# yml-bit/CTA-GAN

Measured on AMD Instinct MI355X. Metric: paired 512x512 slices/sec (G+D step); generator rel-L2 vs CPU reference, higher is better.
Workload: dtype bf16; 1 GPU; HdGan stage-2 full G+D train step (G, Reg, STN, D_m, losses, Adam x3), 16 paired 512x512 slices/GPU; per_gpu_batch=16, global_batch=16, size=512, parallelism=single, rccl_ranks=1, dp_backend=none

## Files before the change

cta_gan_amd/_lib.py:

```python
from __future__ import annotations

import ctypes
import os

import torch

_HERE = os.path.dirname(os.path.abspath(__file__))
LIB_PATH = os.environ.get("CTG_LIB") or os.path.join(_HERE, "_build", "libctagan_hip.so")

_I, _L, _P, _F = ctypes.c_int, ctypes.c_long, ctypes.c_void_p, ctypes.c_float

SIGNATURES = {
    "ctg_conv_igemm": "iipppp" + "i" * 20 + "ppppp",
    "ctg_conv_igemm_classes": "i" + "pppp" + "i" * 14 + "ppppppp",
    "ctg_conv_wgrad": "ipppiiiiiiiiiiiiipp",
    "ctg_wgrad_reduce": "piiiipiilllip",
    "ctg_wgrad_reduce_multi": "ippppppppppppp",
    "ctg_in_stats": "ipiiiiiipppp",
    "ctg_in_finalize": "piiiiippp",
    "ctg_in_apply": "ipippipipiiiiip",
    "ctg_in_apply_part": "ipipippipipiiiiip",
    "ctg_in_bwd_partial": "ipipiippiiiiiipp",
    "ctg_in_bwd_apply": "ipipiippppipiiiiip",
    "ctg_in_bwd_stats": "ipipiippipiiiiiipp",
    "ctg_in_bwd": "ipipiippipiiiiiipppp",
    "ctg_grad_combine": "ipipiipiipiiiiip",
    "ctg_fold_f32": "ppiiiiip",
    "ctg_act_bwd_f32": "ppiplp",
    "ctg_bias_grad": "ipiiiiiiiippip",
    "ctg_bias_grad_act": "ipiipiipiiiiiiippip",
    "ctg_maxpool2_fwd": "ipipiiiiip",
    "ctg_maxpool2_bwd": "ipipipiiiiiip",
    "ctg_bilinear_fwd": "ipipiiiiiiip",
    "ctg_bilinear_bwd": "ipipiiiiiiip",
    "ctg_copy_channels": "ipipiilp",
    "ctg_split_weights": "plpilp",
    "ctg_split_weights_multi": "ippppp",
    "ctg_pair_convert": "iplplilp",
    "ctg_abi_version": "",
    "ctg_chan_pad": "ipipilp",
    "ctg_im2col_pack": "ippiiiiiiiiipiiip",
    "ctg_conv_smallcin": "ippiiiiiiiiipiiipipiiiippp",
    "ctg_conv_tail7": "ipipppiiiip",
    "ctg_corr_smallcin": "piiiiiippiiiiiiiiiipip",
    "ctg_weight_pack": "ipllliipiiip",
    "ctg_weight_pack_multi": "iippppppppppp",
    "ctg_warp_fwd": "ppllllpiiip",
    "ctg_warp_bwd": "ppllllpppiiipp",
    "ctg_smooth_fwd": "plllliiiifppp",
    "ctg_smooth_bwd": "plllliiiifppip",
    "ctg_l1_fwd": "ppplfppp",
    "ctg_l1_bwd": "ppplfppip",
    "ctg_lsgan_fwd": "piiiffffippp",
    "ctg_lsgan_bwd": "piiiffffippp",
    "ctg_sum_scalars": "ippp",
    "ctg_act_bwd_sum_f32": "ppiplppip",
    "ctg_avgpool_fwd": "piipp",
    "ctg_avgpool_bwd": "piipp",
    "ctg_to_windowdata": "ppppilp",
    "ctg_window_metrics": "ppppiliippp",
    "ctg_ssim": "ppppiiiiidppp",
    "ctg_conv_cout1_fwd": "ipipppiiiiiiiiip",
    "ctg_conv_cout1_bwd": "ipppiiiiiiiiip",
    "ctg_conv_cout1_wgrad": "ippipiiiiiiiiip",
    "ctg_hu_to_inputs": "pffpplp",
    "ctg_resize_nearest": "piiipiip",
    "ctg_adam_step": "ipppppffffipp",
    "ctg_adam_tick": "pffp",
}
DIAG_SIGNATURES = {
    "ctg_lds_canary": "iipip",
}
_CT = {"i": _I, "l": _L, "p": _P, "f": _F, "d": ctypes.c_double}
ABI_VERSION = 11

_lib = None


def ensure_built():
    if os.environ.get("CTG_LIB") or os.environ.get("CTG_NO_AUTOBUILD") is not None:
        return
    from . import build as _build
    if _build.is_current():
        return
    try:
        _build._hipcc()
    except RuntimeError:
        return
    import sys
    print("cta_gan_amd: kernel sources changed -- building %s (hipcc, a few minutes)" % LIB_PATH, file=sys.stderr, flush=True)
    _build.build()


def load():
    global _lib
    if _lib is not None:
        return _lib
    ensure_built()
    if not os.path.exists(LIB_PATH):
        raise RuntimeError(
            "libctagan_hip.so not found at %s and hipcc is not available to build it (`python -m cta_gan_amd.build`): "
            "the HIP path is the only implementation; there is no fallback" % LIB_PATH)
    lib = ctypes.CDLL(LIB_PATH)
    try:
        ver = lib.ctg_abi_version
    except AttributeError:
        raise RuntimeError("%s predates ctg_abi_version(): rebuild it (`python -m cta_gan_amd.build --force`)" % LIB_PATH)
    ver.argtypes, ver.restype = [], _I
    if ver() != ABI_VERSION:
        raise RuntimeError("%s has C-ABI version %d, this binding was written against %d: rebuild it "
                           "(`python -m cta_gan_amd.build --force`)" % (LIB_PATH, ver(), ABI_VERSION))
    for name, sig in SIGNATURES.items():
        fn = getattr(lib, name)
        fn.argtypes = [_CT[c] for c in sig]
        fn.restype = _I
    for name, sig in DIAG_SIGNATURES.items():
        fn = getattr(lib, name, None)
        if fn is not None:
            fn.argtypes = [_CT[c] for c in sig]
            fn.restype = _I
    _lib = lib
    return lib


def check(status: int, what: str):
    if status != 0:
        if status == 1:
            raise RuntimeError("%s: invalid argument (CTG_EINVAL)" % what)
        raise RuntimeError("%s: HIP error %d" % (what, status - 1000))
```

cta_gan_amd/csrc/common.h:

```cpp
#pragma once
#include <hip/hip_runtime.h>
#include <stdint.h>
#include <utility>
#include "../../include/ctagan_hip.h"

#define CTG_OK 0
#define CTG_EINVAL 1

enum { DT_F32 = 0, DT_BF16 = 1, DT_PAIR = 2, DT_MIX = 3 };
enum { ACT_NONE = 0, ACT_RELU = 1, ACT_LRELU = 2, ACT_TANH = 3, ACT_SIGMOID = 4 };
enum { PAD_ZERO = 0, PAD_REFLECT = 1 };

typedef __bf16 bf16_t;
struct bfpair_t { bf16_t v; };
typedef float f32x4 __attribute__((ext_vector_type(4)));
typedef unsigned u32x4 __attribute__((ext_vector_type(4)));
typedef __bf16 bf16x8 __attribute__((ext_vector_type(8)));
typedef __bf16 bf16x4 __attribute__((ext_vector_type(4)));

#define LRELU_SLOPE 0.2f

#define CTG_ENTER() (void)hipGetLastError()

static inline int ctg_launch_status() {
    hipError_t e = hipGetLastError();
    return e == hipSuccess ? CTG_OK : 1000 + (int)e;
}

static inline int ctg_cu_count() {
    static int n_cu[64];
    int dev = 0;
    if (hipGetDevice(&dev) != hipSuccess) dev = 0;
    dev &= 63;
    if (n_cu[dev] == 0) {
        int n = 0;
        n_cu[dev] = (hipDeviceGetAttribute(&n, hipDeviceAttributeMultiprocessorCount, dev) == hipSuccess && n > 0) ? n : 256;
    }
    return n_cu[dev];
}
static inline int ctg_lds_attr_once(const void* fn, int bytes, unsigned long long* mask) {
    int dev = 0;
    if (hipGetDevice(&dev) != hipSuccess) dev = 0;
    const unsigned long long bit = 1ull << (dev & 63);
    if (*mask & bit) return CTG_OK;
    const hipError_t e = hipFuncSetAttribute(fn, hipFuncAttributeMaxDynamicSharedMemorySize, bytes);
    if (e != hipSuccess) return 1000 + (int)e;
    *mask |= bit;
    return CTG_OK;
}

template <typename T> struct VecOf;
template <> struct VecOf<float> { static constexpr int N = 4; };
template <> struct VecOf<bf16_t> { static constexpr int N = 8; };
template <> struct VecOf<bfpair_t> { static constexpr int N = 8; };

template <typename T> struct Chunk;
template <> struct Chunk<float> {
    static constexpr int N = 4;
    float v[4];
    __device__ __forceinline__ void load(const float* p) {
        const f32x4 t = *reinterpret_cast<const f32x4*>(p);
        v[0] = t[0]; v[1] = t[1]; v[2] = t[2]; v[3] = t[3];
    }
    __device__ __forceinline__ void store(float* p) const {
        *reinterpret_cast<f32x4*>(p) = f32x4{v[0], v[1], v[2], v[3]};
    }
    __device__ __forceinline__ void load(const float* p, int) { load(p); }
    __device__ __forceinline__ void store(float* p, int) const { store(p); }
    __device__ __forceinline__ void zero() { v[0] = v[1] = v[2] = v[3] = 0.f; }
};
template <> struct Chunk<bf16_t> {
    static constexpr int N = 8;
    float v[8];
    __device__ __forceinline__ void load(const bf16_t* p) {
        const u32x4 t = *reinterpret_cast<const u32x4*>(p);
#pragma unroll
        for (int i = 0; i < 4; ++i) {
            v[2 * i] = __uint_as_float(t[i] << 16);
            v[2 * i + 1] = __uint_as_float(t[i] & 0xffff0000u);
        }
    }
    __device__ __forceinline__ void store(bf16_t* p) const {
        bf16x8 o;
#pragma unroll
        for (int i = 0; i < 8; ++i) o[i] = (bf16_t)v[i];
        *reinterpret_cast<bf16x8*>(p) = o;
    }
    __device__ __forceinline__ void load(const bf16_t* p, int) { load(p); }
    __device__ __forceinline__ void store(bf16_t* p, int) const { store(p); }
    __device__ __forceinline__ void zero() {
#pragma unroll
        for (int i = 0; i < 8; ++i) v[i] = 0.f;
    }
};
template <> struct Chunk<bfpair_t> {
    static constexpr int N = 8;
    float v[8];
    __device__ __forceinline__ void load(const bfpair_t* p, int ld) {
        const u32x4 h = *reinterpret_cast<const u32x4*>(p);
        const u32x4 l = *reinterpret_cast<const u32x4*>(p + (ld >> 1));
#pragma unroll
        for (int i = 0; i < 4; ++i) {
            v[2 * i] = __uint_as_float(h[i] << 16) + __uint_as_float(l[i] << 16);
            v[2 * i + 1] = __uint_as_float(h[i] & 0xffff0000u) + __uint_as_float(l[i] & 0xffff0000u);
        }
    }
    __device__ __forceinline__ void store(bfpair_t* p, int ld) const {
        bf16x8 h, l;
#pragma unroll
        for (int i = 0; i < 8; ++i) {
            h[i] = (bf16_t)v[i];
            l[i] = (bf16_t)(v[i] - (float)h[i]);
        }
        *reinterpret_cast<bf16x8*>(p) = h;
        *reinterpret_cast<bf16x8*>(p + (ld >> 1)) = l;
    }
    __device__ __forceinline__ void zero() {
#pragma unroll
        for (int i = 0; i < 8; ++i) v[i] = 0.f;
    }
};
template <typename T> struct PlanesOf { static constexpr int N = 1; };
template <> struct PlanesOf<bfpair_t> { static constexpr int N = 2; };

__device__ __forceinline__ float ld1(const float* p) { return *p; }
__device__ __forceinline__ float ld1(const bf16_t* p) { return (float)*p; }
__device__ __forceinline__ void st1(float* p, float v) { *p = v; }
__device__ __forceinline__ void st1(bf16_t* p, float v) { *p = (bf16_t)v; }

__device__ __forceinline__ float act_apply(float x, int act) {
    switch (act) {
        case ACT_RELU: return x > 0.f ? x : 0.f;
        case ACT_LRELU: return x > 0.f ? x : LRELU_SLOPE * x;
        case ACT_TANH: return tanhf(x);
        case ACT_SIGMOID: return 1.f / (1.f + __expf(-x));
        default: return x;
    }
}
__device__ __forceinline__ float act_grad_from_out(float y, int act) {
    switch (act) {
        case ACT_RELU: return y > 0.f ? 1.f : 0.f;
        case ACT_LRELU: return y > 0.f ? 1.f : LRELU_SLOPE;
        case ACT_TANH: return 1.f - y * y;
        case ACT_SIGMOID: return y * (1.f - y);
        default: return 1.f;
    }
}

template <typename F, int... I>
__device__ __forceinline__ void static_for_impl(F&& f, std::integer_sequence<int, I...>) {
    (f(std::integral_constant<int, I>{}), ...);
}
template <int N, typename F> __device__ __forceinline__ void static_for(F&& f) {
    static_for_impl(static_cast<F&&>(f), std::make_integer_sequence<int, N>{});
}

#define IN_EPS 1e-5f

__device__ __forceinline__ int xcd_contiguous(int id, int G) {
    const int x = id & 7, q = G >> 3, r = G & 7;
    return x * q + (x < r ? x : r) + (id >> 3);
}

__device__ __forceinline__ void lds_barrier() {
    asm volatile("s_waitcnt lgkmcnt(0)" ::: "memory");
    __builtin_amdgcn_s_barrier();
    asm volatile("" ::: "memory");
}

template <int KCH> __device__ __forceinline__ int swz(int row, int c) {
    if constexpr (KCH == 4) return c ^ ((row >> 1) & 3);
    else return c ^ (row & 7);
}

__device__ __forceinline__ int reflect_idx(int i, int n) {
    i = i < 0 ? -i : i;
    return i >= n ? 2 * (n - 1) - i : i;
}

__device__ __forceinline__ float row16_sum_to_lane15(float v) {
    v += __builtin_bit_cast(float, __builtin_amdgcn_update_dpp(0, __builtin_bit_cast(int, v), 0x111, 0xf, 0xf, true));
    v += __builtin_bit_cast(float, __builtin_amdgcn_update_dpp(0, __builtin_bit_cast(int, v), 0x112, 0xf, 0xf, true));
    v += __builtin_bit_cast(float, __builtin_amdgcn_update_dpp(0, __builtin_bit_cast(int, v), 0x114, 0xf, 0xf, true));
    v += __builtin_bit_cast(float, __builtin_amdgcn_update_dpp(0, __builtin_bit_cast(int, v), 0x118, 0xf, 0xf, true));
    return v;
}

__device__ __forceinline__ float wave_sum(float v) {
#pragma unroll
    for (int o = 32; o > 0; o >>= 1) v += __shfl_xor(v, o, 64);
    return v;
}
```

cta_gan_amd/csrc/norm_act.hip:

```cpp
#include "common.h"
#include "ctg_knobs.h"

#define MAX_SLABS 128

__device__ __forceinline__ int fold_srcs(int y, int H, int p, int* s) {
    int k = 0;
    s[k++] = y;
    if (y >= 1 && y <= p) s[k++] = -y;
    if (y >= H - 1 - p && y <= H - 2) s[k++] = 2 * (H - 1) - y;
    return k;
}

template <typename T>
__device__ __forceinline__ void fold_load(Chunk<T>& out, const T* __restrict__ d, int n, int y, int x, int ch, int H,
                                          int W, int p, int ld) {
    if (p == 0) {
        out.load(d + (((size_t)n * H + y) * W + x) * ld + ch, ld);
        return;
    }
    const int Hp = H + 2 * p, Wp = W + 2 * p;
    int ys[3], xs[3];
    const int ny = fold_srcs(y, H, p, ys), nx = fold_srcs(x, W, p, xs);
    out.zero();
    for (int a = 0; a < ny; ++a)
// ... 23 lines not shown
    const int pbeg = slab * per, pend = min(pbeg + per, HW);
    const int ch = cc * EPC;
    float s1[EPC], s2[EPC], mu[EPC], rs[EPC];
#pragma unroll
    for (int e = 0; e < EPC; ++e) {
        s1[e] = 0.f; s2[e] = 0.f;
        if (MODE == 1) { mu[e] = mean[n * C + ch + e]; rs[e] = rstd[n * C + ch + e]; }
    }
    constexpr int UNR = 4;
    for (int pb = pbeg + pl; pb < pend; pb += PL * UNR) {
        Chunk<TX> v[UNR];
        Chunk<T> g[UNR];
        bool ok[UNR];
#pragma unroll
        for (int u = 0; u < UNR; ++u) {
            const int p = pb + u * PL;
            ok[u] = p < pend;
            const int pc = ok[u] ? p : pbeg;
            if (MODE == 0 || MODE == 1 || MODE == 3) v[u].load(x + ((size_t)n * HW + pc) * x_ld + ch, x_ld);
            if (MODE == 1 || MODE == 2 || MODE == 3) {
                if (pad == 0) {
                    g[u].load(dout + ((size_t)n * HW + pc) * d_ld + ch, d_ld);
                } else {
                    const int y = pc / W;
                    fold_load<T>(g[u], dout, n, y, pc - y * W, ch, H, W, pad, d_ld);
                }
            }
        }
#pragma unroll
        for (int u = 0; u < UNR; ++u) {
            if (!ok[u]) continue;
            if (MODE == 0) {
#pragma unroll
                for (int e = 0; e < EPC; ++e) { s1[e] += v[u].v[e]; s2[e] += v[u].v[e] * v[u].v[e]; }
            } else if (MODE == 1) {
#pragma unroll
                for (int e = 0; e < EPC; ++e) {
                    const float xh = (v[u].v[e] - mu[e]) * rs[e];
                    float gg = g[u].v[e];
                    if (act == ACT_RELU) gg = xh > 0.f ? gg : 0.f;
                    else if (act == ACT_LRELU) gg = xh > 0.f ? gg : LRELU_SLOPE * gg;
                    s1[e] += gg; s2[e] += gg * xh;
                }
            } else if (MODE == 3) {
                Chunk<T> o;
#pragma unroll
                for (int e = 0; e < EPC; ++e) {
                    o.v[e] = g[u].v[e] * act_grad_from_out(v[u].v[e], act);
                    s1[e] += o.v[e];
                }
                o.store(gout + ((size_t)n * HW + pb + u * PL) * go_ld + ch, go_ld);
            } else {
#pragma unroll
                for (int e = 0; e < EPC; ++e) s1[e] += g[u].v[e];
            }
        }
    }
    float* out = part + (((size_t)n * nslabs + slab) * C) * 2;
    __shared__ float stage[256 * 8];
#pragma unroll
    for (int which = 0; which < 2; ++which) {
        __syncthreads();
#pragma unroll
        for (int e = 0; e < EPC; ++e) stage[pl * C + ch + e] = which ? s2[e] : s1[e];
        __syncthreads();
        for (int c = tid; c < C; c += 256) {
            float s = 0.f;
            for (int q = 0; q < PL; ++q) s += stage[q * C + c];
            out[c * 2 + which] = s;
        }
    }
}


__global__ __launch_bounds__(64) void moments_finalize_wave_kernel(const float* __restrict__ part, int nslabs, int C,
                                                                   float invHW, int mode, float* __restrict__ mean,
                                                                   float* __restrict__ rstd) {
    const int i = blockIdx.x;
    const int n = i / C, c = i - n * C;
    double a = 0.0, b = 0.0;
    for (int s = threadIdx.x; s < nslabs; s += 64) {
        const float* p = part + (((size_t)n * nslabs + s) * C + c) * 2;
        a += (double)p[0];
        b += (double)p[1];
    }
#pragma unroll
    for (int o = 32; o > 0; o >>= 1) {
        a += __shfl_xor(a, o, 64);
        b += __shfl_xor(b, o, 64);
    }
    if (threadIdx.x == 0) {
        if (mode == 0) {
            const double m = a * invHW;
            double var = b * invHW - m * m;
            var = var < 0.0 ? 0.0 : var;
            mean[i] = (float)m;
            rstd[i] = (float)(1.0 / sqrt(var + (double)IN_EPS));
        } else {
            mean[i] = (float)(a * invHW);
            rstd[i] = (float)(b * invHW);
        }
    }
}

__global__ __launch_bounds__(64) void bias_finalize_kernel(const float* __restrict__ part, int B, int nslabs, int C,
                                                           int Creal, float* __restrict__ db, int accumulate) {
    const int c = blockIdx.x;
    if (c >= Creal) return;
    const int total = B * nslabs;
    float a = 0.f;
    for (int i = threadIdx.x; i < total; i += 64) a += part[((size_t)i * C + c) * 2];
    a = wave_sum(a);
    if (threadIdx.x == 0) db[c] = accumulate ? db[c] + a : a;
}

template <typename T> struct ChanParams {
    static constexpr int EPC = Chunk<T>::N;
    float v[EPC];
    __device__ __forceinline__ void load(const float* __restrict__ p) {
#pragma unroll
        for (int q = 0; q < EPC / 4; ++q) {
            const f32x4 t = *reinterpret_cast<const f32x4*>(p + 4 * q);
            v[4 * q] = t[0]; v[4 * q + 1] = t[1]; v[4 * q + 2] = t[2]; v[4 * q + 3] = t[3];
        }
    }
};

template <typename T>
__global__ __launch_bounds__(256) void in_apply_kernel(const T* x, int x_ld,
                                                       const float* __restrict__ mean,
                                                       const float* __restrict__ rstd, int act,
                                                       const T* res, int r_ld, T* out,
                                                       int o_ld, int HW, int C) {
    constexpr int EPC = Chunk<T>::N;
    const int CPP = C / EPC, PL = 256 / CPP;
    const int cc = threadIdx.x % CPP, pl = threadIdx.x / CPP;
    const int n = blockIdx.y, ch = cc * EPC;
    ChanParams<T> mu, rs;
    mu.load(mean + n * C + ch);
    rs.load(rstd + n * C + ch);
    const size_t base = (size_t)n * HW;
    for (int p = blockIdx.x * PL + pl; p < HW; p += gridDim.x * PL) {
        Chunk<T> v, o;
        v.load(x + (base + p) * x_ld + ch, x_ld);
#pragma unroll
        for (int e = 0; e < EPC; ++e) o.v[e] = act_apply((v.v[e] - mu.v[e]) * rs.v[e], act);
        if (res != nullptr) {
            Chunk<T> r;
            r.load(res + (base + p) * r_ld + ch, r_ld);
#pragma unroll
            for (int e = 0; e < EPC; ++e) o.v[e] += r.v[e];
        }
        o.store(out + (base + p) * o_ld + ch, o_ld);
    }
}

template <typename T, typename TX = T>
__global__ __launch_bounds__(256) void in_bwd_apply_kernel(const TX* __restrict__ x, int x_ld,
                                                           const T* __restrict__ dout, int d_ld, int pad,
                                                           const float* __restrict__ mean,
                                                           const float* __restrict__ rstd,
                                                           const float* __restrict__ s1,
                                                           const float* __restrict__ s2, int act,
                                                           T* __restrict__ dx, int dx_ld, int H, int W, int C) {
    constexpr int EPC = Chunk<T>::N;
    const int CPP = C / EPC, PL = 256 / CPP;
    const int cc = threadIdx.x % CPP, pl = threadIdx.x / CPP;
    const int n = blockIdx.y, ch = cc * EPC;
    const int HW = H * W;
    ChanParams<T> mu, rs, a1, a2;
    mu.load(mean + n * C + ch);
    rs.load(rstd + n * C + ch);
    a1.load(s1 + n * C + ch);
    a2.load(s2 + n * C + ch);
    const size_t base = (size_t)n * HW;
    for (int p = blockIdx.x * PL + pl; p < HW; p += gridDim.x * PL) {
        Chunk<TX> v;
        Chunk<T> g, o;
        v.load(x + (base + p) * x_ld + ch, x_ld);
        if (pad == 0) {
            g.load(dout + (base + p) * d_ld + ch, d_ld);
        } else {
            const int y = p / W;
            fold_load<T>(g, dout, n, y, p - y * W, ch, H, W, pad, d_ld);
        }
#pragma unroll
        for (int e = 0; e < EPC; ++e) {
            const float xh = (v.v[e] - mu.v[e]) * rs.v[e];
            float gg = g.v[e];
            if (act == ACT_RELU) gg = xh > 0.f ? gg : 0.f;
            else if (act == ACT_LRELU) gg = xh > 0.f ? gg : LRELU_SLOPE * gg;
            o.v[e] = rs.v[e] * (gg - a1.v[e] - xh * a2.v[e]);
        }
        o.store(dx + (base + p) * dx_ld + ch, dx_ld);
    }
}

#define FUSED_MAX_SLABS 128

template <int MODE>
__device__ __forceinline__ void wg_finalize(const float* __restrict__ part, int n, int nslabs, int C, int c0, int nch,
                                            float invHW, float* fa, float* fb, double* scratch) {
    const int tid = threadIdx.x;
    const int npairs = 2 * nch;
    const int stripes = 256 / npairs;
    const int pair = tid % npairs, stripe = tid / npairs;
    double acc = 0.0;
    const float* src = part + ((size_t)n * nslabs * C + c0) * 2 + pair;
    for (int s = stripe; s < nslabs; s += stripes) acc += (double)src[(size_t)s * C * 2];
    scratch[stripe * npairs + pair] = acc;
    __syncthreads();
    if (tid < nch) {
        double a = 0.0, b = 0.0;
        for (int q = 0; q < stripes; ++q) { a += scratch[q * npairs + 2 * tid]; b += scratch[q * npairs + 2 * tid + 1]; }
        if (MODE == 0) {
            const double m = a * invHW;
            double var = b * invHW - m * m;
            var = var < 0.0 ? 0.0 : var;
            fa[tid] = (float)m;
            fb[tid] = (float)(1.0 / sqrt(var + (double)IN_EPS));
        } else {
            fa[tid] = (float)(a * invHW);
            fb[tid] = (float)(b * invHW);
        }
    }
    __syncthreads();
}

template <typename T>
__global__ __launch_bounds__(256) void in_apply_part_kernel(const T* x, int x_ld,
                                                            const float* __restrict__ part, int nslabs, float invHW,
                                                            float* __restrict__ mean, float* __restrict__ rstd, int act,
                                                            const T* res, int r_ld, T* out,
                                                            int o_ld, int HW, int C, int CGC) {
    constexpr int EPC = Chunk<T>::N;
    __shared__ double scratch[256];
    __shared__ float fa[64], fb[64];
    const int PL = 256 / CGC;
    const int cc = threadIdx.x % CGC, pl = threadIdx.x / CGC;
    const int n = blockIdx.z, c0 = blockIdx.y * CGC * EPC, ch = c0 + cc * EPC;
    const size_t base = (size_t)n * HW;
    constexpr int UNR = 4;
    const int p0 = blockIdx.x * PL + pl, pstep = gridDim.x * PL;
    Chunk<T> v[UNR], r[UNR];
#pragma unroll
    for (int u = 0; u < UNR; ++u) {
        const int p = p0 + u * pstep;
        const int pc = p < HW ? p : 0;
        v[u].load(x + (base + pc) * x_ld + ch, x_ld);
        if (res != nullptr) r[u].load(res + (base + pc) * r_ld + ch, r_ld);
    }
    wg_finalize<0>(part, n, nslabs, C, c0, CGC * EPC, invHW, fa, fb, scratch);
    if (blockIdx.x == 0 && threadIdx.x < CGC * EPC) {
        mean[(size_t)n * C + c0 + threadIdx.x] = fa[threadIdx.x];
        rstd[(size_t)n * C + c0 + threadIdx.x] = fb[threadIdx.x];
    }
    float mu[EPC], rs[EPC];
#pragma unroll
    for (int e = 0; e < EPC; ++e) { mu[e] = fa[cc * EPC + e]; rs[e] = fb[cc * EPC + e]; }
    for (int pb = p0; pb < HW; pb += UNR * pstep) {
#pragma unroll
        for (int u = 0; u < UNR; ++u) {
            const int p = pb + u * pstep;
            if (p < HW) {
                Chunk<T> o;
#pragma unroll
                for (int e = 0; e < EPC; ++e) o.v[e] = act_apply((v[u].v[e] - mu[e]) * rs[e], act);
                if (res != nullptr) {
#pragma unroll
                    for (int e = 0; e < EPC; ++e) o.v[e] += r[u].v[e];
                }
                o.store(out + (base + p) * o_ld + ch, o_ld);
            }
        }
        const int pn = pb + UNR * pstep;
        if (pn < HW) {
#pragma unroll
            for (int u = 0; u < UNR; ++u) {
                const int p = pn + u * pstep;
                const int pc = p < HW ? p : 0;
                v[u].load(x + (base + pc) * x_ld + ch, x_ld);
                if (res != nullptr) r[u].load(res + (base + pc) * r_ld + ch, r_ld);
            }
        }
    }
}

template <typename T, typename TX = T>
__global__ __launch_bounds__(256) void in_bwd_apply_part_kernel(const TX* __restrict__ x, int x_ld,
                                                                const T* __restrict__ dout, int d_ld, int pad,
                                                                const float* __restrict__ mean,
                                                                const float* __restrict__ rstd,
                                                                const float* __restrict__ part, int nslabs, float invHW,
                                                                int act, T* __restrict__ dx, int dx_ld, int H, int W,
                                                                int C, int CGC) {
    constexpr int EPC = Chunk<T>::N;
    __shared__ double scratch[256];
    __shared__ float fa[64], fb[64];
    const int PL = 256 / CGC;
    const int cc = threadIdx.x % CGC, pl = threadIdx.x / CGC;
    const int n = blockIdx.z, c0 = blockIdx.y * CGC * EPC, ch = c0 + cc * EPC;
    const int HW = H * W;
    const size_t base = (size_t)n * HW;
    constexpr int UNR = 2;
    const int p0 = blockIdx.x * PL + pl, pstep = gridDim.x * PL;
    Chunk<TX> v[UNR];
// ... 21 lines not shown
#pragma unroll
    for (int e = 0; e < EPC; ++e) { a1[e] = fa[cc * EPC + e]; a2[e] = fb[cc * EPC + e]; }
    for (int pb = p0; pb < HW; pb += UNR * pstep) {
#pragma unroll
        for (int u = 0; u < UNR; ++u) {
            const int p = pb + u * pstep;
            if (p < HW) {
                Chunk<T> o;
#pragma unroll
                for (int e = 0; e < EPC; ++e) {
                    const float xh = (v[u].v[e] - mu.v[e]) * rs.v[e];
                    float gg = g[u].v[e];
                    if (act == ACT_RELU) gg = xh > 0.f ? gg : 0.f;
                    else if (act == ACT_LRELU) gg = xh > 0.f ? gg : LRELU_SLOPE * gg;
                    o.v[e] = rs.v[e] * (gg - a1[e] - xh * a2[e]);
                }
                o.store(dx + (base + p) * dx_ld + ch, dx_ld);
            }
        }
        const int pn = pb + UNR * pstep;
        if (pn < HW) fetch(pn);
    }
}

template <typename T>
__global__ void grad_combine_kernel(const T* __restrict__ a, int a_ld, const T* __restrict__ b, int b_ld, int pad,
                                    const T* __restrict__ yact, int y_ld, int act, T* __restrict__ out, int o_ld,
                                    int H, int W, int C, long items) {
    constexpr int EPC = Chunk<T>::N;
    const int CPP = C / EPC;
    const int HW = H * W;
    for (long it = (long)blockIdx.x * blockDim.x + threadIdx.x; it < items; it += (long)gridDim.x * blockDim.x) {
        const unsigned pixu = (unsigned)it / (unsigned)CPP;
        const long pix = pixu;
        const int ch = (int)(it - pix * CPP) * EPC;
        Chunk<T> o;
        o.zero();
        if (a != nullptr) o.load(a + pix * a_ld + ch, a_ld);
        if (b != nullptr) {
            const int n = (int)(pixu / (unsigned)HW);
            const int p = (int)(pix - (long)n * HW);
            const int y = p / W, xx = p - y * W;
            Chunk<T> t;
            fold_load<T>(t, b, n, y, xx, ch, H, W, pad, b_ld);
#pragma unroll
            for (int e = 0; e < EPC; ++e) o.v[e] += t.v[e];
        }
        if (yact != nullptr) {
            Chunk<T> yv;
            yv.load(yact + pix * y_ld + ch, y_ld);
#pragma unroll
            for (int e = 0; e < EPC; ++e) o.v[e] *= act_grad_from_out(yv.v[e], act);
        }
        o.store(out + pix * o_ld + ch, o_ld);
    }
}

__global__ void fold_f32_kernel(const float* __restrict__ dp, float* __restrict__ out, int B, int H, int W, int C,
                                int p) {
    const long total = (long)B * H * W * C;
    const int Hp = H + 2 * p, Wp = W + 2 * p;
    for (long i = (long)blockIdx.x * blockDim.x + threadIdx.x; i < total; i += (long)gridDim.x * blockDim.x) {
        const int c = (int)(i % C);
        const int x = (int)((i / C) % W);
        const int y = (int)((i / ((long)C * W)) % H);
        const int n = (int)(i / ((long)C * W * H));
        int ys[3], xs[3];
        const int ny = fold_srcs(y, H, p, ys), nx = fold_srcs(x, W, p, xs);
        float s = 0.f;
        for (int a = 0; a < ny; ++a)
            for (int b = 0; b < nx; ++b) s += dp[(((size_t)n * Hp + ys[a] + p) * Wp + xs[b] + p) * C + c];
        out[i] = s;
    }
}

__global__ void act_bwd_f32_kernel(const float* __restrict__ g, const float* __restrict__ y, int act,
                                   float* __restrict__ out, long n) {
    for (long i = (long)blockIdx.x * blockDim.x + threadIdx.x; i < n; i += (long)gridDim.x * blockDim.x)
        out[i] = g[i] * act_grad_from_out(y[i], act);
}

static inline int ew_blocks(long items) {
    long b = (items + 255) / 256;
    return (int)(b < 1 ? 1 : (b > 8192 ? 8192 : b));
}

static inline dim3 pix_grid(int dtype, int B, int HW, int C) {
    const int cpp = C / (dtype == DT_F32 ? 4 : 8);
    const int pl = 256 / cpp;
    const bool no_smallb = ctg_knobs().no_smallb;
    int per = 16;
    if (!no_smallb) while (per > 2 && (((long)HW + pl * per - 1) / (pl * per)) * B < 2048) per >>= 1;
    long bx = ((long)HW + pl * per - 1) / (pl * per);
    if (bx < 1) bx = 1;
    if (bx > 4096) bx = 4096;
    return dim3((unsigned)bx, (unsigned)B);
}

static inline bool pow2(int v) { return v > 0 && (v & (v - 1)) == 0; }

#define DISPATCH_T(dtype, CALL)                   \
    if ((dtype) == DT_BF16) { typedef bf16_t T; CALL; } \
    else if ((dtype) == DT_F32) { typedef float T; CALL; } \
    else if ((dtype) == DT_PAIR) { typedef bfpair_t T; CALL; } \
    else return CTG_EINVAL;

#define DISPATCH_TX(dtype, CALL)                  \
    if ((dtype) == DT_BF16) { typedef bf16_t T; typedef bf16_t TX; CALL; } \
    else if ((dtype) == DT_F32) { typedef float T; typedef float TX; CALL; } \
    else if ((dtype) == DT_PAIR) { typedef bfpair_t T; typedef bfpair_t TX; CALL; } \
    else if ((dtype) == DT_MIX) { typedef bf16_t T; typedef bfpair_t TX; CALL; } \
    else return CTG_EINVAL;

static int check_c(int dtype, int C) {
    const int epc = dtype == DT_F32 ? 4 : 8;
    if (C % epc) return CTG_EINVAL;
    const int cpp = C / epc;
    return (pow2(cpp) && cpp <= 256) ? CTG_OK : CTG_EINVAL;
}

extern "C" int ctg_in_stats(int dtype, const void* x, int x_ld, int B, int H, int W, int C, int nslabs, float* part,
                            float* mean, float* rstd, void* stream) {
    CTG_ENTER();
    if (check_c(dtype, C) || nslabs < 1 || nslabs > MAX_SLABS) return CTG_EINVAL;
    hipStream_t st = (hipStream_t)stream;
    DISPATCH_T(dtype, hipLaunchKernelGGL((moments_partial_kernel<T, 0>), dim3(nslabs, B), dim3(256), 0, st,
                                         (const T*)x, x_ld, (const T*)nullptr, 0, 0, (const float*)nullptr,
                                         (const float*)nullptr, 0, H, W, C, part));
    if (mean != nullptr)
        hipLaunchKernelGGL(moments_finalize_wave_kernel, dim3(B * C), dim3(64), 0, st, part, nslabs, C,
                           1.0f / (float)(H * W), 0, mean, rstd);
    return ctg_launch_status();
}

extern "C" int ctg_in_finalize(const float* part, int B, int C, int nslabs, int HW, int mode, float* mean, float* rstd,
                               void* stream) {
    CTG_ENTER();
    if (B < 1 || C < 1 || nslabs < 1 || HW < 1 || (mode != 0 && mode != 1)) return CTG_EINVAL;
    hipLaunchKernelGGL(moments_finalize_wave_kernel, dim3(B * C), dim3(64), 0, (hipStream_t)stream, part, nslabs, C,
                       1.0f / (float)HW, mode, mean, rstd);
    return ctg_launch_status();
}

extern "C" int ctg_in_apply(int dtype, const void* x, int x_ld, const float* mean, const float* rstd, int act,
                            const void* res, int r_ld, void* out, int o_ld, int B, int H, int W, int C, void* stream) {
    CTG_ENTER();
    if (check_c(dtype, C) || out == nullptr) return CTG_EINVAL;
    DISPATCH_T(dtype, hipLaunchKernelGGL((in_apply_kernel<T>), pix_grid(dtype, B, H * W, C), dim3(256), 0,
                                         (hipStream_t)stream, (const T*)x, x_ld, mean, rstd, act, (const T*)res, r_ld,
                                         (T*)out, o_ld, H * W, C));
    return ctg_launch_status();
}

static inline dim3 fused_grid(int dtype, int B, int HW, int C, int nslabs, int* cgc_out) {
    const int cpp = C / (dtype == DT_F32 ? 4 : 8);
    const int cgc = cpp < 8 ? cpp : 8;
    const int ncg = cpp / cgc, pl = 256 / cgc;
    long gx = (long)HW / (16L * nslabs);
    if (gx * ncg * B < 1024) gx = (1024 + (long)ncg * B - 1) / ((long)ncg * B);
    const long gmax = ((long)HW + pl * 4 - 1) / (pl * 4);
    if (gx > gmax) gx = gmax;
    if (gx < 1) gx = 1;
    *cgc_out = cgc;
    return dim3((unsigned)gx, (unsigned)ncg, (unsigned)B);
}

extern "C" int ctg_in_apply_part(int dtype, const void* x, int x_ld, const float* part, int nslabs, float* mean,
                                 float* rstd, int act, const void* res, int r_ld, void* out, int o_ld, int B, int H,
                                 int W, int C, void* stream) {
    CTG_ENTER();
    if (check_c(dtype, C) || nslabs < 1 || nslabs > FUSED_MAX_SLABS || part == nullptr || mean == nullptr || rstd == nullptr)
        return CTG_EINVAL;
    int cgc;
    const dim3 grid = fused_grid(dtype, B, H * W, C, nslabs, &cgc);
    DISPATCH_T(dtype, hipLaunchKernelGGL((in_apply_part_kernel<T>), grid, dim3(256), 0, (hipStream_t)stream, (const T*)x,
                                         x_ld, part, nslabs, 1.0f / (float)(H * W), mean, rstd, act, (const T*)res, r_ld,
                                         (T*)out, o_ld, H * W, C, cgc));
    return ctg_launch_status();
}

extern "C" int ctg_in_bwd_partial(int dtype, const void* x, int x_ld, const void* dout, int d_ld, int pad,
                                  const float* mean, const float* rstd, int act, int B, int H, int W, int C, int nslabs,
                                  float* part, void* stream) {
    CTG_ENTER();
    if (check_c(dtype, C) || nslabs < 1 || nslabs > MAX_SLABS || pad < 0 || pad >= H || pad >= W) return CTG_EINVAL;
    DISPATCH_TX(dtype, hipLaunchKernelGGL((moments_partial_kernel<T, 1, TX>), dim3(nslabs, B), dim3(256), 0,
                                          (hipStream_t)stream, (const TX*)x, x_ld, (const T*)dout, d_ld, pad, mean, rstd, act,
                                          H, W, C, part, (T*)nullptr, 0));
    return ctg_launch_status();
}

extern "C" int ctg_in_bwd(int dtype, const void* x, int x_ld, const void* dout, int d_ld, int pad, const float* mean,
                          const float* rstd, int act, void* dx, int dx_ld, int B, int H, int W, int C, int nslabs,
                          float* part, float* s1, float* s2, void* stream) {
    int st = ctg_in_bwd_partial(dtype, x, x_ld, dout, d_ld, pad, mean, rstd, act, B, H, W, C, nslabs, part, stream);
    if (st != CTG_OK) return st;
    st = ctg_in_finalize(part, B, C, nslabs, H * W, 1, s1, s2, stream);
    if (st != CTG_OK) return st;
    return ctg_in_bwd_apply(dtype, x, x_ld, dout, d_ld, pad, mean, rstd, s1, s2, act, dx, dx_ld, B, H, W, C, stream);
}

extern "C" int ctg_in_bwd_apply(int dtype, const void* x, int x_ld, const void* dout, int d_ld, int pad, const float* mean,
                                const float* rstd, const float* s1, const float* s2, int act, void* dx, int dx_ld, int B,
                                int H, int W, int C, void* stream) {
    CTG_ENTER();
    if (check_c(dtype, C) || pad < 0 || pad >= H || pad >= W || s1 == nullptr || s2 == nullptr) return CTG_EINVAL;
    DISPATCH_TX(dtype, hipLaunchKernelGGL((in_bwd_apply_kernel<T, TX>), pix_grid(dtype, B, H * W, C), dim3(256), 0,
                                          (hipStream_t)stream, (const TX*)x, x_ld, (const T*)dout, d_ld, pad, mean, rstd, s1, s2,
                                          act, (T*)dx, dx_ld, H, W, C));
    return ctg_launch_status();
}

extern "C" int ctg_in_bwd_stats(int dtype, const void* x, int x_ld, const void* dout, int d_ld, int pad, const float* mean,
                                const float* rstd, int act, void* dx, int dx_ld, int B, int H, int W, int C, int nslabs,
                                const float* part, void* stream) {
    CTG_ENTER();
    if (check_c(dtype, C) || nslabs < 1 || nslabs > FUSED_MAX_SLABS || part == nullptr || pad < 0 || pad >= H || pad >= W)
        return CTG_EINVAL;
    int cgc;
    const dim3 grid = fused_grid(dtype, B, H * W, C, nslabs, &cgc);
    DISPATCH_TX(dtype, hipLaunchKernelGGL((in_bwd_apply_part_kernel<T, TX>), grid, dim3(256), 0, (hipStream_t)stream, (const TX*)x,
                                          x_ld, (const T*)dout, d_ld, pad, mean, rstd, part, nslabs, 1.0f / (float)(H * W), act,
                                          (T*)dx, dx_ld, H, W, C, cgc));
    return ctg_launch_status();
}

extern "C" int ctg_grad_combine(int dtype, const void* a, int a_ld, const void* b, int b_ld, int pad, const void* yact,
                                int y_ld, int act, void* out, int o_ld, int B, int H, int W, int C, void* stream) {
    CTG_ENTER();
    const int epc = dtype == DT_F32 ? 4 : 8;
    if (C % epc || (a == nullptr && b == nullptr) || pad < 0 || pad >= H || pad >= W) return CTG_EINVAL;
    const long items = (long)B * H * W * (C / epc);
    if (items >= (1L << 31)) return CTG_EINVAL;
    DISPATCH_T(dtype, hipLaunchKernelGGL((grad_combine_kernel<T>), dim3(ew_blocks(items)), dim3(256), 0,
                                         (hipStream_t)stream, (const T*)a, a_ld, (const T*)b, b_ld, pad,
                                         (const T*)yact, y_ld, act, (T*)out, o_ld, H, W, C, items));
    return ctg_launch_status();
}

extern "C" int ctg_act_bwd_f32(const float* g, const float* y, int act, float* out, long n, void* stream) {
    CTG_ENTER();
    if (n < 1 || g == nullptr || y == nullptr || out == nullptr) return CTG_EINVAL;
    hipLaunchKernelGGL(act_bwd_f32_kernel, dim3(ew_blocks(n)), dim3(256), 0, (hipStream_t)stream, g, y, act, out, n);
    return ctg_launch_status();
}

extern "C" int ctg_bias_grad(int dtype, const void* g, int g_ld, int pad, int B, int H, int W, int C, int Creal,
                             int nslabs, float* part, float* db, int accumulate, void* stream) {
    CTG_ENTER();
    if (check_c(dtype, C) || nslabs < 1 || nslabs > MAX_SLABS || Creal > C) return CTG_EINVAL;
    hipStream_t st = (hipStream_t)stream;
    DISPATCH_T(dtype, hipLaunchKernelGGL((moments_partial_kernel<T, 2>), dim3(nslabs, B), dim3(256), 0, st,
                                         (const T*)nullptr, 0, (const T*)g, g_ld, pad, (const float*)nullptr,
                                         (const float*)nullptr, 0, H, W, C, part));
    hipLaunchKernelGGL(bias_finalize_kernel, dim3(Creal), dim3(64), 0, st, part, B, nslabs, C, Creal, db,
                       accumulate);
    return ctg_launch_status();
}

extern "C" int ctg_bias_grad_act(int dtype, const void* g, int g_ld, int pad, const void* yact, int y_ld, int act, void* gout,
                                 int go_ld, int B, int H, int W, int C, int Creal, int nslabs, float* part, float* db,
                                 int accumulate, void* stream) {
    CTG_ENTER();
    if (check_c(dtype, C) || nslabs < 1 || nslabs > MAX_SLABS || Creal > C || yact == nullptr || gout == nullptr) return CTG_EINVAL;
    if (act != ACT_RELU && act != ACT_LRELU) return CTG_EINVAL;
    hipStream_t st = (hipStream_t)stream;
    DISPATCH_T(dtype, hipLaunchKernelGGL((moments_partial_kernel<T, 3>), dim3(nslabs, B), dim3(256), 0, st,
                                         (const T*)yact, y_ld, (const T*)g, g_ld, pad, (const float*)nullptr,
                                         (const float*)nullptr, act, H, W, C, part, (T*)gout, go_ld));
    hipLaunchKernelGGL(bias_finalize_kernel, dim3(Creal), dim3(64), 0, st, part, B, nslabs, C, Creal, db, accumulate);
    return ctg_launch_status();
}

extern "C" int ctg_fold_f32(const float* dp, float* out, int B, int H, int W, int C, int pad, void* stream) {
    CTG_ENTER();
    if (pad < 1 || pad >= H || pad >= W || C < 1) return CTG_EINVAL;
    hipLaunchKernelGGL(fold_f32_kernel, dim3(ew_blocks((long)B * H * W * C)), dim3(256), 0, (hipStream_t)stream, dp,
                       out, B, H, W, C, pad);
    return ctg_launch_status();
}
```

cta_gan_amd/csrc/spatial.hip:

```cpp
#include "common.h"

static inline int ew_blocks(long items) {
    long b = (items + 255) / 256;
    return (int)(b < 1 ? 1 : (b > 8192 ? 8192 : b));
}

#define DISPATCH_T(dtype, CALL)                   \
    if ((dtype) == DT_BF16) { typedef bf16_t T; CALL; } \
    else if ((dtype) == DT_F32) { typedef float T; CALL; } \
    else if ((dtype) == DT_PAIR) { typedef bfpair_t T; CALL; } \
    else return CTG_EINVAL;

template <typename T>
__global__ void maxpool2_fwd_kernel(const T* __restrict__ x, int x_ld, T* __restrict__ out, int o_ld, int H, int W,
                                    int C, long items) {
    constexpr int EPC = Chunk<T>::N;
    const int CPP = C / EPC, Ho = H / 2, Wo = W / 2;
    for (long it = (long)blockIdx.x * blockDim.x + threadIdx.x; it < items; it += (long)gridDim.x * blockDim.x) {
        const unsigned pixu = (unsigned)it / (unsigned)CPP;
        const long pix = pixu;
        const int ch = (int)(it - pix * CPP) * EPC;
        const int ox = (int)(pixu % (unsigned)Wo);
        const int oy = (int)((pixu / (unsigned)Wo) % (unsigned)Ho);
        const int n = (int)(pixu / ((unsigned)Wo * (unsigned)Ho));
        const T* base = x + (((size_t)n * H + 2 * oy) * W + 2 * ox) * x_ld + ch;
        Chunk<T> a, b, c, d, o;
        a.load(base, x_ld); b.load(base + x_ld, x_ld); c.load(base + (size_t)W * x_ld, x_ld); d.load(base + (size_t)(W + 1) * x_ld, x_ld);
#pragma unroll
        for (int e = 0; e < EPC; ++e) o.v[e] = fmaxf(fmaxf(a.v[e], b.v[e]), fmaxf(c.v[e], d.v[e]));
        o.store(out + pix * o_ld + ch, o_ld);
    }
}

template <typename T, typename TX = T>
__global__ void maxpool2_bwd_kernel(const TX* __restrict__ x, int x_ld, const T* __restrict__ dout, int d_ld,
                                    T* __restrict__ dx, int dx_ld, int accumulate, int H, int W, int C, long items) {
    constexpr int EPC = Chunk<T>::N;
    const int CPP = C / EPC, Ho = H / 2, Wo = W / 2;
    for (long it = (long)blockIdx.x * blockDim.x + threadIdx.x; it < items; it += (long)gridDim.x * blockDim.x) {
        const unsigned pixu = (unsigned)it / (unsigned)CPP;
        const long pix = pixu;
        const int ch = (int)(it - pix * CPP) * EPC;
        const int xx = (int)(pixu % (unsigned)W);
        const int y = (int)((pixu / (unsigned)W) % (unsigned)H);
        const int n = (int)(pixu / ((unsigned)W * (unsigned)H));
        const int oy = y >> 1, ox = xx >> 1;
        Chunk<T> o;
        o.zero();
        if (oy < Ho && ox < Wo) {
            const TX* base = x + (((size_t)n * H + 2 * oy) * W + 2 * ox) * x_ld + ch;
            Chunk<TX> w[4];
            Chunk<T> g;
            w[0].load(base, x_ld); w[1].load(base + x_ld, x_ld); w[2].load(base + (size_t)W * x_ld, x_ld);
            w[3].load(base + (size_t)(W + 1) * x_ld, x_ld);
            g.load(dout + (((size_t)n * Ho + oy) * Wo + ox) * d_ld + ch, d_ld);
            const int me = (y & 1) * 2 + (xx & 1);
#pragma unroll
            for (int e = 0; e < EPC; ++e) {
                int arg = 0;
                float m = w[0].v[e];
#pragma unroll
                for (int k = 1; k < 4; ++k)
                    if (w[k].v[e] > m) { m = w[k].v[e]; arg = k; }
                o.v[e] = arg == me ? g.v[e] : 0.f;
            }
        }
        T* dst = dx + pix * dx_ld + ch;
        if (accumulate) {
            Chunk<T> prev;
            prev.load(dst, dx_ld);
#pragma unroll
            for (int e = 0; e < EPC; ++e) o.v[e] += prev.v[e];
        }
        o.store(dst, dx_ld);
    }
}

__device__ __forceinline__ void bil_src(int o, float scale, int Hi, int& i0, int& i1, float& l) {
    float s = scale * ((float)o + 0.5f) - 0.5f;
    s = s < 0.f ? 0.f : s;
    i0 = (int)s;
    i1 = i0 + (i0 < Hi - 1 ? 1 : 0);
    l = s - (float)i0;
}

template <typename T>
__global__ void bilinear_fwd_kernel(const T* __restrict__ x, int x_ld, T* __restrict__ out, int o_ld, int Hi, int Wi,
                                    int Ho, int Wo, int C, long items) {
    constexpr int EPC = Chunk<T>::N;
    const int CPP = C / EPC;
    const float sh = (float)Hi / (float)Ho, sw = (float)Wi / (float)Wo;
    for (long it = (long)blockIdx.x * blockDim.x + threadIdx.x; it < items; it += (long)gridDim.x * blockDim.x) {
        const unsigned pixu = (unsigned)it / (unsigned)CPP;
        const long pix = pixu;
        const int ch = (int)(it - pix * CPP) * EPC;
        const int ox = (int)(pixu % (unsigned)Wo);
        const int oy = (int)((pixu / (unsigned)Wo) % (unsigned)Ho);
        const int n = (int)(pixu / ((unsigned)Wo * (unsigned)Ho));
        int y0, y1, x0, x1;
        float ly, lx;
        bil_src(oy, sh, Hi, y0, y1, ly);
        bil_src(ox, sw, Wi, x0, x1, lx);
        const T* b = x + (size_t)n * Hi * Wi * x_ld + ch;
        Chunk<T> v00, v01, v10, v11, o;
        v00.load(b + ((size_t)y0 * Wi + x0) * x_ld, x_ld); v01.load(b + ((size_t)y0 * Wi + x1) * x_ld, x_ld);
        v10.load(b + ((size_t)y1 * Wi + x0) * x_ld, x_ld); v11.load(b + ((size_t)y1 * Wi + x1) * x_ld, x_ld);
        const float hy = 1.f - ly, hx = 1.f - lx;
#pragma unroll
        for (int e = 0; e < EPC; ++e)
            o.v[e] = hy * (hx * v00.v[e] + lx * v01.v[e]) + ly * (hx * v10.v[e] + lx * v11.v[e]);
        o.store(out + pix * o_ld + ch, o_ld);
    }
}

template <typename T>
__global__ void bilinear_bwd_kernel(const T* __restrict__ dout, int d_ld, T* __restrict__ dx, int dx_ld, int Hi,
                                    int Wi, int Ho, int Wo, int C, long items) {
    constexpr int EPC = Chunk<T>::N;
    const int CPP = C / EPC;
    const float sh = (float)Hi / (float)Ho, sw = (float)Wi / (float)Wo;
    for (long it = (long)blockIdx.x * blockDim.x + threadIdx.x; it < items; it += (long)gridDim.x * blockDim.x) {
        const unsigned pixu = (unsigned)it / (unsigned)CPP;
        const long pix = pixu;
        const int ch = (int)(it - pix * CPP) * EPC;
        const int ix = (int)(pixu % (unsigned)Wi);
        const int iy = (int)((pixu / (unsigned)Wi) % (unsigned)Hi);
        const int n = (int)(pixu / ((unsigned)Wi * (unsigned)Hi));
        float wy[5], wx[5];
#pragma unroll
        for (int k = 0; k < 5; ++k) {
            const int oy = 2 * iy - 2 + k, ox = 2 * ix - 2 + k;
            wy[k] = 0.f; wx[k] = 0.f;
            if (oy >= 0 && oy < Ho) {
                int a0, a1; float l;
                bil_src(oy, sh, Hi, a0, a1, l);
                wy[k] = (a0 == iy ? 1.f - l : 0.f) + (a1 == iy ? l : 0.f);
            }
            if (ox >= 0 && ox < Wo) {
                int a0, a1; float l;
                bil_src(ox, sw, Wi, a0, a1, l);
                wx[k] = (a0 == ix ? 1.f - l : 0.f) + (a1 == ix ? l : 0.f);
            }
        }
        Chunk<T> o;
        o.zero();
        const T* b = dout + (size_t)n * Ho * Wo * d_ld + ch;
        for (int a = 0; a < 5; ++a) {
            if (wy[a] == 0.f) continue;
            const int oy = 2 * iy - 2 + a;
            for (int c = 0; c < 5; ++c) {
                if (wx[c] == 0.f) continue;
                const int ox = 2 * ix - 2 + c;
                Chunk<T> g;
                g.load(b + ((size_t)oy * Wo + ox) * d_ld, d_ld);
                const float w = wy[a] * wx[c];
#pragma unroll
                for (int e = 0; e < EPC; ++e) o.v[e] += w * g.v[e];
            }
        }
        o.store(dx + pix * dx_ld + ch, dx_ld);
    }
}

template <typename T>
__global__ void chan_pad_kernel(const float* __restrict__ src, int Cs, T* __restrict__ dst, int Cpad, long P) {
    constexpr int EPC = Chunk<T>::N;
    const int CPP = Cpad / EPC;
    for (long pix = (long)blockIdx.x * blockDim.x + threadIdx.x; pix < P; pix += (long)gridDim.x * blockDim.x) {
        Chunk<T> o;
        o.zero();
        if (Cs == 2 && ((uintptr_t)src & 7) == 0) {
            const float2 v = *reinterpret_cast<const float2*>(src + pix * 2);
            o.v[0] = v.x; o.v[1] = v.y;
        } else {
            for (int c = 0; c < Cs; ++c) o.v[c] = src[pix * Cs + c];
        }
        constexpr int PL = PlanesOf<T>::N;
        T* d = dst + pix * Cpad * PL;
        o.store(d, Cpad * PL);
        o.zero();
        for (int cc = 1; cc < CPP; ++cc) o.store(d + cc * EPC, Cpad * PL);
    }
}

template <typename T>
__global__ void im2col_pack_kernel(const float* __restrict__ s0, const float* __restrict__ s1, int Cin, int Hi, int Wi,
                                   int kh, int kw, int stride, int pad, int pad_mode, T* __restrict__ dst, int Ho,
                                   int Wo, int Kpad, long items) {
    constexpr int EPC = Chunk<T>::N;
    const int CPP = Kpad / EPC;
    const int K = Cin * kh * kw;
    for (long it = (long)blockIdx.x * blockDim.x + threadIdx.x; it < items; it += (long)gridDim.x * blockDim.x) {
        const unsigned pixu = (unsigned)it / (unsigned)CPP;
        const long pix = pixu;
        const int cc = (int)(it - pix * CPP);
        const int ox = (int)(pixu % (unsigned)Wo);
        const int oy = (int)((pixu / (unsigned)Wo) % (unsigned)Ho);
        const int n = (int)(pixu / ((unsigned)Wo * (unsigned)Ho));
        Chunk<T> o;
#pragma unroll
        for (int e = 0; e < EPC; ++e) {
            const int k = cc * EPC + e;
            float v = 0.f;
            if (k < K) {
                const int c = k / (kh * kw);
                const int r = k - c * kh * kw;
                const int ky = r / kw, kx = r - ky * kw;
                int iy = oy * stride - pad + ky, ix = ox * stride - pad + kx;
                bool ok = true;
                if (pad_mode == PAD_REFLECT) { iy = reflect_idx(iy, Hi); ix = reflect_idx(ix, Wi); }
                else ok = (unsigned)iy < (unsigned)Hi && (unsigned)ix < (unsigned)Wi;
                if (ok) v = (c == 0 ? s0 : s1)[((size_t)n * Hi + iy) * Wi + ix];
            }
            o.v[e] = v;
        }
        o.store(dst + pix * Kpad * PlanesOf<T>::N + cc * EPC, Kpad * PlanesOf<T>::N);
    }
}

template <typename T>
__global__ void copy_channels_kernel(const T* __restrict__ src, int s_ld, T* __restrict__ dst, int d_ld, int C,
                                     long items) {
    constexpr int EPC = Chunk<T>::N;
    const int CPP = C / EPC;
    for (long it = (long)blockIdx.x * blockDim.x + threadIdx.x; it < items; it += (long)gridDim.x * blockDim.x) {
        const unsigned pixu = (unsigned)it / (unsigned)CPP;
        const long pix = pixu;
        const int ch = (int)(it - pix * CPP) * EPC;
        *reinterpret_cast<u32x4*>(dst + pix * d_ld + ch) = *reinterpret_cast<const u32x4*>(src + pix * s_ld + ch);
        if constexpr (PlanesOf<T>::N == 2)
            *reinterpret_cast<u32x4*>(dst + pix * d_ld + (d_ld >> 1) + ch) = *reinterpret_cast<const u32x4*>(src + pix * s_ld + (s_ld >> 1) + ch);
    }
}

extern "C" int ctg_maxpool2_fwd(int dtype, const void* x, int x_ld, void* out, int o_ld, int B, int H, int W, int C,
                                void* stream) {
    CTG_ENTER();
    const int epc = dtype == DT_F32 ? 4 : 8;
    if (C % epc || H < 2 || W < 2) return CTG_EINVAL;
    const long items = (long)B * (H / 2) * (W / 2) * (C / epc);
    if (items >= (1L << 31)) return CTG_EINVAL;
    DISPATCH_T(dtype, hipLaunchKernelGGL((maxpool2_fwd_kernel<T>), dim3(ew_blocks(items)), dim3(256), 0,
                                         (hipStream_t)stream, (const T*)x, x_ld, (T*)out, o_ld, H, W, C, items));
    return ctg_launch_status();
}

extern "C" int ctg_maxpool2_bwd(int dtype, const void* x, int x_ld, const void* dout, int d_ld, void* dx, int dx_ld,
                                int accumulate, int B, int H, int W, int C, void* stream) {
    CTG_ENTER();
    const int epc = dtype == DT_F32 ? 4 : 8;
    if (C % epc || H < 2 || W < 2) return CTG_EINVAL;
    const long items = (long)B * H * W * (C / epc);
    if (items >= (1L << 31)) return CTG_EINVAL;
    if (dtype == DT_MIX) {
        hipLaunchKernelGGL((maxpool2_bwd_kernel<bf16_t, bfpair_t>), dim3(ew_blocks(items)), dim3(256), 0, (hipStream_t)stream,
                           (const bfpair_t*)x, x_ld, (const bf16_t*)dout, d_ld, (bf16_t*)dx, dx_ld, accumulate, H, W, C, items);
        return ctg_launch_status();
    }
    DISPATCH_T(dtype, hipLaunchKernelGGL((maxpool2_bwd_kernel<T>), dim3(ew_blocks(items)), dim3(256), 0,
                                         (hipStream_t)stream, (const T*)x, x_ld, (const T*)dout, d_ld, (T*)dx, dx_ld,
                                         accumulate, H, W, C, items));
    return ctg_launch_status();
}

extern "C" int ctg_bilinear_fwd(int dtype, const void* x, int x_ld, void* out, int o_ld, int B, int Hi, int Wi, int Ho,
                                int Wo, int C, void* stream) {
    CTG_ENTER();
    const int epc = dtype == DT_F32 ? 4 : 8;
    if (C % epc) return CTG_EINVAL;
    const long items = (long)B * Ho * Wo * (C / epc);
    if (items >= (1L << 31)) return CTG_EINVAL;
    DISPATCH_T(dtype, hipLaunchKernelGGL((bilinear_fwd_kernel<T>), dim3(ew_blocks(items)), dim3(256), 0,
                                         (hipStream_t)stream, (const T*)x, x_ld, (T*)out, o_ld, Hi, Wi, Ho, Wo, C,
                                         items));
    return ctg_launch_status();
}

extern "C" int ctg_bilinear_bwd(int dtype, const void* dout, int d_ld, void* dx, int dx_ld, int B, int Hi, int Wi,
                                int Ho, int Wo, int C, void* stream) {
    CTG_ENTER();
    const int epc = dtype == DT_F32 ? 4 : 8;
    if (C % epc || Ho != 2 * Hi || Wo != 2 * Wi) return CTG_EINVAL;
    const long items = (long)B * Hi * Wi * (C / epc);
    if (items >= (1L << 31)) return CTG_EINVAL;
    DISPATCH_T(dtype, hipLaunchKernelGGL((bilinear_bwd_kernel<T>), dim3(ew_blocks(items)), dim3(256), 0,
                                         (hipStream_t)stream, (const T*)dout, d_ld, (T*)dx, dx_ld, Hi, Wi, Ho, Wo, C,
                                         items));
    return ctg_launch_status();
}

__global__ void split_weights_kernel(const float* __restrict__ x, long x_ld, bf16_t* __restrict__ out, int C, long P) {
    const int cpp = C / 8;
    const long items = P * cpp;
    for (long it = (long)blockIdx.x * blockDim.x + threadIdx.x; it < items; it += (long)gridDim.x * blockDim.x) {
        const long p = it / cpp;
        const int c = (int)(it - p * cpp) * 8;
        const float* src = x + p * x_ld + c;
        const f32x4 a = *reinterpret_cast<const f32x4*>(src), b = *reinterpret_cast<const f32x4*>(src + 4);
        bf16x8 hi, lo;
#pragma unroll
        for (int e = 0; e < 4; ++e) {
            hi[e] = (bf16_t)a[e];
            lo[e] = (bf16_t)(a[e] - (float)hi[e]);
            hi[4 + e] = (bf16_t)b[e];
            lo[4 + e] = (bf16_t)(b[e] - (float)hi[4 + e]);
        }
        bf16_t* row = out + p * (2L * C);
        const int j = c >> 5, i = c & 31;
        *reinterpret_cast<bf16x8*>(row + 64 * j + i) = hi;
        *reinterpret_cast<bf16x8*>(row + 64 * j + 32 + i) = lo;
    }
}

extern "C" int ctg_split_weights(const float* x, long x_ld, void* out, int C, long P, void* stream) {
    CTG_ENTER();
    if (C < 32 || C % 32 || x_ld < C || x_ld % 4 || P < 1 || ((uintptr_t)x & 15) || ((uintptr_t)out & 15)) return CTG_EINVAL;
    hipLaunchKernelGGL(split_weights_kernel, dim3(ew_blocks(P * (C / 8))), dim3(256), 0, (hipStream_t)stream, x, x_ld,
                       (bf16_t*)out, C, P);
    return ctg_launch_status();
}

#define SPLIT_MAX_T 32
struct SplitList {
    const float* src[SPLIT_MAX_T];
    bf16_t* dst[SPLIT_MAX_T];
    int C[SPLIT_MAX_T];
    long P[SPLIT_MAX_T];
    int first[SPLIT_MAX_T + 1];
    int count;
};
__global__ __launch_bounds__(256) void split_weights_multi_kernel(const SplitList L) {
    int j = 0;
    while (j + 1 < L.count && (int)blockIdx.x >= L.first[j + 1]) ++j;
    const int C = L.C[j], cpp = C / 8;
    const long items = L.P[j] * cpp;
    const long it = ((long)blockIdx.x - L.first[j]) * 256 + threadIdx.x;
    if (it >= items) return;
    const long p = it / cpp;
    const int c = (int)(it - p * cpp) * 8;
    const float* src = L.src[j] + p * C + c;
    const f32x4 a = *reinterpret_cast<const f32x4*>(src), b = *reinterpret_cast<const f32x4*>(src + 4);
    bf16x8 hi, lo;
#pragma unroll
    for (int e = 0; e < 4; ++e) {
        hi[e] = (bf16_t)a[e];
        lo[e] = (bf16_t)(a[e] - (float)hi[e]);
        hi[4 + e] = (bf16_t)b[e];
        lo[4 + e] = (bf16_t)(b[e] - (float)hi[4 + e]);
    }
    bf16_t* row = L.dst[j] + p * (2L * C);
    const int jj = c >> 5, i = c & 31;
    *reinterpret_cast<bf16x8*>(row + 64 * jj + i) = hi;
    *reinterpret_cast<bf16x8*>(row + 64 * jj + 32 + i) = lo;
}

extern "C" int ctg_split_weights_multi(int count, const void* const* x, void* const* out, const int* C, const long* P, void* stream) {
    CTG_ENTER();
    if (count < 0) return CTG_EINVAL;
    for (int base = 0; base < count; base += SPLIT_MAX_T) {
        SplitList L;
        L.count = count - base < SPLIT_MAX_T ? count - base : SPLIT_MAX_T;
        long blocks = 0;
        for (int i = 0; i < L.count; ++i) {
            const int q = base + i;
            if (C[q] < 32 || C[q] % 32 || P[q] < 1 || x[q] == nullptr || out[q] == nullptr || ((uintptr_t)x[q] & 15) || ((uintptr_t)out[q] & 15))
                return CTG_EINVAL;
            L.src[i] = (const float*)x[q]; L.dst[i] = (bf16_t*)out[q]; L.C[i] = C[q]; L.P[i] = P[q];
            L.first[i] = (int)blocks;
            blocks += (P[q] * (C[q] / 8) + 255) / 256;
            if (blocks >= (1L << 31)) return CTG_EINVAL;
        }
        L.first[L.count] = (int)blocks;
        if (blocks == 0) continue;
        hipLaunchKernelGGL(split_weights_multi_kernel, dim3((unsigned)blocks), dim3(256), 0, (hipStream_t)stream, L);
    }
    return ctg_launch_status();
}

__global__ void pair_from_f32_kernel(const float* __restrict__ src, long s_ld, bfpair_t* __restrict__ dst, int d_ld, int C,
                                     long items) {
    const int cpp = C / 8;
    for (long it = (long)blockIdx.x * blockDim.x + threadIdx.x; it < items; it += (long)gridDim.x * blockDim.x) {
        const long p = it / cpp;
        const int c = (int)(it - p * cpp) * 8;
        Chunk<float> a, b;
        a.load(src + p * s_ld + c);
        b.load(src + p * s_ld + c + 4);
        Chunk<bfpair_t> o;
#pragma unroll
        for (int e = 0; e < 4; ++e) { o.v[e] = a.v[e]; o.v[4 + e] = b.v[e]; }
        o.store(dst + p * d_ld + c, d_ld);
    }
}
__global__ void pair_to_f32_kernel(const bfpair_t* __restrict__ src, int s_ld, float* __restrict__ dst, long d_ld, int C,
                                   long items) {
    const int cpp = C / 8;
    for (long it = (long)blockIdx.x * blockDim.x + threadIdx.x; it < items; it += (long)gridDim.x * blockDim.x) {
        const long p = it / cpp;
        const int c = (int)(it - p * cpp) * 8;
        Chunk<bfpair_t> v;
        v.load(src + p * s_ld + c, s_ld);
        Chunk<float> a, b;
#pragma unroll
        for (int e = 0; e < 4; ++e) { a.v[e] = v.v[e]; b.v[e] = v.v[4 + e]; }
        a.store(dst + p * d_ld + c);
        b.store(dst + p * d_ld + c + 4);
    }
}

extern "C" int ctg_pair_convert(int dir, const void* src, long s_ld, void* dst, long d_ld, int C, long P, void* stream) {
    CTG_ENTER();
    if (C < 8 || C % 8 || P < 1 || (dir != 0 && dir != 1) || ((uintptr_t)src & 15) || ((uintptr_t)dst & 15)) return CTG_EINVAL;
    const long pl = dir == 0 ? d_ld : s_ld, fl = dir == 0 ? s_ld : d_ld;
    if (pl < 2 * C || pl % 16 || pl >= (1L << 31) || fl < C || fl % 4) return CTG_EINVAL;
    const long items = P * (C / 8);
    if (dir == 0)
        hipLaunchKernelGGL(pair_from_f32_kernel, dim3(ew_blocks(items)), dim3(256), 0, (hipStream_t)stream, (const float*)src,
                           s_ld, (bfpair_t*)dst, (int)d_ld, C, items);
    else
        hipLaunchKernelGGL(pair_to_f32_kernel, dim3(ew_blocks(items)), dim3(256), 0, (hipStream_t)stream,
                           (const bfpair_t*)src, (int)s_ld, (float*)dst, d_ld, C, items);
    return ctg_launch_status();
}

extern "C" int ctg_chan_pad(int dtype, const float* src, int Cs, void* dst, int Cpad, long P, void* stream) {
    CTG_ENTER();
    const int epc = dtype == DT_F32 ? 4 : 8;
    if (Cs < 1 || Cs > 4 || Cpad % epc || P * (Cpad / epc) >= (1L << 31)) return CTG_EINVAL;
    DISPATCH_T(dtype, hipLaunchKernelGGL((chan_pad_kernel<T>), dim3(ew_blocks(P)), dim3(256), 0,
                                         (hipStream_t)stream, src, Cs, (T*)dst, Cpad, P));
    return ctg_launch_status();
}

extern "C" int ctg_im2col_pack(int dtype, const float* s0, const float* s1, int Cin, int B, int Hi, int Wi, int kh,
                               int kw, int stride, int pad, int pad_mode, void* dst, int Ho, int Wo, int Kpad,
                               void* stream) {
    CTG_ENTER();
    const int epc = dtype == DT_F32 ? 4 : 8;
    if (Cin < 1 || Cin > 2 || (Cin == 2 && s1 == nullptr) || Kpad % epc || Kpad < Cin * kh * kw) return CTG_EINVAL;
    if (pad_mode == PAD_REFLECT && (pad >= Hi || pad >= Wi)) return CTG_EINVAL;
    if (Ho != (Hi + 2 * pad - kh) / stride + 1 || Wo != (Wi + 2 * pad - kw) / stride + 1) return CTG_EINVAL;
// ... 22 lines not shown
```

cta_gan_amd/engine.py:

```python
from __future__ import annotations

import os

from dataclasses import dataclass
from typing import Callable, List, Optional

import torch

from . import dp, ops
from .ops import ACT_LRELU, ACT_NONE, ACT_RELU, ACT_SIGMOID, ACT_TANH, PAD_REFLECT, PAD_ZERO, pack_tap


class Act:
    __slots__ = ("t", "grad", "req", "moments", "in_src", "in_plain", "grad_stats")

    def __init__(self, t: torch.Tensor, req: bool = False):
        self.t = t
        self.grad = None
        self.req = req
        self.moments = None
        self.in_src = None
        self.in_plain = False
        self.grad_stats = None

    @property
    def shape(self):
        return tuple(self.t.shape)


class Tape:
    def __init__(self, enabled: bool):
        self.enabled = enabled
        self.nodes: List[Callable[[], None]] = []

    def record(self, fn: Callable[[], None]):
        if self.enabled:
            self.nodes.append(fn)

    def backward(self):
        for fn in reversed(self.nodes):
            fn()
        self.nodes = []


_EMU_BF16_BWD = int(os.environ.get("CTG_EMU_BF16_BWD", "0") or 0)


def add_grad(a: Act, g: torch.Tensor, pad: int = 0):
    if not a.req:
        return
    if a.grad is None:
        a.grad = (g, pad)
        return
    g0, p0 = a.grad
    if p0 and pad:
        g0, p0 = _fold(g0, p0, a.t.shape), 0
    out = ops.empty_act(a.t.shape, g.dtype, g.device)
    if p0:
        ops.grad_combine(g, g0, p0, None, ACT_NONE, out)
    else:
        ops.grad_combine(g0, g, pad, None, ACT_NONE, out)
    a.grad = (out, 0)


def _fold(g, pad, shape):
    out = ops.empty_act(shape, g.dtype, g.device)
    ops.grad_combine(None, g, pad, None, ACT_NONE, out)
    return out


def take_grad(a: Act, allow_pad: bool = False):
    if a.grad is None:
        return None, 0
    g, pad = a.grad
    a.grad = None
    if _EMU_BF16_BWD and ops.is_pair(g):
        ops.pair_lo(g).zero_()
    if pad and not allow_pad:
        return _fold(g, pad, a.t.shape), 0
    return g, pad


class PackCache:

    def __init__(self):
        self.store = {}

    @staticmethod
    def _ver(param):
        return (param._version, getattr(param, "_ctg_version", 0))

    def get(self, param: torch.Tensor, kind: str, dtype, maker):
        key = (id(param), kind, dtype)
        ver = self._ver(param)
        hit = self.store.get(key)
        if hit is not None and hit[0] == ver and hit[2] == param.data_ptr():
            return hit[1]
        val = maker()
        self.store[key] = (ver, val, param.data_ptr(), None, None)
        return val

    def get_pack(self, param: torch.Tensor, kind: str, dtype, recipe):
        key = (id(param), kind, dtype)
        ver = self._ver(param)
        hit = self.store.get(key)
        if hit is not None and hit[0] == ver and hit[2] == param.data_ptr():
            return hit[1]
        ntaps, nreal, kreal, npad, kpad, sn, sk, stp = recipe
        val = ops.weight_pack(param, dtype, ntaps, nreal, kreal, npad, kpad, sn, sk, stp)
        self.store[key] = (ver, val, param.data_ptr(), recipe, param)
        return val

    def refresh(self):
        stale = {}
        for key, (ver, val, ptr, recipe, param) in self.store.items():
            if recipe is None or param is None:
                continue
            nv = self._ver(param)
            if nv != ver and ptr == param.data_ptr() and param.is_contiguous():
                stale.setdefault(key[2], []).append((key, nv, val, recipe, param))
        for dtype, items in stale.items():
            ops.weight_pack_multi([(param.detach(), val, r[0], r[1], r[2], r[3], r[4], r[5], r[6], r[7])
                                   for (_, _, val, r, param) in items])
            for key, nv, val, recipe, param in items:
                self.store[key] = (nv, val, param.data_ptr(), recipe, param)
            if ops.PAIR and dtype == torch.float32:
                ops.split_w_pair_refresh([val for (_, _, val, _, _) in items])


_NO_IN_FUSE = bool(os.environ.get("CTG_NO_IN_FUSE"))
_NO_BIAS_ACT = bool(os.environ.get("CTG_NO_BIAS_ACT"))
_NO_FRAME = bool(os.environ.get("CTG_NO_FRAME"))


def _round_up(v, m):
    return (v + m - 1) // m * m


def _bn_for(cout):
    return 128 if cout > 64 else 64 if cout > 32 else 32 if cout > 16 else 16


@dataclass
class ConvSpec:
    cin: int
    cout: int
    k: int
    stride: int = 1
    pad: int = 0
    reflect: bool = False
    transposed: bool = False
    use_bias: bool = True
    act: int = ACT_NONE
    out_f32: bool = False

    @property
    def kk(self):
        return self.k * self.k


def _taps_fwd(spec: ConvSpec):
    return [pack_tap(ky - spec.pad, kx - spec.pad, ky * spec.k + kx) for ky in range(spec.k) for kx in range(spec.k)]


def _taps_1d_transposed(k, pad, parity):
    return [(ky, (parity + pad - ky) // 2) for ky in range(k) if (parity + pad - ky) % 2 == 0]


def _convT_classes(k, pad):
    classes = []
    for py in (0, 1):
        for px in (0, 1):
            taps = [pack_tap(dy, dx, ky * k + kx)
                    for ky, dy in _taps_1d_transposed(k, pad, py) for kx, dx in _taps_1d_transposed(k, pad, px)]
            classes.append((py, px, taps))
    return classes


def _pack_dtype(dtype):
    return torch.float32 if (ops.PAIR and dtype == torch.bfloat16) else dtype


def _pack_fwd(cache: PackCache, spec: ConvSpec, w: torch.Tensor, dtype, kpad=None):
    dtype = _pack_dtype(dtype)
    npad = _round_up(spec.cout, _bn_for(spec.cout))
    kk = spec.kk
    if kpad is not None:
        return cache.get_pack(w, "fwd_packed", dtype, (1, spec.cout, spec.cin * kk, npad, kpad, spec.cin * kk, 1, 0)), npad
    if spec.transposed:
        return cache.get_pack(w, "fwd", dtype, (kk, spec.cout, spec.cin, npad, spec.cin, kk, spec.cout * kk, 1)), npad
    return cache.get_pack(w, "fwd", dtype, (kk, spec.cout, spec.cin, npad, spec.cin, spec.cin * kk, kk, 1)), npad


def _pack_bwd(cache: PackCache, spec: ConvSpec, w: torch.Tensor, dtype, kpad=None):
    dtype = _pack_dtype(dtype)
    npad = _round_up(spec.cin, _bn_for(spec.cin))
    kk = spec.kk
    kdim = spec.cout if kpad is None else kpad
    if spec.transposed:
        return cache.get_pack(w, "bwd", dtype, (kk, spec.cin, spec.cout, npad, kdim, spec.cout * kk, kk, 1)), npad
    return cache.get_pack(w, "bwd", dtype, (kk, spec.cin, spec.cout, npad, kdim, kk, spec.cin * kk, 1)), npad


def conv_out_hw(spec: ConvSpec, h, w):
    if spec.transposed:
        return 2 * h, 2 * w
    return (h + 2 * spec.pad - spec.k) // spec.stride + 1, (w + 2 * spec.pad - spec.k) // spec.stride + 1


def _cout1(spec, dtype):
    return ops.cout1_ok(spec.cin, spec.cout, spec.k, spec.stride, spec.reflect, spec.pad, spec.transposed, dtype)



def conv_forward(tape: Tape, cache: PackCache, spec: ConvSpec, x: Act, weight, bias, dtype,
                 img_sources=None) -> Act:
    dev = weight.device
    pad_mode = PAD_REFLECT if spec.reflect else PAD_ZERO
    b_eff = bias if spec.use_bias else None
    odt = torch.float32 if spec.out_f32 else dtype
    packed_x = None
    moments = None
    preq = (bool(weight.requires_grad), bool(bias is not None and bias.requires_grad))
    if img_sources is not None:
        s0, s1 = img_sources
        bsz, hi, wi = s0.shape
        ho, wo = conv_out_hw(spec, hi, wi)
        kpad = _round_up(spec.cin * spec.kk, 32)
        wp, npad = _pack_fwd(cache, spec, weight, dtype, kpad=kpad)
        y = ops.empty_act((bsz, ho, wo, spec.cout), odt, dev)

        def packed_x():
            return ops.im2col_pack(s0, s1, spec.k, spec.stride, spec.pad, pad_mode, dtype, kpad)
        packed_x.sources = (s0, s1)
        if ops.smallcin_ok(spec.cin, spec.cout, spec.k, dtype, odt, spec.stride):
            kxw = ops.kxw_ok(spec.cin, spec.cout, spec.k, spec.stride, dtype) and odt == dtype
            if kxw:
                pdt = _pack_dtype(dtype)
                wp = cache.get(weight, "fwd_kxw", pdt, lambda: ops.kxw_pack(weight.reshape(spec.cout, spec.kk), spec.k, npad, pdt))
            moments = ops.conv_smallcin(s0, s1, spec.k, spec.stride, spec.pad, pad_mode, wp, npad, b_eff, spec.act, y,
                                        spec.cout, want_stats=not spec.use_bias, kxw=kxw)
        else:
            px = packed_x()
            packed_x = lambda: px
            packed_x.sources = (s0, s1)
            ops.conv_igemm(px, wp, npad, y, b_eff, spec.cout, ho, wo, 0, 0, 1, 1, PAD_ZERO, spec.act,
                           [pack_tap(0, 0, 0)])
    else:
        bsz, hi, wi, cin = x.t.shape
        assert cin == spec.cin, (cin, spec.cin)
        ho, wo = conv_out_hw(spec, hi, wi)
        y = ops.empty_act((bsz, ho, wo, spec.cout), odt, dev)
        if spec.out_f32 and ops.conv_tail7_ok(spec.cin, spec.cout, spec.k, spec.stride, spec.reflect, spec.pad, dtype, hi, wi):
            tdt = "pair" if (ops.PAIR and dtype == torch.bfloat16) else dtype
            wp7 = cache.get(weight, "tail7", tdt, lambda: ops.tail7_pack(weight, tdt))
            ops.conv_tail7(x.t, wp7, b_eff, y, spec.act)
            out = Act(y, req=tape.enabled)
            if tape.enabled:
                tape.record(lambda: _conv_backward(cache, spec, x, out, weight, bias, dtype, None, preq))
            return out
        if spec.out_f32 and _cout1(spec, dtype):
            w16 = cache.get(weight, "cout1", torch.float32, lambda: ops.cout1_pack(weight))
            ops.conv_cout1_fwd(x.t, w16, b_eff, y, spec.act, spec.pad)
            out = Act(y, req=tape.enabled)
            if tape.enabled:
                tape.record(lambda: _conv_backward(cache, spec, x, out, weight, bias, dtype, None, preq))
            return out
        wp, npad = _pack_fwd(cache, spec, weight, dtype)
        if spec.transposed:
            classes = _convT_classes(spec.k, spec.pad)
            merged = ops.conv_igemm_classes(x.t, wp, npad, y, b_eff, spec.cout, hi, wi, classes, PAD_ZERO, spec.act,
                                            want_stats=not spec.use_bias)
            if merged is not None:
                if merged[0] is not None and merged[1] > 0:
                    moments = merged
            else:
                parts = []
                for py, px, taps in classes:
                    parts.append(ops.conv_igemm(x.t, wp, npad, y, b_eff, spec.cout, hi, wi, py, px, 2, 1, PAD_ZERO,
                                                spec.act, taps, want_stats=not spec.use_bias))
                if all(p is not None and p[1] > 0 for p in parts):
                    moments = (torch.cat([p[0] for p in parts], dim=1), sum(p[1] for p in parts))
        else:
            moments = ops.conv_igemm(x.t, wp, npad, y, b_eff, spec.cout, ho, wo, 0, 0, 1, spec.stride, pad_mode,
                                     spec.act, _taps_fwd(spec), want_stats=not spec.use_bias)
    out = Act(y, req=tape.enabled)
    if moments is not None and moments[1] > 0:
        out.moments = moments
    if tape.enabled:
        tape.record(lambda: _conv_backward(cache, spec, x, out, weight, bias, dtype, packed_x, preq))
    return out


def _conv_backward(cache, spec: ConvSpec, x: Act, out: Act, weight, bias, dtype, packed_x, preq=(True, True)):
    wreq, breq = preq
    g, _ = take_grad(out)
    if g is None:
        return
    dev = weight.device
    bsz, ho, wo, cout = out.t.shape
    pad_mode = PAD_REFLECT if spec.reflect else PAD_ZERO
    kk = spec.kk
    tail_db = fused_db = None
    if (spec.act != ACT_NONE and spec.out_f32 and cout == 1 and spec.use_bias and bias is not None and breq):
        tail_db = _grad_like(bias)
        g = ops.act_bwd_sum_f32(g.contiguous(), out.t.contiguous(), spec.act, tail_db)
    elif spec.act != ACT_NONE:
        if spec.out_f32 and g.numel() % 4:
            gg = ops.act_bwd_f32(g.contiguous(), out.t.contiguous(), spec.act)
        elif spec.out_f32:
            gg = torch.empty_like(g)
            n4 = g.numel() // 4
            ops.grad_combine(g.view(1, 1, n4, 4), None, 0, out.t.view(1, 1, n4, 4), spec.act, gg.view(1, 1, n4, 4))
        elif (spec.act in (ACT_RELU, ACT_LRELU) and spec.use_bias and bias is not None and breq and not _NO_BIAS_ACT
              and g.shape[-1] % 8 == 0):
            gg = ops.empty_like_act(g)
            fused_db = _grad_like(bias)
            ops.bias_grad_act(g, 0, out.t, spec.act, gg, cout, fused_db)
        else:
            gg = ops.empty_like_act(g)
            ops.grad_combine(g, None, 0, out.t, spec.act, gg)
        g = gg
    tail_dx_small = (spec.out_f32 and cout == 1 and spec.reflect and packed_x is None and spec.k * spec.k <= 64
                     and spec.stride == 1 and ops.smallcin_ok(1, spec.cin, spec.k, dtype, dtype))
    tail_small = tail_dx_small and ops.corr_smallcin_ok(1, spec.cin, spec.k, spec.stride, dtype)
    tail_dx_small = tail_small or (tail_dx_small and ops.PAIR)
    cout1 = spec.out_f32 and packed_x is None and _cout1(spec, dtype)
    if cout1:
        g1 = g.contiguous()
        if spec.use_bias and bias is not None and breq:
            db = tail_db
            if db is None:
                db = _grad_like(bias)
                torch.sum(g1.reshape(1, -1), dim=1, out=db)
            _store_param_grad(bias, db)
        if wreq:
            dw = _grad_like(weight)
            ops.conv_cout1_wgrad(g1, x.t, dw, spec.pad, defer=_REDUCE_JOBS)
            _store_param_grad(weight, dw)
        if x.req:
            bsz, hi, wi, cin = x.t.shape
            dx = ops.empty_act((bsz, hi, wi, cin), dtype, dev)
            ops.conv_cout1_bwd(g1, cache.get(weight, "cout1", torch.float32, lambda: ops.cout1_pack(weight)), dx, spec.pad)
            add_grad(x, dx, 0)
        return
    if tail_small:
        gm, m_c = None, cout
    elif spec.out_f32:
        gm = ops.chan_pad(g.contiguous(), cout, dtype, 32)
        m_c = 32
    else:
        gm = g
        m_c = cout
    if spec.use_bias and bias is not None and breq:
        if tail_db is not None or fused_db is not None:
            db = tail_db if tail_db is not None else fused_db
        elif tail_small:
            db = _grad_like(bias)
            torch.sum(g.reshape(1, -1), dim=1, out=db)
        else:
            db = _grad_like(bias)
            ops.bias_grad(gm, 0, cout, db)
        _store_param_grad(bias, db)
    if wreq:
        dw = _grad_like(weight)
        if tail_small:
            p = spec.pad
            ops.corr_smallcin(x.t, p, PAD_REFLECT, g.reshape(bsz, ho, wo), None, spec.k, 2 * p, PAD_ZERO,
                              ho + 2 * p, wo + 2 * p, dw, kk - 1, spec.cin, kk, kk, -1, defer=_REDUCE_JOBS)
        elif packed_x is not None and ops.corr_smallcin_ok(spec.cin, cout, spec.k, spec.stride, dtype) and not spec.out_f32:
            s0, s1 = packed_x.sources
            ops.corr_smallcin(gm, 0, PAD_ZERO, s0, s1, spec.k, spec.pad, pad_mode, ho, wo, dw, 0, cout,
                              spec.cin * kk, spec.cin * kk, 1, defer=_REDUCE_JOBS)
        elif packed_x is not None:
            ops.conv_wgrad(gm, packed_x(), [pack_tap(0, 0, 0)], 1, PAD_ZERO, dw, cout, spec.cin * kk,
                           spec.cin * kk, 1, 0, defer=_REDUCE_JOBS)
        elif spec.transposed:
            taps = [pack_tap(ky - spec.pad, kx - spec.pad, ky * spec.k + kx)
                    for ky in range(spec.k) for kx in range(spec.k)]
            ops.conv_wgrad(x.t, gm, taps, 2, PAD_ZERO, dw, spec.cin, cout, cout * kk, kk, 1, defer=_REDUCE_JOBS)
        else:
            g_w = gm[..., :16] if (spec.out_f32 and dtype == torch.bfloat16 and spec.stride == 1 and spec.k == 7
                                   and spec.cin % 64 == 0 and ho >= 8 and wo >= 16) else gm
            ops.conv_wgrad(g_w, x.t, _taps_fwd(spec), spec.stride, pad_mode, dw, cout, spec.cin, spec.cin * kk, kk, 1,
                           defer=_REDUCE_JOBS)
        _store_param_grad(weight, dw)
    if not x.req:
        return
    if packed_x is not None:
        bsz, hi, wi, cin = x.t.shape
        wb, npad = _pack_bwd(cache, spec, weight, dtype, kpad=m_c if spec.out_f32 else None)
        if spec.reflect:
            p = spec.pad
            assert spec.stride == 1
            dxp = torch.empty((bsz, hi + 2 * p, wi + 2 * p, cin), dtype=torch.float32, device=dev)
            taps = [pack_tap(-ky, -kx, ky * spec.k + kx) for ky in range(spec.k) for kx in range(spec.k)]
            ops.conv_igemm(gm, wb, npad, dxp, None, cin, hi + 2 * p, wi + 2 * p, 0, 0, 1, 1, PAD_ZERO, ACT_NONE, taps)
            add_grad(x, ops.fold_f32(dxp, p), 0)
            return
        dx = torch.empty((bsz, hi, wi, cin), dtype=torch.float32, device=dev)
        _bwd_data_launch(spec, gm, wb, npad, dx, hi, wi, cin)
        add_grad(x, dx, 0)
        return
    bsz, hi, wi, cin = x.t.shape
    if tail_dx_small:
        p = spec.pad
        kxw = ops.kxw_ok(1, cin, spec.k, 1, dtype)
        if kxw:
            wflip = cache.get(weight, "tail_bwd_kxw", _pack_dtype(dtype), lambda: ops.kxw_pack(
                weight.detach()[0].flip(-1, -2).reshape(cin, kk), spec.k, _round_up(cin, 32), _pack_dtype(dtype)))
        else:
            wflip = cache.get(weight, "tail_bwd_small", _pack_dtype(dtype), lambda: ops.weight_pack(
                weight.detach()[0].flip(-1, -2).reshape(cin, kk).contiguous(), _pack_dtype(dtype), 1, cin, kk, _round_up(cin, 32), 64,
                kk, 1, 0))
        dxp = ops.empty_act((bsz, hi + 2 * p, wi + 2 * p, cin), dtype, dev)
        ops.conv_smallcin(g.reshape(bsz, ho, wo), None, spec.k, 1, 2 * p, PAD_ZERO, wflip, _round_up(cin, 32), None,
                          ACT_NONE, dxp, cin, kxw=kxw)
        add_grad(x, dxp, p)
        return
    wb, npad = _pack_bwd(cache, spec, weight, dtype, kpad=m_c if spec.out_f32 else None)
    if spec.transposed:
        dx = ops.empty_act((bsz, hi, wi, cin), dtype, dev)
        taps = [pack_tap(ky - spec.pad, kx - spec.pad, ky * spec.k + kx) for ky in range(spec.k) for kx in range(spec.k)]
        ops.conv_igemm(gm, wb, npad, dx, None, cin, hi, wi, 0, 0, 1, 2, PAD_ZERO, ACT_NONE, taps)
        add_grad(x, dx, 0)
    elif spec.reflect:
        p = spec.pad
        dxp = ops.empty_act((bsz, hi + 2 * p, wi + 2 * p, cin), dtype, dev)
        assert spec.stride == 1
        taps = [pack_tap(-ky, -kx, ky * spec.k + kx) for ky in range(spec.k) for kx in range(spec.k)]
        if p == 1 and hi % 16 == 0 and wi % 16 == 0 and hi >= 32 and wi >= 32 and not _NO_FRAME:
            taps_in = [pack_tap(p - ky, p - kx, ky * spec.k + kx) for ky in range(spec.k) for kx in range(spec.k)]
            if ops.conv_fusable(cin, hi, wi):
                ops.conv_igemm(gm, wb, npad, dxp, None, cin, hi + 2 * p, wi + 2 * p, 0, 0, 1, 1, PAD_ZERO, ACT_NONE, taps,
                               frame=True)
                res = None
                if x.grad is not None and x.grad[1] == 0 and x.grad[0].dtype == dtype \
                        and tuple(x.grad[0].shape) == (bsz, hi, wi, cin):
                    res, x.grad = x.grad[0], None
                dx = ops.empty_act((bsz, hi, wi, cin), dtype, dev)
                want_in = (x.in_src is not None and x.grad is None and dtype == torch.bfloat16 and not _NO_IN_FUSE)
                in_arg = x.in_src if want_in else None
                if want_in and ops.PAIR_BWD_ACTIVE:
                    zact = x.in_src[3]
                    if zact == ACT_RELU and x.in_plain:
                        in_arg = (x.t, _unit_stats(x.t, 0.0), _unit_stats(x.t, 1.0), ACT_RELU)
                    elif zact != ACT_NONE:
                        want_in, in_arg = False, None
                part, slabs = ops.conv_igemm(gm, wb, npad, dx, None, cin, hi, wi, 0, 0, 1, 1, PAD_ZERO, ACT_NONE, taps_in,
                                             res=res, fold=dxp, in_bwd=in_arg)
                add_grad(x, dx, 0)
                if want_in and slabs > 0:
                    x.grad_stats = (dx, part)
                return
            ops.conv_igemm(gm, wb, npad, dxp, None, cin, hi, wi, p, p, 1, 1, PAD_ZERO, ACT_NONE, taps_in)
            ops.conv_igemm(gm, wb, npad, dxp, None, cin, hi + 2 * p, wi + 2 * p, 0, 0, 1, 1, PAD_ZERO, ACT_NONE, taps,
                           frame=True)
        else:
            ops.conv_igemm(gm, wb, npad, dxp, None, cin, hi + 2 * p, wi + 2 * p, 0, 0, 1, 1, PAD_ZERO, ACT_NONE, taps)
        add_grad(x, dxp, p)
    else:
        dx = ops.empty_act((bsz, hi, wi, cin), dtype, dev)
        _bwd_data_launch(spec, gm, wb, npad, dx, hi, wi, cin)
        add_grad(x, dx, 0)


_UNIT_STATS = {}


def _unit_stats(t, value):
    key = (t.device, t.shape[0], t.shape[3], value)
    hit = _UNIT_STATS.get(key)
    if hit is None:
        hit = _UNIT_STATS[key] = torch.full((t.shape[0], t.shape[3]), value, dtype=torch.float32, device=t.device)
    return hit


def _bwd_data_launch(spec: ConvSpec, gm, wb, npad, dx, hi, wi, cin):
    if spec.stride == 1:
        taps = [pack_tap(spec.pad - ky, spec.pad - kx, ky * spec.k + kx) for ky in range(spec.k) for kx in range(spec.k)]
        ops.conv_igemm(gm, wb, npad, dx, None, cin, hi, wi, 0, 0, 1, 1, PAD_ZERO, ACT_NONE, taps)
    else:
        assert spec.stride == 2
        classes = _convT_classes(spec.k, spec.pad)
        if hi % 2 == 0 and wi % 2 == 0 and dx.dtype == gm.dtype and \
                ops.conv_igemm_classes(gm, wb, npad, dx, None, cin, hi // 2, wi // 2, classes, PAD_ZERO, ACT_NONE) is not None:
            return
        for py, px, taps in classes:
            hs, ws = (hi - py + 1) // 2, (wi - px + 1) // 2
            if hs > 0 and ws > 0 and taps:
                ops.conv_igemm(gm, wb, npad, dx, None, cin, hs, ws, py, px, 2, 1, PAD_ZERO, ACT_NONE, taps)
            elif hs > 0 and ws > 0:
                ops.zero_act(dx[:, py::2, px::2, :])


def _grad_like(param):
    if dp._ACTIVE:
        buf = dp.grad_buffer(param)
        if buf is not None:
            return buf
    return torch.empty_like(param)


def fire_mark(net, tag):
    if dp._ACTIVE and (tag == "done" or dp.wants_mark(net, tag)):
        flush_reduces()
        dp.fire_mark(net, tag)


_PARAM_GRADS = None
_REDUCE_JOBS = None


def flush_reduces():
    if _REDUCE_JOBS:
        ops.wgrad_reduce_multi(_REDUCE_JOBS)
        del _REDUCE_JOBS[:]


def _store_param_grad(param, grad):
    if _PARAM_GRADS is None:
        raise RuntimeError("parameter gradient produced outside a network backward")
    prev = _PARAM_GRADS.get(id(param))
    if prev is not None:
        flush_reduces()
    _PARAM_GRADS[id(param)] = grad if prev is None else prev + grad


_INPLACE_NOGRAD = not __import__("os").environ.get("CTG_NO_INPLACE_IN")


def conv_inorm_forward(tape: Tape, cache: PackCache, spec: ConvSpec, x: Act, weight, bias, dtype, act: int,
                       res: Optional[Act] = None, out_t: Optional[torch.Tensor] = None) -> Act:
    if (not tape.enabled) and (not spec.use_bias) and spec.act == ACT_NONE and (not spec.transposed) and (not spec.out_f32) \
            and x.t.shape[-1] == spec.cin:
        bsz, hi, wi, _ = x.t.shape
        ho, wo = conv_out_hw(spec, hi, wi)
        if ops.conv_in_fusable(x.t, spec.cin, spec.cout, spec.k, spec.stride, ho, wo) and (ho, wo) == (hi, wi):
            wp, npad = _pack_fwd(cache, spec, weight, dtype)
            o = out_t if out_t is not None else ops.empty_act((bsz, ho, wo, spec.cout), dtype, weight.device)
            r = ops.conv_igemm(x.t, wp, npad, o, None, spec.cout, ho, wo, 0, 0, 1, 1, PAD_REFLECT if spec.reflect else PAD_ZERO,
                               ACT_NONE, _taps_fwd(spec), want_stats=True, res=res.t if res is not None else None, in_fuse=act)
            if r is not None:
                return Act(o, req=False)
    y = conv_forward(tape, cache, spec, x, weight, bias, dtype)
    return inorm_forward(tape, y, act, res=res, out_t=out_t)


def inorm_forward(tape: Tape, y: Act, act: int, res: Optional[Act] = None, out_t: Optional[torch.Tensor] = None) -> Act:
    if y.moments is not None:
        part, nsl = y.moments
        y.moments = None
    else:
        part, nsl = ops.in_partial(y.t)
    if out_t is not None:
        o = out_t
    elif not tape.enabled and _INPLACE_NOGRAD:
        o = y.t
    else:
        o = ops.empty_like_act(y.t)
    if ops.fin_fusable(nsl):
        mean, rstd = ops.in_apply_part(y.t, part, act, res.t if res is not None else None, o)
    else:
        mean, rstd = ops.in_finalize(part, nsl, y.t.shape[1] * y.t.shape[2])
        ops.in_apply(y.t, mean, rstd, act, res.t if res is not None else None, o)
    out = Act(o, req=tape.enabled)
    if tape.enabled:
        out.in_src = (y.t, mean, rstd, act)
        out.in_plain = res is None

        def bwd():
            g, pad = take_grad(out, allow_pad=True)
            st, out.grad_stats = out.grad_stats, None
            if g is None:
                return
            if res is not None and res.req:
                if pad:
                    g = _fold(g, pad, out.t.shape)
                    pad = 0
                add_grad(res, g, 0)
            if y.req:
                dy = ops.empty_like_act(y.t)
                if st is not None and st[0] is g and pad == 0:
                    ops.in_bwd_stats(y.t, g, mean, rstd, act, dy, st[1])
                else:
                    ops.in_bwd(y.t, g, pad, mean, rstd, act, dy)
                add_grad(y, dy, 0)
        tape.record(bwd)
    return out


def bnorm_forward(tape: Tape, y: Act, act: int, bn) -> Act:
    b, h, w, c = y.t.shape
    n = b * h * w
    training = bool(bn.training)
    gamma, beta = bn.weight.detach(), bn.bias.detach()
    with torch.no_grad():
        if training:
            part, nsl = y.moments if y.moments is not None else ops.in_partial(y.t)
            y.moments = None
            mean, rstd = ops.in_finalize(part.reshape(1, b * nsl, c, 2), b * nsl, n)
            mean, rstd = mean[0], rstd[0]
            var = 1.0 / (rstd * rstd) - bn.eps
            bn.running_mean.mul_(1.0 - bn.momentum).add_(bn.momentum * mean)
            bn.running_var.mul_(1.0 - bn.momentum).add_(bn.momentum * var * (n / max(n - 1, 1)))
            bn.num_batches_tracked += 1
        else:
            mean, rstd = bn.running_mean.float(), torch.rsqrt(bn.running_var.float() + bn.eps)
        gs = torch.where(gamma.abs() < 1e-30, torch.full_like(gamma, 1e-30), gamma)
        rstd_f = (rstd * gs).contiguous()
        mean_f = (mean - beta / rstd_f).contiguous()
        mean_bc, rstd_bc = mean_f.expand(b, c).contiguous(), rstd_f.expand(b, c).contiguous()
    o = ops.empty_like_act(y.t)
    ops.in_apply(y.t, mean_bc, rstd_bc, act, None, o)
    out = Act(o, req=tape.enabled)
    if tape.enabled:
        greq = (bool(bn.weight.requires_grad), bool(bn.bias.requires_grad))

        def bwd():
            g, pad = take_grad(out, allow_pad=True)
            if g is None:
                return
            part = ops.in_bwd_partial(y.t, g, pad, mean_bc, rstd_bc, act)
            sums = part.sum(dim=(0, 1))
            s1 = sums[:, 0]
            s2x = (sums[:, 1] - beta * s1) / gs
            if greq[0]:
                dg = _grad_like(bn.weight)
                dg.copy_(s2x)
                _store_param_grad(bn.weight, dg)
            if greq[1]:
                db = _grad_like(bn.bias)
                db.copy_(s1)
                _store_param_grad(bn.bias, db)
            if y.req:
                if training:
                    a2 = s2x / (gs * n)
                    a1 = s1 / n - beta * a2
                else:
                    a1 = a2 = torch.zeros_like(s1)
                dy = ops.empty_like_act(y.t)
                ops.in_bwd_apply(y.t, g, pad, mean_bc, rstd_bc, a1.expand(b, c).contiguous(), a2.expand(b, c).contiguous(), act, dy)
                add_grad(y, dy, 0)
        tape.record(bwd)
    return out


def maxpool_forward(tape: Tape, x: Act) -> Act:
    b, h, w, c = x.t.shape
    o = ops.empty_act((b, h // 2, w // 2, c), x.t.dtype, x.t.device)
    ops.maxpool2_fwd(x.t, o)
    out = Act(o, req=tape.enabled)
    if tape.enabled:
        def bwd():
            g, _ = take_grad(out)
            if g is None or not x.req:
                return
            if x.grad is not None and x.grad[1] == 0 and x.grad[0].shape == x.t.shape:
                ops.maxpool2_bwd(x.t, g, x.grad[0], True)
            else:
                dx = ops.empty_act(x.t.shape, g.dtype, g.device)
                ops.maxpool2_bwd(x.t, g, dx, False)
                add_grad(x, dx, 0)
        tape.record(bwd)
    return out


def upsample_concat_forward(tape: Tape, x: Act, skip: Act, buf: Optional[torch.Tensor] = None) -> Act:
    b, h, w, c1 = x.t.shape
    _, hs, ws, c2 = skip.t.shape
    in_place = buf is not None
    if in_place:
        assert buf.shape == (b, hs, ws, c1 + c2) and skip.t.data_ptr() == buf[..., c1:].data_ptr()
    else:
        buf = ops.empty_act((b, hs, ws, c1 + c2), x.t.dtype, x.t.device)
        ops.copy_channels(skip.t, buf[..., c1:])
    ops.bilinear_fwd(x.t, buf[..., :c1])
    out = Act(buf, req=tape.enabled)
    if tape.enabled:
        def bwd():
            g, _ = take_grad(out)
            if g is None:
                return
            if x.req:
                dx = ops.empty_act(x.t.shape, g.dtype, g.device)
                ops.bilinear_bwd(g[..., :c1], dx)
                add_grad(x, dx, 0)
            if skip.req:
                if in_place:
                    add_grad(skip, g[..., c1:], 0)
                else:
                    ds = ops.empty_act(skip.t.shape, g.dtype, g.device)
                    ops.copy_channels(g[..., c1:], ds)
                    add_grad(skip, ds, 0)
        tape.record(bwd)
    return out
```

cta_gan_amd/nets.py:

```python
from __future__ import annotations

import math
import os
from typing import Dict, List, Sequence

import torch
import torch.nn as nn

from . import engine as E
from . import ops
from .engine import ACT_LRELU, ACT_NONE, ACT_RELU, ACT_SIGMOID, ACT_TANH, Act, ConvSpec, Tape

_DEFAULT_DTYPE = torch.float32


def set_default_compute_dtype(dtype):
    global _DEFAULT_DTYPE
    pair = isinstance(dtype, str) and dtype in ("bf16x3", "bf16x3f")
    bwd_plain = pair and (dtype == "bf16x3f" or bool(os.environ.get("CTG_X3F")))
    if pair:
        dtype = torch.bfloat16
    if dtype not in (torch.float32, torch.bfloat16):
        raise ValueError('compute dtype must be torch.float32, torch.bfloat16, "bf16x3" or "bf16x3f"')
    _DEFAULT_DTYPE = dtype
    ops.set_pair_mode(pair, bwd_plain)


def default_compute_dtype():
    return _DEFAULT_DTYPE


def compute_mode():
    if ops.PAIR:
        return "bf16x3f" if ops.PAIR_BWD_PLAIN else "bf16x3"
    return "bf16" if _DEFAULT_DTYPE == torch.bfloat16 else "fp32"


class _Slot(nn.Module):

    def __init__(self, wshape, bshape):
        super().__init__()
        self.weight = nn.Parameter(torch.empty(wshape))
        self.bias = nn.Parameter(torch.empty(bshape))


class _BNSlot(nn.Module):

    def __init__(self, c, eps=1e-5, momentum=0.1):
        super().__init__()
        self.weight = nn.Parameter(torch.ones(c))
        self.bias = nn.Parameter(torch.zeros(c))
        self.register_buffer("running_mean", torch.zeros(c))
        self.register_buffer("running_var", torch.ones(c))
        self.register_buffer("num_batches_tracked", torch.tensor(0, dtype=torch.long))
        self.eps, self.momentum = eps, momentum


class _Tree(nn.Module):
    """Anonymous container: children are attached by (possibly numeric) name."""


def _attach(root: nn.Module, dotted: str, mod: nn.Module):
    parts = dotted.split(".")
    cur = root
    for p in parts[:-1]:
        if p not in cur._modules:
            cur.add_module(p, _Tree())
        cur = cur._modules[p]
    cur.add_module(parts[-1], mod)


def _default_conv_init(slot: _Slot):
    nn.init.kaiming_uniform_(slot.weight, a=math.sqrt(5))
    fan_in, _ = nn.init._calculate_fan_in_and_fan_out(slot.weight)
    bound = 1 / math.sqrt(fan_in) if fan_in > 0 else 0
    nn.init.uniform_(slot.bias, -bound, bound)


def _to_nhwc(x: torch.Tensor, dtype) -> torch.Tensor:
    t = x.permute(0, 2, 3, 1)
    if ops.PAIR and dtype == torch.bfloat16:
        return ops.to_pair(t.float().contiguous())
    if t.dtype != dtype:
        t = t.to(dtype)
    return t.contiguous()


def _to_nchw_view(t: torch.Tensor) -> torch.Tensor:
    if ops.is_pair(t):
        t = ops.from_pair(t)
    return t.permute(0, 3, 1, 2)


_NO_MULTI_REDUCE = bool(os.environ.get("CTG_NO_MULTI_REDUCE"))


def _require_cuda(x):
    if not x.is_cuda:
        raise RuntimeError("cta_gan_amd runs on an MI355X only: got a %s tensor and there is no CPU fallback "
                           "(use oracle/ for CPU reference results in tests)" % x.device)


class _NetFn(torch.autograd.Function):
    @staticmethod
    def forward(ctx, net, n_in, *tensors):
        n_in, grad_on = n_in
        inputs = tensors[:n_in]
        ctx.set_materialize_grads(False)
        need_in = [bool(f) and grad_on for f in ctx.needs_input_grad[2:2 + n_in]]
        need_any = grad_on and any(ctx.needs_input_grad[2:])
        tape = Tape(need_any)
        net._cache.refresh()
        out_acts, in_acts, finish = net._run(tape, inputs, need_in)
        ctx.tape, ctx.out_acts, ctx.in_acts, ctx.finish = tape, out_acts, in_acts, finish
        ctx.params = tensors[n_in:]
        ctx.net = net
        ctx.n_in = n_in
        ctx.in_shapes = [tuple(t.shape) for t in inputs]
        outs = tuple(_to_nchw_view(a.t) for a in out_acts)
        return outs

    @staticmethod
    def backward(ctx, *gouts):
        tape = ctx.tape
        if tape is None:
            raise RuntimeError("this network call was already back-propagated (the tape keeps no second copy)")
        grads: Dict[int, torch.Tensor] = {}
        E._PARAM_GRADS = grads
        E._REDUCE_JOBS = [] if not _NO_MULTI_REDUCE else None
        try:
            with ops.plain_backward():
                for a, g in zip(ctx.out_acts, gouts):
                    if g is None:
                        continue
                    E.add_grad(a, _to_nhwc(g, a.t.dtype), 0)
                tape.backward()
                E.flush_reduces()
                E.fire_mark(ctx.net, "done")
                in_grads = ctx.finish(ctx.in_acts) if ctx.finish is not None else [None] * ctx.n_in
        finally:
            E._PARAM_GRADS = None
            E._REDUCE_JOBS = None
        res = [None, None]
        for i in range(ctx.n_in):
            res.append(in_grads[i] if ctx.needs_input_grad[2 + i] else None)
        for p in ctx.params:
            res.append(grads.get(id(p)))
        ctx.tape = None
        ctx.net = None
        ctx.out_acts = ctx.in_acts = None
        return tuple(res)


class HipNet(nn.Module):

    def __init__(self):
        super().__init__()
        self.compute_dtype = None
        self._cache = E.PackCache()

    @property
    def dtype_(self):
        return self.compute_dtype or _DEFAULT_DTYPE

    def _call(self, *inputs):
        for x in inputs:
            _require_cuda(x)
        params = [p for p in self.parameters()]
        return _NetFn.apply(self, (len(inputs), torch.is_grad_enabled()), *inputs, *params)

    def _p(self, key: str):
        mod = self
        for part in key.split("."):
            mod = mod._modules[part] if part in mod._modules else getattr(mod, part)
        return mod


def _img_plane(x: torch.Tensor, c: int) -> torch.Tensor:
    t = x[:, c]
    if t.dtype != torch.float32:
        t = t.float()
    return t.contiguous()


def _image_grad_finish(n_ch):
    def finish(in_acts):
        a = in_acts[0]
        g, _ = E.take_grad(a)
        if g is None:
            return [None]
        return [_to_nchw_view(g)]
    return finish


class GeneratorNet(HipNet):

    def grad_buckets(self):
        late, early = [], []
        split = self.n_blocks // 2
        for key, p in self.named_parameters():
            parts = key.split(".")
            is_late = parts[0] == "model_tail" or (parts[0] == "model_body" and int(parts[1]) > split)
            (late if is_late else early).append(p)
        return [(late, "mid"), (early, "done")]

    def __init__(self, input_nc: int, output_nc: int, n_residual_blocks: int = 9):
        super().__init__()
        if input_nc not in (1, 2) or not 1 <= output_nc <= 4:
            raise NotImplementedError("HIP generator supports input_nc in {1,2}, output_nc <= 4 (reference uses 1/1)")
        self.input_nc, self.output_nc, self.n_blocks = input_nc, output_nc, n_residual_blocks
        shapes = [("model_head.1", (64, input_nc, 7, 7), 64), ("model_head.4", (128, 64, 3, 3), 128),
                  ("model_head.7", (256, 128, 3, 3), 256)]
        for i in range(n_residual_blocks):
            shapes += [("model_body.%d.conv_block.1" % i, (256, 256, 3, 3), 256),
                       ("model_body.%d.conv_block.5" % i, (256, 256, 3, 3), 256)]
        shapes += [("model_tail.0", (256, 128, 3, 3), 128), ("model_tail.3", (128, 64, 3, 3), 64),
                   ("model_tail.7", (output_nc, 64, 7, 7), output_nc)]
        for key, ws, bs in shapes:
            slot = _Slot(ws, (bs,))
            _attach(self, key, slot)
            _default_conv_init(slot)
        self.s_head = ConvSpec(input_nc, 64, 7, 1, 3, reflect=True, use_bias=False)
        self.s_d1 = ConvSpec(64, 128, 3, 2, 1, use_bias=False)
        self.s_d2 = ConvSpec(128, 256, 3, 2, 1, use_bias=False)
        self.s_res = ConvSpec(256, 256, 3, 1, 1, reflect=True, use_bias=False)
        self.s_u1 = ConvSpec(256, 128, 3, 2, 1, transposed=True, use_bias=False)
        self.s_u2 = ConvSpec(128, 64, 3, 2, 1, transposed=True, use_bias=False)
        self.s_tail = ConvSpec(64, output_nc, 7, 1, 3, reflect=True, use_bias=True, act=ACT_TANH, out_f32=True)

    def forward(self, x):
        return self._call(x)[0]

    def _run(self, tape: Tape, inputs, need_in):
        (x,) = inputs
        dt, cache = self.dtype_, self._cache
        b, c, h, w = x.shape
        assert c == self.input_nc
        if h % 4 or w % 4:
            raise RuntimeError("generator input height/width must be multiples of 4")
        x_act = Act(torch.zeros(1, device=x.device).expand(b, h, w, c), req=need_in[0])
        srcs = (_img_plane(x, 0), _img_plane(x, 1) if c == 2 else None)

        def wb(key):
            s = self._p(key)
            return s.weight, s.bias

        a = E.conv_forward(tape, cache, self.s_head, x_act, *wb("model_head.1"), dt, img_sources=srcs)
        a = E.inorm_forward(tape, a, ACT_RELU)
        a = E.conv_forward(tape, cache, self.s_d1, a, *wb("model_head.4"), dt)
        a = E.inorm_forward(tape, a, ACT_RELU)
        a = E.conv_forward(tape, cache, self.s_d2, a, *wb("model_head.7"), dt)
        a = E.inorm_forward(tape, a, ACT_RELU)
        for i in range(self.n_blocks):
            a = _res_block(tape, cache, self.s_res, a, wb("model_body.%d.conv_block.1" % i),
                           wb("model_body.%d.conv_block.5" % i), dt)
            if i == self.n_blocks // 2:
                tape.record(lambda: E.fire_mark(self, "mid"))
        a = E.conv_forward(tape, cache, self.s_u1, a, *wb("model_tail.0"), dt)
        a = E.inorm_forward(tape, a, ACT_RELU)
        a = E.conv_forward(tape, cache, self.s_u2, a, *wb("model_tail.3"), dt)
        a = E.inorm_forward(tape, a, ACT_RELU)
        a = E.conv_forward(tape, cache, self.s_tail, a, *wb("model_tail.7"), dt)
        return [a], [x_act], _image_grad_finish(c)


def _res_block(tape, cache, spec, x: Act, wb1, wb2, dt, out_t=None) -> Act:
    h = E.conv_inorm_forward(tape, cache, spec, x, wb1[0], wb1[1], dt, ACT_RELU)
    return E.conv_inorm_forward(tape, cache, spec, h, wb2[0], wb2[1], dt, ACT_NONE, res=x, out_t=out_t)


class ResidualBlockNet(HipNet):

    def __init__(self, in_features: int):
        super().__init__()
        c = in_features
        for idx in (1, 5):
            slot = _Slot((c, c, 3, 3), (c,))
            _attach(self, "conv_block.%d" % idx, slot)
            _default_conv_init(slot)
        self.spec = ConvSpec(c, c, 3, 1, 1, reflect=True, use_bias=False)

    def forward(self, x):
        return self._call(x)[0].to(x.dtype)

    def _run(self, tape, inputs, need_in):
        (x,) = inputs
        dt = self.dtype_
        xa = Act(_to_nhwc(x, dt), req=need_in[0])
        s1, s5 = self._p("conv_block.1"), self._p("conv_block.5")
        out = _res_block(tape, self._cache, self.spec, xa, (s1.weight, s1.bias), (s5.weight, s5.bias), dt)

        def finish(in_acts):
            g, _ = E.take_grad(in_acts[0])
            return [None if g is None else _to_nchw_view(g).to(x.dtype)]
        return [out], [xa], finish


class PatchStack:

    def __init__(self, owner: nn.Module, input_nc: int, keys: Sequence[str], ndf: int = 64, n_layers: int = 3,
                 sigmoid: bool = False, norm: str = "instance", norm_keys: Sequence[str] = ()):
        if input_nc not in (1, 2):
            raise NotImplementedError("HIP discriminator supports input_nc in {1, 2}")
        self.norm = norm
        self.input_nc = input_nc
        chans = [input_nc, ndf]
        nf = ndf
        for _ in range(1, n_layers):
            nf = min(nf * 2, 512)
            chans.append(nf)
        chans.append(min(nf * 2, 512))
        chans.append(1)
        self.chans = chans
        nconv = len(chans) - 1
        assert len(keys) == nconv
        self.keys = list(keys)
        root = owner
        self._root = [root]
        for i, key in enumerate(keys):
            slot = _Slot((chans[i + 1], chans[i], 4, 4), (chans[i + 1],))
            _attach(root, key, slot)
            _default_conv_init(slot)
        bn = norm == "batch"
        self.norm_keys = list(norm_keys)
        if bn:
            assert len(self.norm_keys) == nconv - 2
            for i, key in enumerate(self.norm_keys):
                _attach(root, key, _BNSlot(chans[i + 2]))
        self.specs = [ConvSpec(chans[0], chans[1], 4, 2, 1, use_bias=True, act=ACT_LRELU)]
        for i in range(1, nconv - 2):
            self.specs.append(ConvSpec(chans[i], chans[i + 1], 4, 2, 1, use_bias=bn))
        self.specs.append(ConvSpec(chans[nconv - 2], chans[nconv - 1], 4, 1, 1, use_bias=bn))
        self.specs.append(ConvSpec(chans[nconv - 1], 1, 4, 1, 1, use_bias=True, out_f32=True,
                                   act=ACT_SIGMOID if sigmoid else ACT_NONE))

    def _slots(self):
        root = self._root[0]
        out = []
        for key in self.keys:
            mod = root
            for part in key.split("."):
                mod = mod._modules[part]
            out.append(mod)
        return out

    def _norm_slot(self, j):
        mod = self._root[0]
        for part in self.norm_keys[j].split("."):
            mod = mod._modules[part]
        return mod

    def run_stack(self, tape: Tape, cache, x: torch.Tensor, need_in: bool, dt):
        b, c, h, w = x.shape
        assert c == self.input_nc
        slots = self._slots()
        x_act = Act(torch.zeros(1, device=x.device).expand(b, h, w, c), req=need_in)
        srcs = (_img_plane(x, 0), _img_plane(x, 1) if c == 2 else None)
        feats = []
        a = E.conv_forward(tape, cache, self.specs[0], x_act, slots[0].weight, slots[0].bias, dt, img_sources=srcs)
        feats.append(a)
        for i in range(1, len(self.specs) - 1):
            a = E.conv_forward(tape, cache, self.specs[i], a, slots[i].weight, slots[i].bias, dt)
            if self.norm == "batch":
                a = E.bnorm_forward(tape, a, ACT_LRELU, self._norm_slot(i - 1))
            else:
                a = E.inorm_forward(tape, a, ACT_LRELU)
            feats.append(a)
        a = E.conv_forward(tape, cache, self.specs[-1], a, slots[-1].weight, slots[-1].bias, dt)
        feats.append(a)
        return feats, x_act


class RegNet(HipNet):

    NDF = [32, 64, 64, 64, 64, 64, 64]
    NUF = [64, 64, 64, 64, 64, 64, 32]

    def __init__(self, nc_a: int, nc_b: int):
        super().__init__()
        if nc_a != 1 or nc_b != 1:
            raise NotImplementedError("HIP Reg supports single-channel image pairs (the reference's configuration)")
        self.add_module("offset_map", _Tree())

        def conv(key, cin, cout, k, act_lrelu=True, zeros=False):
            slot = _Slot((cout, cin, k, k), (cout,))
            _attach(self._modules["offset_map"], key + ".conv2d", slot)
            if zeros:
                nn.init.normal_(slot.weight, mean=0.0, std=1e-5)
            elif act_lrelu:
                nn.init.kaiming_normal_(slot.weight, a=0.2, nonlinearity="leaky_relu", mode="fan_in")
            else:
                nn.init.kaiming_normal_(slot.weight, a=0.0, nonlinearity="relu", mode="fan_in")
            slot.bias.data.zero_()

        def resblocks(key, dim, n):
            for i in range(n):
                for idx in (1, 5):
                    slot = _Slot((dim, dim, 3, 3), (dim,))
                    _attach(self._modules["offset_map"], "%s.model.%d.conv_block.%d" % (key, i, idx), slot)
                    nn.init.kaiming_normal_(slot.weight, a=0.0, nonlinearity="relu", mode="fan_in")
                    slot.bias.data.zero_()

        cin = nc_a + nc_b
        for i, c in enumerate(self.NDF, start=1):
            conv("down_%d.conv_0" % i, cin, c, 3)
            resblocks("down_%d.conv_0.resnet_block" % i, c, 1)
            cin = c
        conv("c1", cin, 2 * cin, 1)
        resblocks("t", 2 * cin, 3)
        conv("c2", 2 * cin, cin, 1)
        n = len(self.NDF)
        for i, c in zip(range(n, 0, -1), self.NUF):
            conv("up_%d" % i, cin + self.NDF[i - 1], c, 3)
            cin = c
        resblocks("refine.0", cin, 1)
        conv("refine.1", cin, cin, 1)
        conv("output", cin, 2, 3, act_lrelu=False, zeros=True)

    def _wb(self, key):
        mod = self._modules["offset_map"]
        for part in key.split("."):
            mod = mod._modules[part]
        return mod.weight, mod.bias

    def forward(self, img_a, img_b):
        return self._call(img_a, img_b)[0]

    def _resblocks(self, tape, x, key, dim, n, dt, out_t=None):
        spec = ConvSpec(dim, dim, 3, 1, 1, reflect=True, use_bias=False)
        for i in range(n):
            x = _res_block(tape, self._cache, spec, x, self._wb("%s.model.%d.conv_block.1" % (key, i)),
                           self._wb("%s.model.%d.conv_block.5" % (key, i)), dt, out_t=out_t if i == n - 1 else None)
        return x

    def _run(self, tape: Tape, inputs, need_in):
        img_a, img_b = inputs
        dt, cache = self.dtype_, self._cache
        b, _, h, w = img_a.shape
        if h % 128 or w % 128 or h < 256 or w < 256:
            raise RuntimeError("Reg input must be a multiple of 128 and >= 256 pixels: 7 pooling levels and a reflection-"
                               "padded bottleneck need >= 2x2 there (the reference fails the same way below 256)")
        need = need_in[0] or need_in[1]
        x_act = Act(torch.zeros(1, device=img_a.device).expand(b, h, w, 2), req=need)
        srcs = (_img_plane(img_a, 0), _img_plane(img_b, 0))
        skips = []
        x = None
        cin = 2
        n_lv = len(self.NDF)
        c_up, cprev = {}, self.NDF[-1]
        for i, c in zip(range(n_lv, 0, -1), self.NUF):
            c_up[i], cprev = cprev, c
        hh, ww = h, w
        for i, c in enumerate(self.NDF, start=1):
            spec = ConvSpec(cin, c, 3, 1, 1, use_bias=True, act=ACT_LRELU)
            wgt, bias = self._wb("down_%d.conv_0.conv2d" % i)
            if i == 1:
                x = E.conv_forward(tape, cache, spec, x_act, wgt, bias, dt, img_sources=srcs)
            else:
                x = E.conv_forward(tape, cache, spec, x, wgt, bias, dt)
            buf = ops.empty_act((b, hh, ww, c_up[i] + c), dt, img_a.device)
            x = self._resblocks(tape, x, "down_%d.conv_0.resnet_block" % i, c, 1, dt, out_t=buf[..., c_up[i]:])
            skips.append((x, buf))
            x = E.maxpool_forward(tape, x)
            cin = c
            hh, ww = hh // 2, ww // 2
        x = E.conv_forward(tape, cache, ConvSpec(cin, 2 * cin, 1, 1, 0, act=ACT_LRELU), x, *self._wb("c1.conv2d"), dt)
        x = self._resblocks(tape, x, "t", 2 * cin, 3, dt)
        x = E.conv_forward(tape, cache, ConvSpec(2 * cin, cin, 1, 1, 0, act=ACT_LRELU), x, *self._wb("c2.conv2d"), dt)
        n = len(self.NDF)
        for i, c in zip(range(n, 0, -1), self.NUF):
            s, buf = skips[i - 1]
            x = E.upsample_concat_forward(tape, x, s, buf=buf)
            x = E.conv_forward(tape, cache, ConvSpec(cin + self.NDF[i - 1], c, 3, 1, 1, act=ACT_LRELU), x,
                               *self._wb("up_%d.conv2d" % i), dt)
            cin = c
        x = self._resblocks(tape, x, "refine.0", cin, 1, dt)
        x = E.conv_forward(tape, cache, ConvSpec(cin, cin, 1, 1, 0, act=ACT_LRELU), x, *self._wb("refine.1.conv2d"), dt)
        x = E.conv_forward(tape, cache, ConvSpec(cin, 2, 3, 1, 1, use_bias=True, out_f32=True), x,
                           *self._wb("output.conv2d"), dt)

        def finish(in_acts):
            g, _ = E.take_grad(in_acts[0])
            if g is None:
                return [None, None]
            gv = _to_nchw_view(g)
            return [gv[:, 0:1] if need_in[0] else None, gv[:, 1:2] if need_in[1] else None]
        return [x], [x_act], finish


class _AvgPoolFn(torch.autograd.Function):

    @staticmethod
    def forward(ctx, x):
        ctx.shape = tuple(x.shape)
        return ops.avgpool_fwd(x.contiguous())

    @staticmethod
    def backward(ctx, g):
        return ops.avgpool_bwd(g, ctx.shape)


def global_avgpool(x: torch.Tensor) -> torch.Tensor:
    _require_cuda(x)
    if x.shape[1] != 1:
        raise NotImplementedError("global_avgpool: single-channel PatchGAN map expected")
    if x.dtype != torch.float32:
        x = x.float()
    return _AvgPoolFn.apply(x)


class _WarpFn(torch.autograd.Function):
    @staticmethod
    def forward(ctx, src, flow):
        ctx.save_for_backward(src, flow)
        return ops.warp_fwd(src, flow)

    @staticmethod
    def backward(ctx, g):
        src, flow = ctx.saved_tensors
        dsrc, dflow = ops.warp_bwd(src, flow, g, ctx.needs_input_grad[0], ctx.needs_input_grad[1])
        return dsrc, dflow


def warp(src, flow):
    _require_cuda(src)
    if src.shape[1] != 1 or flow.shape[1] != 2:
        raise NotImplementedError("Transformer_2D: 1-channel source and 2-channel flow expected")
    return _WarpFn.apply(src.float(), flow.float())


class _SmoothFn(torch.autograd.Function):
    @staticmethod
    def forward(ctx, f, weight):
        ctx.save_for_backward(f)
        ctx.weight = weight
        return ops.smooth_fwd(f, weight)

    @staticmethod
    def backward(ctx, g):
        (f,) = ctx.saved_tensors
        return ops.smooth_bwd(f, g.contiguous(), ctx.weight), None


def smoothing_loss(flow, weight=1.0):
    _require_cuda(flow)
    return _SmoothFn.apply(flow.float(), float(weight))


class _L1Fn(torch.autograd.Function):
    @staticmethod
    def forward(ctx, a, b, mask, weight):
        a, b = a.contiguous(), b.contiguous()
        mask = mask.contiguous() if mask is not None else None
        ctx.save_for_backward(a, b, mask)
        ctx.weight = weight
        return ops.l1_fwd(a, b, mask, weight)

    @staticmethod
    def backward(ctx, g):
        a, b, mask = ctx.saved_tensors
        return ops.l1_bwd(a, b, mask, g.contiguous(), ctx.weight), None, None, None


def l1_loss(a, b, weight=1.0):
    _require_cuda(a)
    return _L1Fn.apply(a.float(), b.detach().float(), None, float(weight))


def masked_l1_loss(a, b, mask_src, weight=1.0):
    _require_cuda(a)
    return _L1Fn.apply(a.float(), b.detach().float(), mask_src.detach().float(), float(weight))


class _LsganFn(torch.autograd.Function):
    @staticmethod
    def forward(ctx, x, nb, t0, s0, t1, s1, mode):
        loss, pooled = ops.lsgan_fwd(x, nb, t0, s0, t1, s1, mode)
        ctx.save_for_backward(pooled)
        ctx.args = (tuple(x.shape), nb, t0, s0, t1, s1, mode)
        return loss

    @staticmethod
    def backward(ctx, g):
        (pooled,) = ctx.saved_tensors
        shape, nb, t0, s0, t1, s1, mode = ctx.args
        return ops.lsgan_bwd(pooled, shape, nb, t0, s0, t1, s1, g.contiguous(), mode), None, None, None, None, None, None


def lsgan_loss(patch, target, weight=1.0, bce=False):
    _require_cuda(patch)
    if patch.shape[1] != 1:
        raise NotImplementedError("lsgan_loss: single-channel PatchGAN map expected")
    b = patch.shape[0]
    return _LsganFn.apply(patch.float().contiguous(), b, float(target), float(weight) / b, 0.0, 0.0, int(bool(bce)))


def lsgan_loss_pair(patch, nb, target_first, target_rest, weight=1.0, bce=False):
    _require_cuda(patch)
    b = patch.shape[0]
    if patch.shape[1] != 1 or not 0 < nb < b:
        raise NotImplementedError("lsgan_loss_pair: (B, 1, h, w) map with 0 < nb < B expected")
    return _LsganFn.apply(patch.float().contiguous(), nb, float(target_first), float(weight) / nb, float(target_rest),
                          float(weight) / (b - nb), int(bool(bce)))


class _SumFn(torch.autograd.Function):
    @staticmethod
    def forward(ctx, *terms):
        return ops.sum_scalars([t.reshape(()) for t in terms])

    @staticmethod
    def backward(ctx, g):
        return tuple(g for _ in ctx.needs_input_grad)

# ... 7 lines not shown
```

cta_gan_amd/ops.py:

```python
from __future__ import annotations

import ctypes
import os
import threading
from typing import Optional, Sequence

import torch

from . import _lib

ACT_NONE, ACT_RELU, ACT_LRELU, ACT_TANH, ACT_SIGMOID = 0, 1, 2, 3, 4
PAD_ZERO, PAD_REFLECT = 0, 1
_DT = {torch.float32: 0, torch.bfloat16: 1}
_EPC = {torch.float32: 4, torch.bfloat16: 8}


def dt(dtype) -> int:
    return _DT[dtype]


def epc(dtype) -> int:
    return _EPC[dtype]


DT_PAIR = 2
DT_MIX = 3

_env = os.environ.get
_NO_NIE = bool(_env("CTG_NO_NIE"))
NIE_POISON = bool(_env("CTG_NIE_POISON"))
NIE_MAX_WGS = int(_env("CTG_NIE_MAX_WGS", "1024"))
NIE_MAX_WGS_PAIR = int(_env("CTG_NIE_MAX_WGS_PAIR", "2048"))
NIE_BUDGET = int(_env("CTG_NIE_BUDGET", "0"))
NIE_SHARE = max(1, int(_env("CTG_NIE_SHARE", "2") or 2))
_TH8_WGS = 0 if _env("CTG_NO_TH8") is not None else int(_env("CTG_TH8_WGS", "384"))
_NO_HALO = bool(_env("CTG_NO_HALO"))
_NO_EPI_FUSE = bool(_env("CTG_NO_EPI_FUSE"))
_NO_WG_GROUPS_FIX = bool(_env("CTG_NO_WG_GROUPS_FIX"))
_WG_S2_FIX = not _env("CTG_NO_WG_S2_FIX")
_WG_FIX_BELOW = int(_env("CTG_WG_FIX_BELOW", "512"))
_NO_SMALLB = bool(_env("CTG_NO_SMALLB"))
_FIN_FUSE = bool(_env("CTG_FIN_FUSE"))
_NO_KXW = bool(_env("CTG_NO_KXW"))
DETERMINISTIC = bool(_env("CTG_DETERMINISTIC"))


def dtc(t) -> int:
    if _pair_now() and t.dtype == torch.bfloat16:
        return DT_PAIR
    return _DT[t.dtype]


def dtc_saved(t) -> int:
    if _PAIR_MODE and getattr(_TLS, "bwd_plain", False) and t.dtype == torch.bfloat16:
        return DT_MIX
    return dtc(t)


KERNEL_EVENTS = None


KERNEL_EVENT_STRIDE = 3
_event_count = {}
KERNEL_BYTES = {}


def _timed_begin(key, nbytes=None):
    if KERNEL_EVENTS is None or key is None:
        return None
    n = _event_count.get(key, 0)
    _event_count[key] = n + 1
    if n % KERNEL_EVENT_STRIDE:
        return None
    if nbytes is not None:
        KERNEL_BYTES[key] = nbytes
    e0 = torch.cuda.Event(enable_timing=True)
    e0.record()
    return e0


def _timed_end(key, e0):
    if e0 is not None:
        e1 = torch.cuda.Event(enable_timing=True)
        e1.record()
        KERNEL_EVENTS.setdefault(key, []).append((e0, e1))


OP_LOG = None


def _log_begin(label, flop, nbytes):
    if OP_LOG is None:
        return None
    e0 = torch.cuda.Event(enable_timing=True)
    e0.record()
    return (label, float(flop), float(nbytes), e0)


def _log_end(tok):
    if tok is not None:
        e1 = torch.cuda.Event(enable_timing=True)
        e1.record()
        OP_LOG.append(tok + (e1,))


def _esz(t):
    return 4 if is_pair(t) else t.element_size()


def _hbm_key(name, x, c_want=256):
    if KERNEL_EVENTS is None or x.shape[-1] != c_want:
        return None
    return "%s|%dx%dx%dx%d" % ((name,) + tuple(x.shape))


_PAIR_MODE = False
PAIR_BWD_PLAIN = False
_TLS = threading.local()


def set_pair_mode(pair: bool, bwd_plain: bool = False):
    global _PAIR_MODE, PAIR_BWD_PLAIN
    _PAIR_MODE, PAIR_BWD_PLAIN = bool(pair), bool(pair and bwd_plain)


def _pair_now() -> bool:
    return _PAIR_MODE and not getattr(_TLS, "bwd_plain", False)


class plain_backward:

    def __enter__(self):
        self.prev = getattr(_TLS, "bwd_plain", False)
        if PAIR_BWD_PLAIN:
            _TLS.bwd_plain = True
        return self

    def __exit__(self, *exc):
        _TLS.bwd_plain = self.prev
        return False


def __getattr__(name):
    if name == "PAIR":
        return _pair_now()
    if name == "PAIR_BWD_ACTIVE":
        return _PAIR_MODE and getattr(_TLS, "bwd_plain", False)
    raise AttributeError("module %r has no attribute %r" % (__name__, name))


def is_pair(t) -> bool:
    return _pair_now() and t.dtype == torch.bfloat16


def empty_act(shape, dtype, device):
    if _pair_now() and dtype == torch.bfloat16:
        b, h, w, c = shape
        if c % 8:
            raise RuntimeError("split-pair activations need a multiple of 8 channels, got %d" % c)
        return torch.empty((b, h, w, 2 * c), dtype=dtype, device=device)[..., :c]
    return torch.empty(tuple(shape), dtype=dtype, device=device)


def empty_like_act(t):
    return empty_act(t.shape, t.dtype, t.device)


def pair_lo(t):
    ld = _nhwc(t)[4]
    return t.as_strided(t.shape, t.stride(), t.storage_offset() + ld // 2)


def to_pair(x32, out=None):
    lib = _lib.load()
    b, h, w, c, ld = _nhwc(x32)
    assert x32.dtype == torch.float32 and _pair_now()
    if out is None:
        out = empty_act((b, h, w, c), torch.bfloat16, x32.device)
    assert tuple(out.shape) == (b, h, w, c) and is_pair(out)
    _lib.check(lib.ctg_pair_convert(0, _p(x32), ld, _p(out), _nhwc(out)[4], c, b * h * w, _stream()), "ctg_pair_convert")
    return out


def from_pair(xp):
    lib = _lib.load()
    b, h, w, c, ld = _nhwc(xp)
    assert is_pair(xp)
    out = torch.empty((b, h, w, c), dtype=torch.float32, device=xp.device)
    _lib.check(lib.ctg_pair_convert(1, _p(xp), ld, _p(out), c, c, b * h * w, _stream()), "ctg_pair_convert")
    return out


def zero_act(t):
    t.zero_()
    if is_pair(t):
        pair_lo(t).zero_()
# ... 308 lines not shown
    dtype = jobs[0][1].dtype
    assert all(j[1].dtype == dtype and j[0].dtype == torch.float32 and j[0].is_contiguous() for j in jobs)
    for j in jobs:
        old = getattr(j[1], "_ctg_split3w", None)
        if old is not None:
            j[1]._ctg_split3w_old = old
        j[1]._ctg_split3w = None
    _lib.check(lib.ctg_weight_pack_multi(
        dt(dtype), n, vp(*[j[0].data_ptr() for j in jobs]), vp(*[j[1].data_ptr() for j in jobs]),
        lg(*[j[7] for j in jobs]), lg(*[j[8] for j in jobs]), lg(*[j[9] for j in jobs]),
        it(*[j[3] for j in jobs]), it(*[j[4] for j in jobs]), it(*[j[2] for j in jobs]),
        it(*[j[5] for j in jobs]), it(*[j[6] for j in jobs]), _stream()), "ctg_weight_pack_multi")


def conv_wgrad(g, x, taps, is_, pad_mode, dst, mreal, nreal, sm, sn, stp, accumulate=False, target_blocks=768,
               defer=None):
    lib = _lib.load()
    b, hs, ws, mc, g_ld = _nhwc(g)
    b2, hi, wi, nc, x_ld = _nhwc(x)
    assert b == b2 and g.dtype == x.dtype and dst.dtype == torch.float32
    pairs = [(g, x)]
    fused_pair = is_pair(g)
    if fused_pair:
        assert is_pair(x)
    cdt = pairs[0][0].dtype
    bm = 128 if mc % 128 == 0 else 64 if mc % 64 == 0 else 32 if mc % 32 == 0 else 16
    bn = 128 if nc % 128 == 0 else 64 if nc % 64 == 0 else 32
    tiles = (mc // bm) * (nc // bn)
    hw = hs * ws
    nt_blk = 9 if (len(taps) == 9 and (bm, bn) in ((32, 32), (64, 32), (32, 64))) else \
        49 if (len(taps) == 49 and bm == 16) else 7 if (len(taps) == 49 and (bm, bn) == (32, 64)) else 1
    groups = tiles * (len(taps) // nt_blk) * b
    if is_ == 1 and cdt == torch.bfloat16 and len(taps) in (1, 4, 9) and hs >= 8 and ws >= 16 and not _NO_WG_GROUPS_FIX:
        halo_groups = (mc // min(bm, 64)) * (nc // min(bn, 64)) * b
        old_sps = max(1, min((target_blocks + groups - 1) // groups, (hw + 63) // 64))
        if halo_groups * old_sps < _WG_FIX_BELOW and not (mc == 256 and nc == 256):
            groups = halo_groups
            if _WG_FIX_BELOW > 256:
                target_blocks = 512
    if is_ == 2 and cdt == torch.bfloat16 and pad_mode == PAD_ZERO and hs >= 8 and ws >= 16 and mc % 32 == 0:
        halo_groups = (mc // min(bm, 64)) * (nc // min(bn, 64)) * b
        old_sps = max(1, min((target_blocks + groups - 1) // groups, (hw + 63) // 64))
        if halo_groups * old_sps < 256 or _WG_S2_FIX:
            groups = halo_groups
        target_blocks = 512
    sps = max(1, min((target_blocks + groups - 1) // groups, (hw + 63) // 64))
    slab = (((hw + sps - 1) // sps) + 63) // 64 * 64
    sps = (hw + slab - 1) // slab
    z1 = b * sps
    arr = _tap_array(taps)
    tok = _log_begin("wgrad %dx%d %dtaps is%d @%dx%d" % (mc, nc, len(taps), is_, hs, ws), 2.0 * b * hs * ws * mc * nc * len(taps),
                     (g.shape.numel() * _esz(g) + x.shape.numel() * _esz(x)) + z1 * len(taps) * mc * nc * 4.0) \
        if OP_LOG is not None else None
    e0 = _timed_begin("wgrad" if (mc == 256 and nc == 256 and len(taps) == 9 and is_ == 1) else None)
    part = None
    z = z1
    if fused_pair:
        part = torch.empty((3 * z1, len(taps), mc, nc), dtype=torch.float32, device=g.device)
        st = lib.ctg_conv_wgrad(DT_PAIR, _p(g), _p(x), _p(part), b, hs, ws, mc, g_ld, hi, wi, nc, x_ld, is_, pad_mode, slab,
                                len(taps), arr, _stream())
        if st == 2:
            pairs = [(g, x), (g, pair_lo(x)), (pair_lo(g), x)]
            z = 3 * z1
        elif st == 3:
            pairs = []
            z = 3 * z1
        else:
            _lib.check(st, "ctg_conv_wgrad")
            pairs = []
    if part is None:
        part = torch.empty((z, len(taps), mc, nc), dtype=torch.float32, device=g.device)
    for i, (gg, xx) in enumerate(pairs):
        st = lib.ctg_conv_wgrad(dt(cdt), _p(gg), _p(xx), _p(part[i * z1]), b, hs, ws, mc, _nhwc(gg)[4], hi, wi, nc,
                                _nhwc(xx)[4], is_, pad_mode, slab, len(taps), arr, _stream())
        _lib.check(st, "ctg_conv_wgrad")
    _timed_end("wgrad", e0)
    _log_end(tok)
    if defer is not None:
        defer.append((part, dst.data_ptr(), z, len(taps), mc, nc, mreal, nreal, sm, sn, stp, int(accumulate), dst))
        return
    _lib.check(lib.ctg_wgrad_reduce(_p(part), z, len(taps), mc, nc, _p(dst), mreal, nreal, sm, sn, stp,
                                    int(accumulate), _stream()), "ctg_wgrad_reduce")


def wgrad_reduce_multi(jobs):
    if not jobs:
        return
    lib = _lib.load()
    n = len(jobs)
    vp, lg, it = ctypes.c_void_p * n, ctypes.c_long * n, ctypes.c_int * n
    _lib.check(lib.ctg_wgrad_reduce_multi(
        n, vp(*[j[0].data_ptr() for j in jobs]), vp(*[j[1] for j in jobs]), it(*[j[2] for j in jobs]),
        it(*[j[3] for j in jobs]), it(*[j[4] for j in jobs]), it(*[j[5] for j in jobs]), it(*[j[6] for j in jobs]),
        it(*[j[7] for j in jobs]), lg(*[j[8] for j in jobs]), lg(*[j[9] for j in jobs]), lg(*[j[10] for j in jobs]),
        it(*[j[11] for j in jobs]), _stream()), "ctg_wgrad_reduce_multi")


def _nslabs(b, hw):
    if b < 16 and not _NO_SMALLB:
        return int(max(1, min(128, (1024 + b - 1) // b, (hw + 63) // 64)))
    return int(max(1, min(64, (1024 + b - 1) // b, (hw + 255) // 256)))


def in_stats(x):
    lib = _lib.load()
    b, h, w, c, ld = _nhwc(x)
    ns = _nslabs(b, h * w)
    part = torch.empty((b, ns, c, 2), dtype=torch.float32, device=x.device)
    mean = torch.empty((b, c), dtype=torch.float32, device=x.device)
    rstd = torch.empty_like(mean)
    _lib.check(lib.ctg_in_stats(dtc(x), _p(x), ld, b, h, w, c, ns, _p(part), _p(mean), _p(rstd), _stream()),
               "ctg_in_stats")
    return mean, rstd


def in_partial(x):
    lib = _lib.load()
    b, h, w, c, ld = _nhwc(x)
    ns = _nslabs(b, h * w)
    part = torch.empty((b, ns, c, 2), dtype=torch.float32, device=x.device)
    _lib.check(lib.ctg_in_stats(dtc(x), _p(x), ld, b, h, w, c, ns, _p(part), None, None, _stream()), "ctg_in_stats")
    return part, ns


def in_finalize(part, nslabs, hw, mode=0):
    lib = _lib.load()
    b, ns, c, _ = part.shape
    assert ns == nslabs and part.is_contiguous()
    mean = torch.empty((b, c), dtype=torch.float32, device=part.device)
    rstd = torch.empty_like(mean)
    _lib.check(lib.ctg_in_finalize(_p(part), b, c, nslabs, hw, mode, _p(mean), _p(rstd), _stream()), "ctg_in_finalize")
    return mean, rstd


FUSED_MAX_SLABS = 128


def fin_fusable(nslabs):
    return nslabs <= FUSED_MAX_SLABS and _FIN_FUSE


def in_apply(x, mean, rstd, act, res, out):
    lib = _lib.load()
    b, h, w, c, ld = _nhwc(x)
    _, _, _, _, o_ld = _nhwc(out)
    r_ld = _nhwc(res)[4] if res is not None else 0
    key = _hbm_key("in_apply_res" if res is not None else "in_apply", x)
    e0 = _timed_begin(key, x.numel() * _esz(x) * (3 if res is not None else 2))
    _lib.check(lib.ctg_in_apply(dtc(x), _p(x), ld, _p(mean), _p(rstd), act, _p(res), r_ld, _p(out), o_ld, b, h, w, c, _stream()),
               "ctg_in_apply")
    _timed_end(key, e0)


def in_apply_part(x, part, act, res, out):
    lib = _lib.load()
    b, h, w, c, ld = _nhwc(x)
    _, _, _, _, o_ld = _nhwc(out)
    r_ld = _nhwc(res)[4] if res is not None else 0
    ns = part.shape[1]
    assert part.shape == (b, ns, c, 2) and part.is_contiguous() and ns <= FUSED_MAX_SLABS
    mean = torch.empty((b, c), dtype=torch.float32, device=x.device)
    rstd = torch.empty_like(mean)
    key = _hbm_key("in_apply_res" if res is not None else "in_apply", x)
    e0 = _timed_begin(key, x.numel() * _esz(x) * (3 if res is not None else 2))
    _lib.check(lib.ctg_in_apply_part(dtc(x), _p(x), ld, _p(part), ns, _p(mean), _p(rstd), act, _p(res), r_ld, _p(out),
                                     o_ld, b, h, w, c, _stream()), "ctg_in_apply_part")
    _timed_end(key, e0)
    return mean, rstd


def in_bwd(x, dout, pad, mean, rstd, act, dx):
    lib = _lib.load()
    b, h, w, c, ld = _nhwc(x)
    d_ld = _nhwc(dout)[4]
    assert dout.shape[1] == h + 2 * pad and dout.shape[2] == w + 2 * pad and dout.dtype == x.dtype
    ns = _nslabs(b, h * w)
    part = torch.empty((b, ns, c, 2), dtype=torch.float32, device=x.device)
    key = _hbm_key("in_bwd_partial", x) if pad == 0 else None
    e0 = _timed_begin(key, x.numel() * x.element_size() * 2)
    _lib.check(lib.ctg_in_bwd_partial(dtc_saved(x), _p(x), ld, _p(dout), d_ld, pad, _p(mean), _p(rstd), act, b, h, w, c, ns,
                                      _p(part), _stream()), "ctg_in_bwd_partial")
    _timed_end(key, e0)
    in_bwd_stats(x, dout, mean, rstd, act, dx, part, pad=pad)


def in_bwd_partial(x, dout, pad, mean, rstd, act):
    lib = _lib.load()
    b, h, w, c, ld = _nhwc(x)
    d_ld = _nhwc(dout)[4]
    ns = _nslabs(b, h * w)
    part = torch.empty((b, ns, c, 2), dtype=torch.float32, device=x.device)
    _lib.check(lib.ctg_in_bwd_partial(dtc_saved(x), _p(x), ld, _p(dout), d_ld, pad, _p(mean), _p(rstd), act, b, h, w, c, ns,
                                      _p(part), _stream()), "ctg_in_bwd_partial")
    return part


def in_bwd_apply(x, dout, pad, mean, rstd, s1, s2, act, dx):
    lib = _lib.load()
    b, h, w, c, ld = _nhwc(x)
    _lib.check(lib.ctg_in_bwd_apply(dtc_saved(x), _p(x), ld, _p(dout), _nhwc(dout)[4], pad, _p(mean), _p(rstd), _p(s1), _p(s2), act,
                                    _p(dx), _nhwc(dx)[4], b, h, w, c, _stream()), "ctg_in_bwd_apply")


def in_bwd_stats(x, dout, mean, rstd, act, dx, part, pad=0):
    lib = _lib.load()
    b, h, w, c, ld = _nhwc(x)
    d_ld = _nhwc(dout)[4]
    dx_ld = _nhwc(dx)[4]
    assert tuple(dout.shape) == (b, h + 2 * pad, w + 2 * pad, c) and dout.dtype == x.dtype
    assert part.shape[0] == b and part.shape[2] == c and part.is_contiguous()
    key = _hbm_key("in_bwd_apply", x) if pad == 0 else None
    nbytes = x.numel() * _esz(x) * 3
    if fin_fusable(part.shape[1]):
        e0 = _timed_begin(key, nbytes)
        _lib.check(lib.ctg_in_bwd_stats(dtc_saved(x), _p(x), ld, _p(dout), d_ld, pad, _p(mean), _p(rstd), act, _p(dx), dx_ld, b,
                                        h, w, c, part.shape[1], _p(part), _stream()), "ctg_in_bwd_stats")
        _timed_end(key, e0)
        return
    s1, s2 = in_finalize(part, part.shape[1], h * w, mode=1)
    e0 = _timed_begin(key, nbytes)
    _lib.check(lib.ctg_in_bwd_apply(dtc_saved(x), _p(x), ld, _p(dout), d_ld, pad, _p(mean), _p(rstd), _p(s1), _p(s2), act,
                                    _p(dx), dx_ld, b, h, w, c, _stream()), "ctg_in_bwd_apply")
    _timed_end(key, e0)


def grad_combine(a, b, pad, yact, act, out):
    lib = _lib.load()
    bsz, h, w, c, o_ld = _nhwc(out)
    a_ld = _nhwc(a)[4] if a is not None else 0
    b_ld = _nhwc(b)[4] if b is not None else 0
    y_ld = _nhwc(yact)[4] if yact is not None else 0
    if b is not None:
        assert b.shape[1] == h + 2 * pad and b.shape[2] == w + 2 * pad
    _lib.check(lib.ctg_grad_combine(dtc(out), _p(a), a_ld, _p(b), b_ld, pad, _p(yact), y_ld, act, _p(out), o_ld,
                                    bsz, h, w, c, _stream()), "ctg_grad_combine")


def fold_f32(dp, pad):
    lib = _lib.load()
    b, hp, wp, c = dp.shape
    assert dp.dtype == torch.float32 and dp.is_contiguous()
    out = torch.empty((b, hp - 2 * pad, wp - 2 * pad, c), dtype=torch.float32, device=dp.device)
    _lib.check(lib.ctg_fold_f32(_p(dp), _p(out), b, hp - 2 * pad, wp - 2 * pad, c, pad, _stream()), "ctg_fold_f32")
    return out


def act_bwd_f32(g, y, act):
    lib = _lib.load()
    assert g.dtype == torch.float32 and y.dtype == torch.float32 and g.is_contiguous() and y.is_contiguous()
    assert g.numel() == y.numel()
    out = torch.empty_like(g)
    _lib.check(lib.ctg_act_bwd_f32(_p(g), _p(y), act, _p(out), g.numel(), _stream()), "ctg_act_bwd_f32")
    return out


def bias_grad(g, pad, creal, db, accumulate=False):
    lib = _lib.load()
    b, hp, wp, c, ld = _nhwc(g)
    h, w = hp - 2 * pad, wp - 2 * pad
    ns = _nslabs(b, h * w)
    part = torch.empty((b, ns, c, 2), dtype=torch.float32, device=g.device)
    _lib.check(lib.ctg_bias_grad(dtc(g), _p(g), ld, pad, b, h, w, c, creal, ns, _p(part), _p(db), int(accumulate),
                                 _stream()), "ctg_bias_grad")


def bias_grad_act(g, pad, yact, act, gout, creal, db, accumulate=False):
    lib = _lib.load()
    b, hp, wp, c, ld = _nhwc(g)
    h, w = hp - 2 * pad, wp - 2 * pad
    assert tuple(yact.shape) == (b, h, w, c) == tuple(gout.shape) and yact.dtype == g.dtype == gout.dtype
    ns = _nslabs(b, h * w)
    part = torch.empty((b, ns, c, 2), dtype=torch.float32, device=g.device)
    _lib.check(lib.ctg_bias_grad_act(dtc(g), _p(g), ld, pad, _p(yact), _nhwc(yact)[4], act, _p(gout), _nhwc(gout)[4], b, h, w, c,
                                     creal, ns, _p(part), _p(db), int(accumulate), _stream()), "ctg_bias_grad_act")


def maxpool2_fwd(x, out):
    lib = _lib.load()
    b, h, w, c, ld = _nhwc(x)
    _lib.check(lib.ctg_maxpool2_fwd(dtc(x), _p(x), ld, _p(out), _nhwc(out)[4], b, h, w, c, _stream()),
               "ctg_maxpool2_fwd")


def maxpool2_bwd(x, dout, dx, accumulate):
    lib = _lib.load()
    b, h, w, c, ld = _nhwc(x)
    _lib.check(lib.ctg_maxpool2_bwd(dtc_saved(x), _p(x), ld, _p(dout), _nhwc(dout)[4], _p(dx), _nhwc(dx)[4],
                                    int(accumulate), b, h, w, c, _stream()), "ctg_maxpool2_bwd")


def bilinear_fwd(x, out):
    lib = _lib.load()
    b, hi, wi, c, ld = _nhwc(x)
    _, ho, wo, _, o_ld = _nhwc(out)
    _lib.check(lib.ctg_bilinear_fwd(dtc(x), _p(x), ld, _p(out), o_ld, b, hi, wi, ho, wo, c, _stream()),
               "ctg_bilinear_fwd")


def bilinear_bwd(dout, dx):
    lib = _lib.load()
    b, ho, wo, c, d_ld = _nhwc(dout)
    _, hi, wi, _, dx_ld = _nhwc(dx)
    _lib.check(lib.ctg_bilinear_bwd(dtc(dx), _p(dout), d_ld, _p(dx), dx_ld, b, hi, wi, ho, wo, c, _stream()),
               "ctg_bilinear_bwd")


def copy_channels(src, dst):
    lib = _lib.load()
    b, h, w, c, s_ld = _nhwc(src)
    _lib.check(lib.ctg_copy_channels(dtc(src), _p(src), s_ld, _p(dst), _nhwc(dst)[4], c, b * h * w, _stream()),
               "ctg_copy_channels")


def chan_pad(src_f32, cs, dtype, cpad):
    lib = _lib.load()
    b, h, w, c = src_f32.shape
    assert c == cs and src_f32.is_contiguous() and src_f32.dtype == torch.float32
    out = empty_act((b, h, w, cpad), dtype, src_f32.device)
    _lib.check(lib.ctg_chan_pad(dtc(out), _p(src_f32), cs, _p(out), cpad, b * h * w, _stream()), "ctg_chan_pad")
    return out


def im2col_pack(s0, s1, k, stride, pad, pad_mode, dtype, kpad):
    lib = _lib.load()
    b, hi, wi = s0.shape
    cin = 1 if s1 is None else 2
    ho = (hi + 2 * pad - k) // stride + 1
    wo = (wi + 2 * pad - k) // stride + 1
    assert s0.is_contiguous() and (s1 is None or s1.is_contiguous())
    out = empty_act((b, ho, wo, kpad), dtype, s0.device)
    _lib.check(lib.ctg_im2col_pack(dtc(out), _p(s0), _p(s1), cin, b, hi, wi, k, k, stride, pad, pad_mode, _p(out),
                                   ho, wo, kpad, _stream()), "ctg_im2col_pack")
    return out


def kxw_ok(cin, cout, k, stride, dtype):
    return (not _NO_KXW) and cin == 1 and stride == 1 and 5 <= k <= 8 and 32 < cout <= 64 and dtype == torch.bfloat16


def kxw_pack(w2d, k, npad, dtype):
    n = w2d.shape[0]
    out = torch.zeros((npad, 8, 8), dtype=torch.float32, device=w2d.device)
    out[:n, :k, :k] = w2d.detach().reshape(n, k, k)
    return out.reshape(1, npad, 64).to(dtype).contiguous()


def conv_smallcin(s0, s1, k, stride, pad, pad_mode, w_packed, w_npad, bias, act, y, cout, want_stats=False, kxw=False):
    lib = _lib.load()
    b, hi, wi = s0.shape
    cin = 1 if s1 is None else 2
    b2, ho, wo, cy, y_ld = _nhwc(y)
    kpad = w_packed.shape[-1]
    assert b == b2 and cy == cout and (y.dtype == w_packed.dtype or (is_pair(y) and w_packed.dtype == torch.float32))
    assert w_packed.shape[-2] == w_npad
    assert s0.is_contiguous() and s0.dtype == torch.float32 and (s1 is None or (s1.is_contiguous() and s1.shape == s0.shape))
    part, slabs = None, ctypes.c_int(0)
    if want_stats and bias is None and act == ACT_NONE:
        part = torch.empty(b * ((ho + 15) // 16) * ((wo + 15) // 16) * cout * 2, dtype=torch.float32, device=y.device)
    if is_pair(y):
        w_packed = split_w_pair(w_packed, kpad)
    tok = _log_begin("first-layer conv %d->%d %dx%d s%d @%dx%d" % (cin, cout, k, k, stride, ho, wo),
                     2.0 * b * ho * wo * cout * cin * k * k, b * hi * wi * cin * 4.0 + b * ho * wo * cout * _esz(y)) \
        if OP_LOG is not None else None
    _lib.check(lib.ctg_conv_smallcin(dtc(y), _p(s0), _p(s1), cin, b, hi, wi, k, k, stride, pad, pad_mode,
                                     _p(w_packed), w_npad, kpad, int(kxw), _p(bias), act, _p(y), y_ld, ho, wo, cout, _p(part),
                                     ctypes.addressof(slabs) if part is not None else None, _stream()),
               "ctg_conv_smallcin")
    _log_end(tok)
    if part is not None and slabs.value > 0:
        part = part.view(b, slabs.value, cout, 2)
    return part, slabs.value


_TAIL_IDX = {}


def tail7_pack(weight, dtype=torch.bfloat16):
    dev = weight.device
    sc = 32 if dtype in (torch.bfloat16, "pair") else 16
    ns = 64 // sc
    idx = _TAIL_IDX.get((dev, sc))
    if idx is None:
        import numpy as np
        ix = np.full((ns, 8, 16, sc), 64 * 49, dtype=np.int64)
        for s in range(ns):
            for j in range(8):
                for o in range(2):
                    kx = j - o
                    if 0 <= kx <= 6:
                        for ky in range(7):
                            ix[s, j, o * 8 + ky, :] = (np.arange(sc) + sc * s) * 49 + ky * 7 + kx
        idx = torch.from_numpy(ix).to(dev)
        _TAIL_IDX[(dev, sc)] = idx
    flat = torch.cat([weight.detach().reshape(-1), weight.new_zeros(1)])
    if dtype == "pair":
        g = flat[idx]
        hi = g.to(torch.bfloat16)
        return torch.stack([hi, (g - hi.float()).to(torch.bfloat16)]).contiguous()
    return flat[idx].to(dtype).contiguous()


def conv_tail7(x, wp, bias, y, act):
    lib = _lib.load()
    b, h, w, c, x_ld = _nhwc(x)
    assert c == 64 and wp.dtype == x.dtype and y.dtype == torch.float32 and y.is_contiguous() and y.numel() == b * h * w
    assert not is_pair(x) or wp.shape[0] == 2
    tok = _log_begin("tail conv 64->1 7x7 @%dx%d" % (h, w), 2.0 * b * h * w * 64 * 49, b * h * w * (64 * _esz(x) + 4.0)) \
        if OP_LOG is not None else None
    _lib.check(lib.ctg_conv_tail7(dtc(x), _p(x), x_ld, _p(wp), _p(bias), _p(y), act, b, h, w, _stream()),
               "ctg_conv_tail7")
    _log_end(tok)


def conv_tail7_ok(spec_cin, spec_cout, k, stride, reflect, pad, dtype, h, w):
    if os.environ.get("CTG_NO_TAIL7"):
        return False
    return (spec_cin == 64 and spec_cout == 1 and k == 7 and stride == 1 and reflect and pad == 3
            and dtype in (torch.bfloat16, torch.float32) and h >= 4 and w >= 4)


def lds_canary(blocks=1024, spins=2000, cap=64, stream=None):
    lib = _lib.load()
    rep = torch.zeros(4 + 4 * cap, dtype=torch.int32, device="cuda")
    st = _stream() if stream is None else stream.cuda_stream
    _lib.check(lib.ctg_lds_canary(blocks, spins, _p(rep), cap, st), "ctg_lds_canary")
    return rep


def cout1_ok(cin, cout, k, stride, reflect, pad, transposed, dtype):
    if os.environ.get("CTG_NO_COUT1"):
        return False
    return (cin == 512 and cout == 1 and k == 4 and stride == 1 and not reflect and not transposed and 0 <= pad < 4
            and dtype == torch.bfloat16)


def cout1_pack(weight):
    assert tuple(weight.shape[:1]) == (1,) and weight.shape[1] == 512 and weight.shape[2] == weight.shape[3] == 4
    return weight.detach()[0].permute(1, 2, 0).reshape(16, 512).float().contiguous()


def conv_cout1_fwd(x, w16, bias, y, act, pad):
    lib = _lib.load()
    b, hi, wi, c, x_ld = _nhwc(x)
    ho, wo = hi + 2 * pad - 3, wi + 2 * pad - 3
    assert c == 512 and x.dtype == torch.bfloat16 and w16.dtype == torch.float32 and tuple(w16.shape) == (16, 512)
    assert y.dtype == torch.float32 and y.is_contiguous() and y.numel() == b * ho * wo
    tok = _log_begin("conv 512->1 16taps is1 os1 @%dx%d" % (ho, wo), 2.0 * b * ho * wo * 512 * 16, b * hi * wi * 512 * _esz(x) + 4.0 * b * ho * wo) \
        if OP_LOG is not None else None
    _lib.check(lib.ctg_conv_cout1_fwd(dtc(x), _p(x), x_ld, _p(w16), _p(bias), _p(y), act, b, hi, wi, 512, 4, pad, ho, wo, _stream()),
               "ctg_conv_cout1_fwd")
    _log_end(tok)


def conv_cout1_bwd(g, w16, dx, pad):
    lib = _lib.load()
    b, hi, wi, c, dx_ld = _nhwc(dx)
    ho, wo = hi + 2 * pad - 3, wi + 2 * pad - 3
# ... 321 lines not shown
```

cta_gan_amd/trainer/layers.py:

```python
from __future__ import annotations

import torch.nn as nn

from .. import engine as E
from ..engine import ACT_LRELU, ACT_NONE, ACT_RELU, ConvSpec
from ..nets import HipNet, ResidualBlockNet, _Slot, _attach, _res_block, _to_nchw_view, _to_nhwc

_ACTS = {"leaky_relu": ACT_LRELU, "relu": ACT_RELU, None: ACT_NONE}


def _init_conv(slot, activation, init_func):
    if init_func == "zeros":
        nn.init.normal_(slot.weight, mean=0.0, std=1e-5)
    elif init_func == "kaiming":
        act = "relu" if activation is None else activation
        a = 0.2 if activation == "leaky_relu" else 0.0
        nn.init.kaiming_normal_(slot.weight, a=a, nonlinearity=act, mode="fan_in")
    else:
        raise NotImplementedError("init_func=%r" % (init_func,))
    slot.bias.data.zero_()


class ResnetBlock(ResidualBlockNet):

    def __init__(self, dim, padding_type="reflect", norm_layer=None, use_dropout=False, use_bias=True):
        if padding_type != "reflect" or use_dropout or not use_bias:
            raise NotImplementedError("ResnetBlock: only reflect / no dropout / bias (layers.py:220-222)")
        super().__init__(dim)
        for p in (self._p("conv_block.1"), self._p("conv_block.5")):
            nn.init.kaiming_normal_(p.weight, a=0.0, nonlinearity="relu", mode="fan_in")
            p.bias.data.zero_()


class _BlockNet(HipNet):

    def _setup(self, cin, cout, k, stride, pad, activation, init_func, n_res, res_prefix, conv_key, pool):
        if activation not in _ACTS:
            raise NotImplementedError("activation=%r" % (activation,))
        if cin % 32 or cout % 32:
            raise NotImplementedError("stand-alone Conv needs channel counts that are multiples of 32")
        self.spec = ConvSpec(cin, cout, k, stride, pad, use_bias=True, act=_ACTS[activation]) if cin else None
        self.n_res, self.res_prefix, self.conv_key, self.pool, self.dim = n_res, res_prefix, conv_key, pool, cout
        if cin:
            slot = _Slot((cout, cin, k, k), (cout,))
            _attach(self, conv_key, slot)
            _init_conv(slot, activation, init_func)
        for i in range(n_res):
            for idx in (1, 5):
                slot = _Slot((cout, cout, 3, 3), (cout,))
                _attach(self, "%s.%d.conv_block.%d" % (res_prefix, i, idx), slot)
                nn.init.kaiming_normal_(slot.weight, a=0.0, nonlinearity="relu", mode="fan_in")
                slot.bias.data.zero_()

    def _run(self, tape, inputs, need_in):
        (x,) = inputs
        dt = self.dtype_
        xa = E.Act(_to_nhwc(x, dt), req=need_in[0])
        h = xa
        if self.spec is not None:
            s = self._p(self.conv_key)
            h = E.conv_forward(tape, self._cache, self.spec, h, s.weight, s.bias, dt)
        rspec = ConvSpec(self.dim, self.dim, 3, 1, 1, reflect=True, use_bias=False)
        for i in range(self.n_res):
            a, b = self._p("%s.%d.conv_block.1" % (self.res_prefix, i)), self._p("%s.%d.conv_block.5" % (self.res_prefix, i))
            h = _res_block(tape, self._cache, rspec, h, (a.weight, a.bias), (b.weight, b.bias), dt)
        outs = [h]
        if self.pool:
            outs = [E.maxpool_forward(tape, h), h]

        def finish(in_acts):
            g, _ = E.take_grad(in_acts[0])
            return [None if g is None else _to_nchw_view(g).to(x.dtype)]
        return outs, [xa], finish


class Conv(_BlockNet):

    def __init__(self, in_channels, out_channels, kernel_size, stride, padding, bias=True, activation="relu",
                 init_func="kaiming", use_norm=False, use_resnet=False, **kwargs):
        super().__init__()
        if use_norm or not bias:
            raise NotImplementedError("Conv: the reference only builds use_norm=False, bias=True on this path")
        self._setup(in_channels, out_channels, kernel_size, stride, padding, activation, init_func,
                    1 if use_resnet else 0, "resnet_block.model", "conv2d", False)

    def forward(self, x):
        return self._call(x)[0].to(x.dtype)


class DownBlock(_BlockNet):

    def __init__(self, in_channels, out_channels, kernel_size, stride, padding, bias=False, activation="relu",
                 init_func="kaiming", use_norm=False, use_resnet=False, skip=True, refine=False, pool=True,
                 pool_size=2, **kwargs):
        super().__init__()
        if use_norm or not bias or refine or not pool or pool_size != 2:
            raise NotImplementedError("DownBlock: only the configuration of trainer/reg.py:43-45 is implemented")
        self.skip = skip
        self._setup(in_channels, out_channels, kernel_size, stride, padding, activation, init_func,
                    1 if use_resnet else 0, "conv_0.resnet_block.model", "conv_0.conv2d", True)

    def forward(self, x):
        pooled, skip = self._call(x)
        pooled, skip = pooled.to(x.dtype), skip.to(x.dtype)
        return (pooled, skip) if self.skip else pooled


class ResnetTransformer(_BlockNet):

    def __init__(self, dim, n_blocks, init_func="kaiming"):
        super().__init__()
        if init_func != "kaiming":
            raise NotImplementedError("init_func=%r" % (init_func,))
        self._setup(0, dim, 3, 1, 1, None, init_func, n_blocks, "model", None, False)

    def forward(self, x):
        return self._call(x)[0].to(x.dtype)
```

include/ctagan_hip.h:

```cpp
#ifndef CTAGAN_HIP_H
#define CTAGAN_HIP_H

#ifdef __cplusplus
extern "C" {
#endif

#define CTG_ABI_VERSION 11
int ctg_abi_version(void);

typedef struct ctg_conv_epilogue {
    const void* res;
    const void* fold;
    const void* bz;
    const float* bmean;
    const float* brstd;
    float* bstats;
    int res_ld, fold_ld, bz_ld;
    int bact;
    void* nie_sync;
    int nie_act;
    int nie_tiles;
    int nie_groups;
    int nie_budget;
} ctg_conv_epilogue;

int ctg_conv_igemm(int dtype, int out_f32, const void* x, const void* w, void* y, const float* bias,
                   int B, int Hi, int Wi, int Cin, int x_ld, int Ho, int Wo, int Cout, int y_ld,
                   int Hs, int Ws, int oy0, int ox0, int os, int is, int frame, int pad_mode, int act,
                   int w_npad, int ntaps, const int* taps_host, float* stats_part, int* stats_slabs_out,
                   const ctg_conv_epilogue* epi, void* stream);
int ctg_conv_igemm_classes(int dtype, const void* x, const void* w, void* y, const float* bias, int B, int Hi, int Wi,
                           int Cin, int x_ld, int Ho, int Wo, int Cout, int y_ld, int Hs, int Ws, int pad_mode, int act,
                           int w_npad, const int* cls_ntaps, const int* cls_oy0, const int* cls_ox0, const int* taps,
                           float* stats_part, int* stats_slabs_out, void* stream);

int ctg_conv_wgrad(int dtype, const void* g, const void* x, float* part, int B, int Hs, int Ws, int Mc, int g_ld,
                   int Hi, int Wi, int Nc, int x_ld, int is, int pad_mode, int slab, int ntaps,
                   const int* taps_host, void* stream);
int ctg_wgrad_reduce(const float* part, int Z, int ntaps, int Mc, int Nc, float* dst, int Mreal, int Nreal,
                     long sm, long sn, long stp, int accumulate, void* stream);
int ctg_wgrad_reduce_multi(int count, const void* const* part, void* const* dst, const int* Z, const int* ntaps,
                           const int* Mc, const int* Nc, const int* Mreal, const int* Nreal, const long* sm,
                           const long* sn, const long* stp, const int* accumulate, void* stream);

int ctg_in_stats(int dtype, const void* x, int x_ld, int B, int H, int W, int C, int nslabs, float* part,
                 float* mean, float* rstd, void* stream);
int ctg_in_finalize(const float* part, int B, int C, int nslabs, int HW, int mode, float* mean, float* rstd, void* stream);
int ctg_in_apply(int dtype, const void* x, int x_ld, const float* mean, const float* rstd, int act,
                 const void* res, int r_ld, void* out, int o_ld, int B, int H, int W, int C, void* stream);
int ctg_in_apply_part(int dtype, const void* x, int x_ld, const float* part, int nslabs, float* mean, float* rstd, int act,
                      const void* res, int r_ld, void* out, int o_ld, int B, int H, int W, int C, void* stream);
int ctg_in_bwd_partial(int dtype, const void* x, int x_ld, const void* dout, int d_ld, int pad, const float* mean,
                       const float* rstd, int act, int B, int H, int W, int C, int nslabs, float* part, void* stream);
int ctg_in_bwd_apply(int dtype, const void* x, int x_ld, const void* dout, int d_ld, int pad, const float* mean,
                     const float* rstd, const float* s1, const float* s2, int act, void* dx, int dx_ld, int B, int H, int W,
                     int C, void* stream);
int ctg_in_bwd(int dtype, const void* x, int x_ld, const void* dout, int d_ld, int pad, const float* mean,
               const float* rstd, int act, void* dx, int dx_ld, int B, int H, int W, int C, int nslabs,
               float* part, float* s1, float* s2, void* stream);
int ctg_in_bwd_stats(int dtype, const void* x, int x_ld, const void* dout, int d_ld, int pad, const float* mean,
                     const float* rstd, int act, void* dx, int dx_ld, int B, int H, int W, int C, int nslabs,
                     const float* part, void* stream);
int ctg_grad_combine(int dtype, const void* a, int a_ld, const void* b, int b_ld, int pad, const void* yact,
                     int y_ld, int act, void* out, int o_ld, int B, int H, int W, int C, void* stream);
int ctg_fold_f32(const float* dp, float* out, int B, int H, int W, int C, int pad, void* stream);
int ctg_act_bwd_f32(const float* g, const float* y, int act, float* out, long n, void* stream);
int ctg_act_bwd_sum_f32(const float* g, const float* y, int act, float* out, long n, float* part, float* sum_out,
                        int accumulate, void* stream);
int ctg_bias_grad(int dtype, const void* g, int g_ld, int pad, int B, int H, int W, int C, int Creal, int nslabs,
                  float* part, float* db, int accumulate, void* stream);

int ctg_bias_grad_act(int dtype, const void* g, int g_ld, int pad, const void* yact, int y_ld, int act, void* gout,
                      int go_ld, int B, int H, int W, int C, int Creal, int nslabs, float* part, float* db,
                      int accumulate, void* stream);

int ctg_maxpool2_fwd(int dtype, const void* x, int x_ld, void* out, int o_ld, int B, int H, int W, int C, void* stream);
int ctg_maxpool2_bwd(int dtype, const void* x, int x_ld, const void* dout, int d_ld, void* dx, int dx_ld,
                     int accumulate, int B, int H, int W, int C, void* stream);
int ctg_bilinear_fwd(int dtype, const void* x, int x_ld, void* out, int o_ld, int B, int Hi, int Wi, int Ho, int Wo,
                     int C, void* stream);
int ctg_bilinear_bwd(int dtype, const void* dout, int d_ld, void* dx, int dx_ld, int B, int Hi, int Wi, int Ho,
                     int Wo, int C, void* stream);
int ctg_copy_channels(int dtype, const void* src, int s_ld, void* dst, int d_ld, int C, long P, void* stream);
int ctg_split_weights(const float* x, long x_ld, void* out, int C, long P, void* stream);
int ctg_split_weights_multi(int count, const void* const* x, void* const* out, const int* C, const long* P, void* stream);
int ctg_pair_convert(int dir, const void* src, long s_ld, void* dst, long d_ld, int C, long P, void* stream);
int ctg_chan_pad(int dtype, const float* src, int Cs, void* dst, int Cpad, long P, void* stream);
int ctg_im2col_pack(int dtype, const float* s0, const float* s1, int Cin, int B, int Hi, int Wi, int kh, int kw,
                    int stride, int pad, int pad_mode, void* dst, int Ho, int Wo, int Kpad, void* stream);
int ctg_conv_smallcin(int dtype, const float* s0, const float* s1, int Cin, int B, int Hi, int Wi, int kh, int kw,
                      int stride, int pad, int pad_mode, const void* w, int w_npad, int Kpad, int w_layout, const float* bias,
                      int act, void* y, int y_ld, int Ho, int Wo, int Cout, float* stats_part, int* stats_slabs_out,
                      void* stream);
int ctg_conv_tail7(int dtype, const void* x, int x_ld, const void* wp, const float* bias, float* y, int act, int B, int H,
                   int W, void* stream);
int ctg_conv_cout1_fwd(int dtype, const void* x, int x_ld, const float* w, const float* bias, float* y, int act, int B, int Hi,
                       int Wi, int Cin, int k, int pad, int Ho, int Wo, void* stream);
int ctg_conv_cout1_bwd(int dtype, const float* g, const float* w, void* dx, int dx_ld, int B, int Hi, int Wi, int Cin, int k,
                       int pad, int Ho, int Wo, void* stream);
int ctg_conv_cout1_wgrad(int dtype, const float* g, const void* x, int x_ld, float* part, int Z, int B, int Hi, int Wi, int Cin,
                         int k, int pad, int Ho, int Wo, void* stream);
int ctg_corr_smallcin(const void* g, int Gh, int Gw, int g_ld, int Mc, int gpad, int g_pad_mode, const float* i0,
                      const float* i1, int Cin, int Ih, int Iw, int kh, int kw, int ipad, int i_pad_mode, int B,
                      int Hs, int Ws, float* part, int wgs, void* stream);
int ctg_weight_pack(int dtype, const float* src, long sn, long sk, long stp, int Nreal, int Kreal, void* dst,
                    int ntaps, int Npad, int Kpad, void* stream);
int ctg_weight_pack_multi(int dtype, int count, const void* const* src, void* const* dst, const long* sn,
                          const long* sk, const long* stp, const int* nreal, const int* kreal, const int* ntaps,
                          const int* npad, const int* kpad, void* stream);

int ctg_warp_fwd(const float* src, const float* flow, long fs_n, long fs_c, long fs_y, long fs_x, float* out,
                 int B, int H, int W, void* stream);
int ctg_warp_bwd(const float* src, const float* flow, long fs_n, long fs_c, long fs_y, long fs_x,
                 const float* gout, float* dsrc, float* dflow, int B, int H, int W, void* det_ws, void* stream);

int ctg_smooth_fwd(const float* f, long sn, long sc, long sy, long sx, int B, int C, int H, int W, float weight, float* part,
                   float* out, void* stream);
int ctg_smooth_bwd(const float* f, long sn, long sc, long sy, long sx, int B, int C, int H, int W, float weight,
                   const float* gscale, float* df, int accumulate, void* stream);
int ctg_l1_fwd(const float* a, const float* b, const float* mask, long n, float weight, float* part, float* out, void* stream);
int ctg_l1_bwd(const float* a, const float* b, const float* mask, long n, float weight, const float* gscale, float* da,
               int accumulate, void* stream);
int ctg_lsgan_fwd(const float* x, int B, int HW, int nb, float t0, float s0, float t1, float s1, int mode, float* pooled,
                  float* out, void* stream);
int ctg_lsgan_bwd(const float* pooled, int B, int HW, int nb, float t0, float s0, float t1, float s1, int mode,
                  const float* gscale, float* dx, void* stream);
int ctg_sum_scalars(int count, const void* const* scalars, float* out, void* stream);
int ctg_avgpool_fwd(const float* x, int B, int HW, float* out, void* stream);
int ctg_avgpool_bwd(const float* gout, int B, int HW, float* dx, void* stream);

int ctg_to_windowdata(const float* img, const float* wc, const float* ww, float* out, int B, long HW, void* stream);
int ctg_ssim(const float* fake, const float* real, const float* wc, const float* ww, int B, int H, int W, int mode, int aliased,
             double data_range, double* part, double* out, void* stream);
int ctg_window_metrics(const float* fake, const float* real, const float* wc, const float* ww, int B, long HW,
                       int nblk, int aliased, double* part, double* out, void* stream);
int ctg_hu_to_inputs(const short* hu, float wc, float ww, float* win, float* full, long n, void* stream);
int ctg_resize_nearest(const float* src, int B, int Hi, int Wi, float* dst, int Ho, int Wo, void* stream);

int ctg_adam_step(int count, void* const* params, const void* const* grads, void* const* exp_avg,
                  void* const* exp_avg_sq, const long* numel, float lr, float beta1, float beta2, float eps,
                  int step, const float* dev_state3, void* stream);
int ctg_adam_tick(float* dev_state3, float beta1, float beta2, void* stream);

#ifdef __cplusplus
}
#endif
#endif
```

Measured before the change: 331.9 slices/s.

## Fuse instance-norm apply with maxpool, and pool/bilinear backward with norm statistics

Adds three fused kernels. The first applies instance norm and emits the 2x2 max-pooled output in one pass. The second combines the maxpool backward with the partial sums the instance-norm backward needs. The third combines the bilinear-upsample backward with the activation gradient and the bias-gradient reduction. Each is meant to remove separate elementwise passes and launches that re-read large 512x512 activations. The trade-off is more kernel and ABI surface, new env switches to disable each path, and rounding that depends on the bf16 store order.

New measurement: 330.8 slices/s. Within noise of the previous version (-0.4%).

```diff
diff --git a/cta_gan_amd/_lib.py b/cta_gan_amd/_lib.py
--- a/cta_gan_amd/_lib.py
+++ b/cta_gan_amd/_lib.py
@@ -19,6 +19,7 @@
     "ctg_in_stats": "ipiiiiiipppp",
     "ctg_in_finalize": "piiiiippp",
     "ctg_in_apply": "ipippipipiiiiip",
+    "ctg_in_apply_pool": "ipippipipipiiiiip",
     "ctg_in_apply_part": "ipipippipipiiiiip",
     "ctg_in_bwd_partial": "ipipiippiiiiiipp",
     "ctg_in_bwd_apply": "ipipiippppipiiiiip",
@@ -28,11 +29,14 @@
     "ctg_fold_f32": "ppiiiiip",
     "ctg_act_bwd_f32": "ppiplp",
     "ctg_bias_grad": "ipiiiiiiiippip",
+    "ctg_bias_finalize": "piiiipip",
     "ctg_bias_grad_act": "ipiipiipiiiiiiippip",
     "ctg_maxpool2_fwd": "ipipiiiiip",
     "ctg_maxpool2_bwd": "ipipipiiiiiip",
     "ctg_bilinear_fwd": "ipipiiiiiiip",
     "ctg_bilinear_bwd": "ipipiiiiiiip",
+    "ctg_maxpool2_bwd_stats": "ipipipiipippiiiiiipp",
+    "ctg_bilinear_bwd_act": "ipipiipiiiiiiiiippip",
     "ctg_copy_channels": "ipipiilp",
     "ctg_split_weights": "plpilp",
     "ctg_split_weights_multi": "ippppp",
@@ -72,7 +76,7 @@
     "ctg_lds_canary": "iipip",
 }
 _CT = {"i": _I, "l": _L, "p": _P, "f": _F, "d": ctypes.c_double}
-ABI_VERSION = 11
+ABI_VERSION = 12
 
 _lib = None
 
diff --git a/cta_gan_amd/csrc/common.h b/cta_gan_amd/csrc/common.h
--- a/cta_gan_amd/csrc/common.h
+++ b/cta_gan_amd/csrc/common.h
@@ -128,6 +128,9 @@
 __device__ __forceinline__ void st1(float* p, float v) { *p = v; }
 __device__ __forceinline__ void st1(bf16_t* p, float v) { *p = (bf16_t)v; }
 
+__device__ __forceinline__ float stored_as(float v, const float*) { return v; }
+__device__ __forceinline__ float stored_as(float v, const bf16_t*) { return (float)(bf16_t)v; }
+
 __device__ __forceinline__ float act_apply(float x, int act) {
     switch (act) {
         case ACT_RELU: return x > 0.f ? x : 0.f;
diff --git a/cta_gan_amd/csrc/norm_act.hip b/cta_gan_amd/csrc/norm_act.hip
--- a/cta_gan_amd/csrc/norm_act.hip
+++ b/cta_gan_amd/csrc/norm_act.hip
@@ -199,6 +199,53 @@
             for (int e = 0; e < EPC; ++e) o.v[e] += r.v[e];
         }
         o.store(out + (base + p) * o_ld + ch, o_ld);
+    }
+}
+
+template <typename T>
+__global__ __launch_bounds__(256) void in_apply_pool_kernel(const T* x, int x_ld,
+                                                            const float* __restrict__ mean,
+                                                            const float* __restrict__ rstd, int act,
+                                                            const T* res, int r_ld, T* out, int o_ld,
+                                                            T* __restrict__ pooled, int p_ld, int H, int W, int C) {
+    constexpr int EPC = Chunk<T>::N;
+    const int CPP = C / EPC, PL = 256 / CPP;
+    const int cc = threadIdx.x % CPP, pl = threadIdx.x / CPP;
+    const int n = blockIdx.y, ch = cc * EPC;
+    ChanParams<T> mu, rs;
+    mu.load(mean + n * C + ch);
+    rs.load(rstd + n * C + ch);
+    const int Wo = W >> 1, NW = (H >> 1) * Wo;
+    const size_t base = (size_t)n * H * W;
+    for (int q = blockIdx.x * PL + pl; q < NW; q += gridDim.x * PL) {
+        const int oy = q / Wo, ox = q - oy * Wo;
+        const size_t p0 = base + (size_t)(2 * oy) * W + 2 * ox;
+        Chunk<T> v[4], o[4];
+#pragma unroll
+        for (int k = 0; k < 4; ++k) v[k].load(x + (p0 + (k >> 1) * W + (k & 1)) * x_ld + ch, x_ld);
+#pragma unroll
+        for (int k = 0; k < 4; ++k)
+#pragma unroll
+            for (int e = 0; e < EPC; ++e) o[k].v[e] = act_apply((v[k].v[e] - mu.v[e]) * rs.v[e], act);
+        if (res != nullptr) {
+#pragma unroll
+            for (int k = 0; k < 4; ++k) {
+                Chunk<T> r;
+                r.load(res + (p0 + (k >> 1) * W + (k & 1)) * r_ld + ch, r_ld);
+#pragma unroll
+                for (int e = 0; e < EPC; ++e) o[k].v[e] += r.v[e];
+            }
+        }
+        Chunk<T> m;
+#pragma unroll
+        for (int k = 0; k < 4; ++k) {
+            o[k].store(out + (p0 + (k >> 1) * W + (k & 1)) * o_ld + ch, o_ld);
+#pragma unroll
+            for (int e = 0; e < EPC; ++e) o[k].v[e] = stored_as(o[k].v[e], (const T*)nullptr);
+        }
+#pragma unroll
+        for (int e = 0; e < EPC; ++e) m.v[e] = fmaxf(fmaxf(o[0].v[e], o[1].v[e]), fmaxf(o[2].v[e], o[3].v[e]));
+        m.store(pooled + ((size_t)n * NW + q) * p_ld + ch, p_ld);
     }
 }
 
@@ -526,6 +573,28 @@
     return ctg_launch_status();
 }
 
+extern "C" int ctg_in_apply_pool(int dtype, const void* x, int x_ld, const float* mean, const float* rstd, int act,
+                                 const void* res, int r_ld, void* out, int o_ld, void* pooled, int p_ld, int B, int H, int W,
+                                 int C, void* stream) {
+    CTG_ENTER();
+    if (check_c(dtype, C) || out == nullptr || pooled == nullptr || H < 2 || W < 2 || (H & 1) || (W & 1)) return CTG_EINVAL;
+    if (dtype != DT_BF16 && dtype != DT_F32) return CTG_EINVAL;
+    const int pl = 256 / (C / (dtype == DT_F32 ? 4 : 8));
+    const long nw = (long)(H / 2) * (W / 2);
+    int per = 4;
+    if (!ctg_knobs().no_smallb) while (per > 1 && ((nw + pl * per - 1) / (pl * per)) * B < 2048) per >>= 1;
+    long bx = (nw + pl * per - 1) / (pl * per);
+    bx = bx < 1 ? 1 : bx > 4096 ? 4096 : bx;
+    const dim3 grid((unsigned)bx, (unsigned)B);
+    if (dtype == DT_BF16)
+        hipLaunchKernelGGL((in_apply_pool_kernel<bf16_t>), grid, dim3(256), 0, (hipStream_t)stream, (const bf16_t*)x, x_ld, mean,
+                           rstd, act, (const bf16_t*)res, r_ld, (bf16_t*)out, o_ld, (bf16_t*)pooled, p_ld, H, W, C);
+    else
+        hipLaunchKernelGGL((in_apply_pool_kernel<float>), grid, dim3(256), 0, (hipStream_t)stream, (const float*)x, x_ld, mean,
+                           rstd, act, (const float*)res, r_ld, (float*)out, o_ld, (float*)pooled, p_ld, H, W, C);
+    return ctg_launch_status();
+}
+
 static inline dim3 fused_grid(int dtype, int B, int HW, int C, int nslabs, int* cgc_out) {
     const int cpp = C / (dtype == DT_F32 ? 4 : 8);
     const int cgc = cpp < 8 ? cpp : 8;
@@ -632,6 +701,14 @@
     return ctg_launch_status();
 }
 
+extern "C" int ctg_bias_finalize(const float* part, int B, int nslabs, int C, int Creal, float* db, int accumulate, void* stream) {
+    CTG_ENTER();
+    if (part == nullptr || db == nullptr || B < 1 || nslabs < 1 || Creal < 1 || Creal > C) return CTG_EINVAL;
+    hipLaunchKernelGGL(bias_finalize_kernel, dim3(Creal), dim3(64), 0, (hipStream_t)stream, part, B, nslabs, C, Creal, db,
+                       accumulate);
+    return ctg_launch_status();
+}
+
 extern "C" int ctg_bias_grad_act(int dtype, const void* g, int g_ld, int pad, const void* yact, int y_ld, int act, void* gout,
                                  int go_ld, int B, int H, int W, int C, int Creal, int nslabs, float* part, float* db,
                                  int accumulate, void* stream) {
diff --git a/cta_gan_amd/csrc/spatial.hip b/cta_gan_amd/csrc/spatial.hip
--- a/cta_gan_amd/csrc/spatial.hip
+++ b/cta_gan_amd/csrc/spatial.hip
@@ -76,6 +76,79 @@
     }
 }
 
+template <int EPC>
+__device__ __forceinline__ void slab_sums_store(const float (&s1)[EPC], const float (&s2)[EPC], int pl, int PL, int ch, int C,
+                                                float* __restrict__ out) {
+    __shared__ float stage[256 * 8];
+#pragma unroll
+    for (int which = 0; which < 2; ++which) {
+        __syncthreads();
+#pragma unroll
+        for (int e = 0; e < EPC; ++e) stage[pl * C + ch + e] = which ? s2[e] : s1[e];
+        __syncthreads();
+        for (int c = threadIdx.x; c < C; c += 256) {
+            float s = 0.f;
+            for (int q = 0; q < PL; ++q) s += stage[q * C + c];
+            out[c * 2 + which] = s;
+        }
+    }
+}
+
+template <typename T>
+__global__ __launch_bounds__(256) void maxpool2_bwd_stats_kernel(const T* __restrict__ x, int x_ld, const T* __restrict__ dout,
+                                                                 int d_ld, T* dx, int dx_ld, int accumulate,
+                                                                 const T* __restrict__ z, int z_ld,
+                                                                 const float* __restrict__ mean, const float* __restrict__ rstd,
+                                                                 int act, int H, int W, int C, float* __restrict__ part) {
+    constexpr int EPC = Chunk<T>::N;
+    const int CPP = C / EPC, PL = 256 / CPP;
+    const int cc = threadIdx.x % CPP, pl = threadIdx.x / CPP;
+    const int n = blockIdx.y, slab = blockIdx.x, nslabs = gridDim.x, ch = cc * EPC;
+    const int Wo = W >> 1, NWIN = (H >> 1) * Wo;
+    const int per = (NWIN + nslabs - 1) / nslabs;
+    const int qbeg = slab * per, qend = min(qbeg + per, NWIN);
+    float s1[EPC], s2[EPC], mu[EPC], rs[EPC];
+#pragma unroll
+    for (int e = 0; e < EPC; ++e) { s1[e] = 0.f; s2[e] = 0.f; mu[e] = mean[n * C + ch + e]; rs[e] = rstd[n * C + ch + e]; }
+    const size_t base = (size_t)n * H * W;
+    for (int q = qbeg + pl; q < qend; q += PL) {
+        const int oy = q / Wo, ox = q - oy * Wo;
+        const size_t p0 = base + (size_t)(2 * oy) * W + 2 * ox;
+        Chunk<T> w[4], zz[4], o[4], g;
+#pragma unroll
+        for (int k = 0; k < 4; ++k) {
+            const size_t p = p0 + (k >> 1) * W + (k & 1);
+            w[k].load(x + p * x_ld + ch, x_ld);
+            zz[k].load(z + p * z_ld + ch, z_ld);
+            if (accumulate) o[k].load(dx + p * dx_ld + ch, dx_ld);
+            else o[k].zero();
+        }
+        g.load(dout + ((size_t)n * NWIN + q) * d_ld + ch, d_ld);
+#pragma unroll
+        for (int e = 0; e < EPC; ++e) {
+            int arg = 0;
+            float m = w[0].v[e];
+#pragma unroll
+            for (int k = 1; k < 4; ++k)
+                if (w[k].v[e] > m) { m = w[k].v[e]; arg = k; }
+#pragma unroll
+            for (int k = 0; k < 4; ++k) {
+                float v = arg == k ? g.v[e] : 0.f;
+                if (accumulate) v += o[k].v[e];
+                o[k].v[e] = v;
+                float gg = stored_as(v, (const T*)nullptr);
+                const float xh = (zz[k].v[e] - mu[e]) * rs[e];
+                if (act == ACT_RELU) gg = xh > 0.f ? gg : 0.f;
+                else if (act == ACT_LRELU) gg = xh > 0.f ? gg : LRELU_SLOPE * gg;
+                s1[e] += gg; s2[e] += gg * xh;
+            }
+        }
+#pragma unroll
+        for (int k = 0; k < 4; ++k) o[k].store(dx + (p0 + (k >> 1) * W + (k & 1)) * dx_ld + ch, dx_ld);
+    }
+    slab_sums_store<EPC>(s1, s2, pl, PL, ch, C, part + (((size_t)n * nslabs + slab) * C) * 2);
+}
+
 __device__ __forceinline__ void bil_src(int o, float scale, int Hi, int& i0, int& i1, float& l) {
     float s = scale * ((float)o + 0.5f) - 0.5f;
     s = s < 0.f ? 0.f : s;
@@ -163,6 +236,67 @@
 }
 
 template <typename T>
+__global__ __launch_bounds__(256) void bilinear_bwd_act_kernel(const T* __restrict__ dout, int d_ld, const T* __restrict__ y,
+                                                               int y_ld, int act, T* __restrict__ gm, int g_ld, int Hi, int Wi,
+                                                               int Ho, int Wo, int C, float* __restrict__ part) {
+    constexpr int EPC = Chunk<T>::N;
+    const int CPP = C / EPC, PL = 256 / CPP;
+    const int cc = threadIdx.x % CPP, pl = threadIdx.x / CPP;
+    const int n = blockIdx.y, slab = blockIdx.x, nslabs = gridDim.x, ch = cc * EPC;
+    const int HW = Hi * Wi;
+    const int per = (HW + nslabs - 1) / nslabs;
+    const int pbeg = slab * per, pend = min(pbeg + per, HW);
+    const float sh = (float)Hi / (float)Ho, sw = (float)Wi / (float)Wo;
+    float s1[EPC], s2[EPC];
+#pragma unroll
+    for (int e = 0; e < EPC; ++e) { s1[e] = 0.f; s2[e] = 0.f; }
+    const T* b = dout + (size_t)n * Ho * Wo * d_ld + ch;
+    for (int p = pbeg + pl; p < pend; p += PL) {
+        const int iy = p / Wi, ix = p - iy * Wi;
+        float wy[5], wx[5];
+#pragma unroll
+        for (int k = 0; k < 5; ++k) {
+            const int oy = 2 * iy - 2 + k, ox = 2 * ix - 2 + k;
+            wy[k] = 0.f; wx[k] = 0.f;
+            if (oy >= 0 && oy < Ho) {
+                int a0, a1; float l;
+                bil_src(oy, sh, Hi, a0, a1, l);
+                wy[k] = (a0 == iy ? 1.f - l : 0.f) + (a1 == iy ? l : 0.f);
+            }
+            if (ox >= 0 && ox < Wo) {
+                int a0, a1; float l;
+                bil_src(ox, sw, Wi, a0, a1, l);
+                wx[k] = (a0 == ix ? 1.f - l : 0.f) + (a1 == ix ? l : 0.f);
+            }
+        }
+        Chunk<T> o, yy;
+        o.zero();
+        const size_t pix = (size_t)n * HW + p;
+        yy.load(y + pix * y_ld + ch, y_ld);
+        for (int a = 0; a < 5; ++a) {
+            if (wy[a] == 0.f) continue;
+            const int oy = 2 * iy - 2 + a;
+            for (int c = 0; c < 5; ++c) {
+                if (wx[c] == 0.f) continue;
+                const int ox = 2 * ix - 2 + c;
+                Chunk<T> g;
+                g.load(b + ((size_t)oy * Wo + ox) * d_ld, d_ld);
+                const float w = wy[a] * wx[c];
+#pragma unroll
+                for (int e = 0; e < EPC; ++e) o.v[e] += w * g.v[e];
+            }
+        }
+#pragma unroll
+        for (int e = 0; e < EPC; ++e) {
+            o.v[e] = stored_as(o.v[e], (const T*)nullptr) * act_grad_from_out(yy.v[e], act);
+            s1[e] += o.v[e];
+        }
+        o.store(gm + pix * g_ld + ch, g_ld);
+    }
+    slab_sums_store<EPC>(s1, s2, pl, PL, ch, C, part + (((size_t)n * nslabs + slab) * C) * 2);
+}
+
+template <typename T>
 __global__ void chan_pad_kernel(const float* __restrict__ src, int Cs, T* __restrict__ dst, int Cpad, long P) {
     constexpr int EPC = Chunk<T>::N;
     const int CPP = Cpad / EPC;
@@ -287,6 +421,53 @@
                                          (hipStream_t)stream, (const T*)dout, d_ld, (T*)dx, dx_ld, Hi, Wi, Ho, Wo, C,
                                          items));
     return ctg_launch_status();
+}
+
+static inline bool slab_c_ok(int dtype, int C) {
+    const int epc = dtype == DT_F32 ? 4 : 8;
+    const int cpp = C / epc;
+    return C % epc == 0 && cpp > 0 && cpp <= 256 && (cpp & (cpp - 1)) == 0;
+}
+#define SPATIAL_MAX_SLABS 128
+
+extern "C" int ctg_maxpool2_bwd_stats(int dtype, const void* x, int x_ld, const void* dout, int d_ld, void* dx, int dx_ld,
+                                      int accumulate, const void* z, int z_ld, const float* mean, const float* rstd, int act,
+                                      int B, int H, int W, int C, int nslabs, float* part, void* stream) {
+    CTG_ENTER();
+    if ((dtype != DT_BF16 && dtype != DT_F32) || !slab_c_ok(dtype, C) || H < 2 || W < 2 || (H & 1) || (W & 1)) return CTG_EINVAL;
+    if (nslabs < 1 || nslabs > SPATIAL_MAX_SLABS || z == nullptr || mean == nullptr || rstd == nullptr || part == nullptr) return CTG_EINVAL;
+    if (act != ACT_NONE && act != ACT_RELU && act != ACT_LRELU) return CTG_EINVAL;
+    if ((long)B * H * W >= (1L << 31)) return CTG_EINVAL;
+    const dim3 grid((unsigned)nslabs, (unsigned)B);
+    if (dtype == DT_BF16)
+        hipLaunchKernelGGL((maxpool2_bwd_stats_kernel<bf16_t>), grid, dim3(256), 0, (hipStream_t)stream, (const bf16_t*)x, x_ld,
+                           (const bf16_t*)dout, d_ld, (bf16_t*)dx, dx_ld, accumulate, (const bf16_t*)z, z_ld, mean, rstd, act, H, W,
+                           C, part);
+    else
+        hipLaunchKernelGGL((maxpool2_bwd_stats_kernel<float>), grid, dim3(256), 0, (hipStream_t)stream, (const float*)x, x_ld,
+                           (const float*)dout, d_ld, (float*)dx, dx_ld, accumulate, (const float*)z, z_ld, mean, rstd, act, H, W, C,
+                           part);
+    return ctg_launch_status();
+}
+
+extern "C" int ctg_bilinear_bwd_act(int dtype, const void* dout, int d_ld, const void* y, int y_ld, int act, void* gm, int g_ld,
+                                    int B, int Hi, int Wi, int Ho, int Wo, int C, int Creal, int nslabs, float* part, float* db,
+                                    int accumulate, void* stream) {
+    CTG_ENTER();
+    if ((dtype != DT_BF16 && dtype != DT_F32) || !slab_c_ok(dtype, C) || Ho != 2 * Hi || Wo != 2 * Wi || Hi < 1 || Wi < 1) return CTG_EINVAL;
+    if (nslabs < 1 || nslabs > SPATIAL_MAX_SLABS || y == nullptr || gm == nullptr || part == nullptr || db == nullptr || Creal > C) return CTG_EINVAL;
+    if (act != ACT_RELU && act != ACT_LRELU) return CTG_EINVAL;
+    if ((long)B * Ho * Wo >= (1L << 31)) return CTG_EINVAL;
+    const dim3 grid((unsigned)nslabs, (unsigned)B);
+    if (dtype == DT_BF16)
+        hipLaunchKernelGGL((bilinear_bwd_act_kernel<bf16_t>), grid, dim3(256), 0, (hipStream_t)stream, (const bf16_t*)dout, d_ld,
+                           (const bf16_t*)y, y_ld, act, (bf16_t*)gm, g_ld, Hi, Wi, Ho, Wo, C, part);
+    else
+        hipLaunchKernelGGL((bilinear_bwd_act_kernel<float>), grid, dim3(256), 0, (hipStream_t)stream, (const float*)dout, d_ld,
+                           (const float*)y, y_ld, act, (float*)gm, g_ld, Hi, Wi, Ho, Wo, C, part);
+    const int st = ctg_launch_status();
+    if (st != CTG_OK) return st;
+    return ctg_bias_finalize(part, B, nslabs, C, Creal, db, accumulate, stream);
 }
 
 __global__ void split_weights_kernel(const float* __restrict__ x, long x_ld, bf16_t* __restrict__ out, int C, long P) {
diff --git a/cta_gan_amd/engine.py b/cta_gan_amd/engine.py
--- a/cta_gan_amd/engine.py
+++ b/cta_gan_amd/engine.py
@@ -12,7 +12,8 @@
 
 
 class Act:
-    __slots__ = ("t", "grad", "req", "moments", "in_src", "in_plain", "grad_stats")
+    __slots__ = ("t", "grad", "req", "moments", "in_src", "in_plain", "grad_stats", "n_cons", "n_deliv", "masked", "act_src",
+                 "pooled")
 
     def __init__(self, t: torch.Tensor, req: bool = False):
         self.t = t
@@ -22,6 +23,11 @@
         self.in_src = None
         self.in_plain = False
         self.grad_stats = None
+        self.n_cons = 0
+        self.n_deliv = 0
+        self.masked = None
+        self.act_src = None
+        self.pooled = None
 
     @property
     def shape(self):
@@ -46,9 +52,22 @@
 _EMU_BF16_BWD = int(os.environ.get("CTG_EMU_BF16_BWD", "0") or 0)
 
 
+def note_consumer(tape, a: Act):
+    if tape.enabled and a.req:
+        a.n_cons += 1
+
+
+def last_delivery(a: Act) -> bool:
+    return a.n_cons > 0 and a.n_deliv + 1 == a.n_cons
+
+
 def add_grad(a: Act, g: torch.Tensor, pad: int = 0):
     if not a.req:
         return
+    if a.masked is not None:
+        raise RuntimeError("gradient added to an activation whose gradient a fused launch already stored through the "
+                           "producer's activation mask (engine.last_delivery was wrong about its consumers)")
+    a.n_deliv += 1
     if a.grad is None:
         a.grad = (g, pad)
         return
@@ -216,6 +235,7 @@
 def conv_forward(tape: Tape, cache: PackCache, spec: ConvSpec, x: Act, weight, bias, dtype,
                  img_sources=None) -> Act:
     dev = weight.device
+    note_consumer(tape, x)
     pad_mode = PAD_REFLECT if spec.reflect else PAD_ZERO
     b_eff = bias if spec.use_bias else None
     odt = torch.float32 if spec.out_f32 else dtype
@@ -287,6 +307,9 @@
     out = Act(y, req=tape.enabled)
     if moments is not None and moments[1] > 0:
         out.moments = moments
+    if (tape.enabled and spec.act in (ACT_RELU, ACT_LRELU) and b_eff is not None and preq[1] and not spec.out_f32
+            and spec.cout % 8 == 0 and not _NO_BIAS_ACT):
+        out.act_src = (spec.act, bias)
     if tape.enabled:
         tape.record(lambda: _conv_backward(cache, spec, x, out, weight, bias, dtype, packed_x, preq))
     return out
@@ -295,14 +318,19 @@
 def _conv_backward(cache, spec: ConvSpec, x: Act, out: Act, weight, bias, dtype, packed_x, preq=(True, True)):
     wreq, breq = preq
     g, _ = take_grad(out)
+    mk, out.masked = out.masked, None
     if g is None:
         return
+    if mk is not None and mk[0] is not g:
+        raise RuntimeError("masked gradient of a conv output was replaced before the conv's backward ran")
     dev = weight.device
     bsz, ho, wo, cout = out.t.shape
     pad_mode = PAD_REFLECT if spec.reflect else PAD_ZERO
     kk = spec.kk
     tail_db = fused_db = None
-    if (spec.act != ACT_NONE and spec.out_f32 and cout == 1 and spec.use_bias and bias is not None and breq):
+    if mk is not None:
+        fused_db = mk[1]
+    elif (spec.act != ACT_NONE and spec.out_f32 and cout == 1 and spec.use_bias and bias is not None and breq):
         tail_db = _grad_like(bias)
         g = ops.act_bwd_sum_f32(g.contiguous(), out.t.contiguous(), spec.act, tail_db)
     elif spec.act != ACT_NONE:
@@ -531,7 +559,7 @@
 
 
 def conv_inorm_forward(tape: Tape, cache: PackCache, spec: ConvSpec, x: Act, weight, bias, dtype, act: int,
-                       res: Optional[Act] = None, out_t: Optional[torch.Tensor] = None) -> Act:
+                       res: Optional[Act] = None, out_t: Optional[torch.Tensor] = None, pool: bool = False) -> Act:
     if (not tape.enabled) and (not spec.use_bias) and spec.act == ACT_NONE and (not spec.transposed) and (not spec.out_f32) \
             and x.t.shape[-1] == spec.cin:
         bsz, hi, wi, _ = x.t.shape
@@ -544,10 +572,14 @@
             if r is not None:
                 return Act(o, req=False)
     y = conv_forward(tape, cache, spec, x, weight, bias, dtype)
-    return inorm_forward(tape, y, act, res=res, out_t=out_t)
-
-
-def inorm_forward(tape: Tape, y: Act, act: int, res: Optional[Act] = None, out_t: Optional[torch.Tensor] = None) -> Act:
+    return inorm_forward(tape, y, act, res=res, out_t=out_t, pool=pool)
+
+
+def inorm_forward(tape: Tape, y: Act, act: int, res: Optional[Act] = None, out_t: Optional[torch.Tensor] = None,
+                  pool: bool = False) -> Act:
+    note_consumer(tape, y)
+    if res is not None:
+        note_consumer(tape, res)
     if y.moments is not None:
         part, nsl = y.moments
         y.moments = None
@@ -559,12 +591,19 @@
         o = y.t
     else:
         o = ops.empty_like_act(y.t)
+    pooled = None
     if ops.fin_fusable(nsl):
         mean, rstd = ops.in_apply_part(y.t, part, act, res.t if res is not None else None, o)
     else:
         mean, rstd = ops.in_finalize(part, nsl, y.t.shape[1] * y.t.shape[2])
-        ops.in_apply(y.t, mean, rstd, act, res.t if res is not None else None, o)
+        _, h_, w_, c_ = y.t.shape
+        if pool and not ops.NO_IN_POOL and h_ % 2 == 0 and w_ % 2 == 0 and not ops.is_pair(y.t):
+            pooled = ops.empty_act((y.t.shape[0], h_ // 2, w_ // 2, c_), y.t.dtype, y.t.device)
+            ops.in_apply_pool(y.t, mean, rstd, act, res.t if res is not None else None, o, pooled)
+        else:
+            ops.in_apply(y.t, mean, rstd, act, res.t if res is not None else None, o)
     out = Act(o, req=tape.enabled)
+    out.pooled = pooled
     if tape.enabled:
         out.in_src = (y.t, mean, rstd, act)
         out.in_plain = res is None
@@ -591,6 +630,7 @@
 
 
 def bnorm_forward(tape: Tape, y: Act, act: int, bn) -> Act:
+    note_consumer(tape, y)
     b, h, w, c = y.t.shape
     n = b * h * w
     training = bool(bn.training)
@@ -647,17 +687,36 @@
 
 
 def maxpool_forward(tape: Tape, x: Act) -> Act:
+    note_consumer(tape, x)
     b, h, w, c = x.t.shape
-    o = ops.empty_act((b, h // 2, w // 2, c), x.t.dtype, x.t.device)
-    ops.maxpool2_fwd(x.t, o)
+    if x.pooled is not None:
+        o, x.pooled = x.pooled, None
+    else:
+        o = ops.empty_act((b, h // 2, w // 2, c), x.t.dtype, x.t.device)
+        ops.maxpool2_fwd(x.t, o)
     out = Act(o, req=tape.enabled)
     if tape.enabled:
         def bwd():
             g, _ = take_grad(out)
             if g is None or not x.req:
                 return
+            cpp = c // ops.epc(x.t.dtype)
+            want_in = (x.in_src is not None and last_delivery(x) and not ops.NO_POOL_STATS and ops.dtc_saved(x.t) in (0, 1)
+                       and g.dtype == x.t.dtype and h % 2 == 0 and w % 2 == 0 and c % ops.epc(x.t.dtype) == 0
+                       and cpp & (cpp - 1) == 0 and cpp <= 256)
             if x.grad is not None and x.grad[1] == 0 and x.grad[0].shape == x.t.shape:
-                ops.maxpool2_bwd(x.t, g, x.grad[0], True)
+                if want_in:
+                    z, mean, rstd, zact = x.in_src
+                    x.grad_stats = (x.grad[0], ops.maxpool2_bwd_stats(x.t, g, x.grad[0], True, z, mean, rstd, zact))
+                else:
+                    ops.maxpool2_bwd(x.t, g, x.grad[0], True)
+                x.n_deliv += 1
+            elif want_in and x.grad is None:
+                z, mean, rstd, zact = x.in_src
+                dx = ops.empty_act(x.t.shape, g.dtype, g.device)
+                part = ops.maxpool2_bwd_stats(x.t, g, dx, False, z, mean, rstd, zact)
+                add_grad(x, dx, 0)
+                x.grad_stats = (dx, part)
             else:
                 dx = ops.empty_act(x.t.shape, g.dtype, g.device)
                 ops.maxpool2_bwd(x.t, g, dx, False)
@@ -667,6 +726,8 @@
 
 
 def upsample_concat_forward(tape: Tape, x: Act, skip: Act, buf: Optional[torch.Tensor] = None) -> Act:
+    note_consumer(tape, x)
+    note_consumer(tape, skip)
     b, h, w, c1 = x.t.shape
     _, hs, ws, c2 = skip.t.shape
     in_place = buf is not None
@@ -682,7 +743,16 @@
             g, _ = take_grad(out)
             if g is None:
                 return
-            if x.req:
+            cpp = c1 // ops.epc(g.dtype)
+            if (x.req and x.act_src is not None and x.grad is None and last_delivery(x) and not ops.NO_BIL_ACT
+                    and ops.dtc_saved(x.t) in (0, 1) and g.dtype == x.t.dtype and c1 % ops.epc(g.dtype) == 0 and cpp & (cpp - 1) == 0 and cpp <= 256):
+                act, bias = x.act_src
+                gm = ops.empty_act(x.t.shape, g.dtype, g.device)
+                db = _grad_like(bias)
+                ops.bilinear_bwd_act(g[..., :c1], x.t, act, gm, c1, db)
+                add_grad(x, gm, 0)
+                x.masked = (gm, db)
+            elif x.req:
                 dx = ops.empty_act(x.t.shape, g.dtype, g.device)
                 ops.bilinear_bwd(g[..., :c1], dx)
                 add_grad(x, dx, 0)
diff --git a/cta_gan_amd/nets.py b/cta_gan_amd/nets.py
--- a/cta_gan_amd/nets.py
+++ b/cta_gan_amd/nets.py
@@ -117,6 +117,8 @@
         ctx.net = net
         ctx.n_in = n_in
         ctx.in_shapes = [tuple(t.shape) for t in inputs]
+        for a in out_acts:
+            E.note_consumer(tape, a)
         outs = tuple(_to_nchw_view(a.t) for a in out_acts)
         return outs
 
@@ -264,9 +266,9 @@
         return [a], [x_act], _image_grad_finish(c)
 
 
-def _res_block(tape, cache, spec, x: Act, wb1, wb2, dt, out_t=None) -> Act:
+def _res_block(tape, cache, spec, x: Act, wb1, wb2, dt, out_t=None, pool=False) -> Act:
     h = E.conv_inorm_forward(tape, cache, spec, x, wb1[0], wb1[1], dt, ACT_RELU)
-    return E.conv_inorm_forward(tape, cache, spec, h, wb2[0], wb2[1], dt, ACT_NONE, res=x, out_t=out_t)
+    return E.conv_inorm_forward(tape, cache, spec, h, wb2[0], wb2[1], dt, ACT_NONE, res=x, out_t=out_t, pool=pool)
 
 
 class ResidualBlockNet(HipNet):
@@ -426,11 +428,12 @@
     def forward(self, img_a, img_b):
         return self._call(img_a, img_b)[0]
 
-    def _resblocks(self, tape, x, key, dim, n, dt, out_t=None):
+    def _resblocks(self, tape, x, key, dim, n, dt, out_t=None, pool=False):
         spec = ConvSpec(dim, dim, 3, 1, 1, reflect=True, use_bias=False)
         for i in range(n):
             x = _res_block(tape, self._cache, spec, x, self._wb("%s.model.%d.conv_block.1" % (key, i)),
-                           self._wb("%s.model.%d.conv_block.5" % (key, i)), dt, out_t=out_t if i == n - 1 else None)
+                           self._wb("%s.model.%d.conv_block.5" % (key, i)), dt, out_t=out_t if i == n - 1 else None,
+                           pool=pool and i == n - 1)
         return x
 
     def _run(self, tape: Tape, inputs, need_in):
@@ -459,7 +462,7 @@
             else:
                 x = E.conv_forward(tape, cache, spec, x, wgt, bias, dt)
             buf = ops.empty_act((b, hh, ww, c_up[i] + c), dt, img_a.device)
-            x = self._resblocks(tape, x, "down_%d.conv_0.resnet_block" % i, c, 1, dt, out_t=buf[..., c_up[i]:])
+            x = self._resblocks(tape, x, "down_%d.conv_0.resnet_block" % i, c, 1, dt, out_t=buf[..., c_up[i]:], pool=True)
             skips.append((x, buf))
             x = E.maxpool_forward(tape, x)
             cin = c
diff --git a/cta_gan_amd/ops.py b/cta_gan_amd/ops.py
--- a/cta_gan_amd/ops.py
+++ b/cta_gan_amd/ops.py
@@ -42,6 +42,9 @@
 _NO_SMALLB = bool(_env("CTG_NO_SMALLB"))
 _FIN_FUSE = bool(_env("CTG_FIN_FUSE"))
 _NO_KXW = bool(_env("CTG_NO_KXW"))
+NO_IN_POOL = bool(_env("CTG_NO_IN_POOL"))
+NO_POOL_STATS = bool(_env("CTG_NO_POOL_STATS"))
+NO_BIL_ACT = bool(_env("CTG_NO_BIL_ACT"))
 DETERMINISTIC = bool(_env("CTG_DETERMINISTIC"))
 
 
@@ -656,6 +659,16 @@
     _timed_end(key, e0)
 
 
+def in_apply_pool(x, mean, rstd, act, res, out, pooled):
+    lib = _lib.load()
+    b, h, w, c, ld = _nhwc(x)
+    o_ld = _nhwc(out)[4]
+    r_ld = _nhwc(res)[4] if res is not None else 0
+    assert tuple(pooled.shape) == (b, h // 2, w // 2, c) and pooled.dtype == x.dtype == out.dtype and not is_pair(x)
+    _lib.check(lib.ctg_in_apply_pool(dtc(x), _p(x), ld, _p(mean), _p(rstd), act, _p(res), r_ld, _p(out), o_ld, _p(pooled),
+                                     _nhwc(pooled)[4], b, h, w, c, _stream()), "ctg_in_apply_pool")
+
+
 def in_apply_part(x, part, act, res, out):
     lib = _lib.load()
     b, h, w, c, ld = _nhwc(x)
@@ -793,6 +806,18 @@
                                     int(accumulate), b, h, w, c, _stream()), "ctg_maxpool2_bwd")
 
 
+def maxpool2_bwd_stats(x, dout, dx, accumulate, z, mean, rstd, act):
+    lib = _lib.load()
+    b, h, w, c, ld = _nhwc(x)
+    assert tuple(z.shape) == (b, h, w, c) == tuple(dx.shape) and z.dtype == x.dtype == dx.dtype == dout.dtype
+    ns = int(max(1, min(128, ((h // 2) * (w // 2) + 255) // 256)))
+    part = torch.empty((b, ns, c, 2), dtype=torch.float32, device=x.device)
+    _lib.check(lib.ctg_maxpool2_bwd_stats(dtc(x), _p(x), ld, _p(dout), _nhwc(dout)[4], _p(dx), _nhwc(dx)[4], int(accumulate),
+                                          _p(z), _nhwc(z)[4], _p(mean), _p(rstd), act, b, h, w, c, ns, _p(part), _stream()),
+               "ctg_maxpool2_bwd_stats")
+    return part
+
+
 def bilinear_fwd(x, out):
     lib = _lib.load()
     b, hi, wi, c, ld = _nhwc(x)
@@ -807,6 +832,17 @@
     _, hi, wi, _, dx_ld = _nhwc(dx)
     _lib.check(lib.ctg_bilinear_bwd(dtc(dx), _p(dout), d_ld, _p(dx), dx_ld, b, hi, wi, ho, wo, c, _stream()),
                "ctg_bilinear_bwd")
+
+
+def bilinear_bwd_act(dout, yact, act, gm, creal, db, accumulate=False):
+    lib = _lib.load()
+    b, ho, wo, c, d_ld = _nhwc(dout)
+    _, hi, wi, _, g_ld = _nhwc(gm)
+    assert tuple(yact.shape) == (b, hi, wi, c) == tuple(gm.shape) and yact.dtype == gm.dtype == dout.dtype
+    ns = _nslabs(b, hi * wi)
+    part = torch.empty((b, ns, c, 2), dtype=torch.float32, device=gm.device)
+    _lib.check(lib.ctg_bilinear_bwd_act(dtc(gm), _p(dout), d_ld, _p(yact), _nhwc(yact)[4], act, _p(gm), g_ld, b, hi, wi, ho, wo, c,
+                                        creal, ns, _p(part), _p(db), int(accumulate), _stream()), "ctg_bilinear_bwd_act")
 
 
 def copy_channels(src, dst):
diff --git a/cta_gan_amd/trainer/layers.py b/cta_gan_amd/trainer/layers.py
--- a/cta_gan_amd/trainer/layers.py
+++ b/cta_gan_amd/trainer/layers.py
@@ -63,7 +63,8 @@
         rspec = ConvSpec(self.dim, self.dim, 3, 1, 1, reflect=True, use_bias=False)
         for i in range(self.n_res):
             a, b = self._p("%s.%d.conv_block.1" % (self.res_prefix, i)), self._p("%s.%d.conv_block.5" % (self.res_prefix, i))
-            h = _res_block(tape, self._cache, rspec, h, (a.weight, a.bias), (b.weight, b.bias), dt)
+            h = _res_block(tape, self._cache, rspec, h, (a.weight, a.bias), (b.weight, b.bias), dt,
+                           pool=self.pool and i == self.n_res - 1)
         outs = [h]
         if self.pool:
             outs = [E.maxpool_forward(tape, h), h]
diff --git a/include/ctagan_hip.h b/include/ctagan_hip.h
--- a/include/ctagan_hip.h
+++ b/include/ctagan_hip.h
@@ -5,7 +5,7 @@
 extern "C" {
 #endif
 
-#define CTG_ABI_VERSION 11
+#define CTG_ABI_VERSION 12
 int ctg_abi_version(void);
 
 typedef struct ctg_conv_epilogue {
@@ -48,6 +48,9 @@
 int ctg_in_finalize(const float* part, int B, int C, int nslabs, int HW, int mode, float* mean, float* rstd, void* stream);
 int ctg_in_apply(int dtype, const void* x, int x_ld, const float* mean, const float* rstd, int act,
                  const void* res, int r_ld, void* out, int o_ld, int B, int H, int W, int C, void* stream);
+int ctg_in_apply_pool(int dtype, const void* x, int x_ld, const float* mean, const float* rstd, int act,
+                      const void* res, int r_ld, void* out, int o_ld, void* pooled, int p_ld, int B, int H, int W, int C,
+                      void* stream);
 int ctg_in_apply_part(int dtype, const void* x, int x_ld, const float* part, int nslabs, float* mean, float* rstd, int act,
                       const void* res, int r_ld, void* out, int o_ld, int B, int H, int W, int C, void* stream);
 int ctg_in_bwd_partial(int dtype, const void* x, int x_ld, const void* dout, int d_ld, int pad, const float* mean,
@@ -69,6 +72,7 @@
                         int accumulate, void* stream);
 int ctg_bias_grad(int dtype, const void* g, int g_ld, int pad, int B, int H, int W, int C, int Creal, int nslabs,
                   float* part, float* db, int accumulate, void* stream);
+int ctg_bias_finalize(const float* part, int B, int nslabs, int C, int Creal, float* db, int accumulate, void* stream);
 
 int ctg_bias_grad_act(int dtype, const void* g, int g_ld, int pad, const void* yact, int y_ld, int act, void* gout,
                       int go_ld, int B, int H, int W, int C, int Creal, int nslabs, float* part, float* db,
@@ -81,6 +85,12 @@
                      int C, void* stream);
 int ctg_bilinear_bwd(int dtype, const void* dout, int d_ld, void* dx, int dx_ld, int B, int Hi, int Wi, int Ho,
                      int Wo, int C, void* stream);
+int ctg_maxpool2_bwd_stats(int dtype, const void* x, int x_ld, const void* dout, int d_ld, void* dx, int dx_ld,
+                           int accumulate, const void* z, int z_ld, const float* mean, const float* rstd, int act, int B,
+                           int H, int W, int C, int nslabs, float* part, void* stream);
+int ctg_bilinear_bwd_act(int dtype, const void* dout, int d_ld, const void* y, int y_ld, int act, void* gm, int g_ld, int B,
+                         int Hi, int Wi, int Ho, int Wo, int C, int Creal, int nslabs, float* part, float* db,
+                         int accumulate, void* stream);
 int ctg_copy_channels(int dtype, const void* src, int s_ld, void* dst, int d_ld, int C, long P, void* stream);
 int ctg_split_weights(const float* x, long x_ld, void* out, int C, long P, void* stream);
 int ctg_split_weights_multi(int count, const void* const* x, void* const* out, const int* C, const long* P, void* stream);
```
